# Kamino666/Video-Captioning-Transformer

Hardware: AMD Instinct MI355X
Metric: video-caption train samples/sec (whole node) (higher is better)
Workload: dtype bf16; 1 GPU; configs[1]: 2 enc + 2 dec layers d=512 ff=2048 H=8 V=30522, synthetic (256,12,512) features -> 20-token captions per GPU, fwd+bwd+Adam, dropout 0.3, SCE alpha 0.5; global_batch=256, per_gpu_batch=256, seq_len=20, frames=12, parallelism=dp1, executor=list

## Files before the change

### include/vct_hip.h

```cpp
#ifndef VCT_HIP_H
#define VCT_HIP_H
#include <stdint.h>

#ifdef __cplusplus
extern "C" {
#endif

#define VCT_ABI_VERSION 15

enum { VCT_F32 = 0, VCT_BF16 = 1 };
enum { VCT_ACT_NONE = 0, VCT_ACT_GELU = 1, VCT_ACT_RELU = 2 };
enum {
  VCT_OK = 0,
  VCT_E_ARG = -1,
  VCT_E_SHAPE = -2,
  VCT_E_ALIGN = -3,
  VCT_E_WORKSPACE = -4
};

int vct_abi_version(void);
int vct_build_info(char* buf, int buflen);

typedef struct vct_gemm_adam {
  float* param; float* exp_avg; float* exp_avg_sq;
  void* shadow; int64_t ld_shadow;
  void* pk_stream; int32_t pk_K, pk_mode; int32_t pk_chunk0[4]; int32_t pk_row0; int32_t store_grad;
  const float* hyper; const int32_t* step;
} vct_gemm_adam;

typedef struct vct_gemm_desc {
  int32_t dtype;
  int32_t out_dtype;
  int32_t ta, tb;
  int32_t M, N, K;
  int32_t act;
  const void* A; int64_t lda;
  const void* B; int64_t ldb;
  void* C; int64_t ldc;
  const float* bias;
  void* preact; int64_t ld_preact;
  const void* addend; int64_t ld_addend;
  const void* dact_src; int64_t ld_dact;
  const uint32_t* seed; uint32_t site; float p_drop;
  float* bias_grad;
  void* workspace; int64_t workspace_bytes;
  int32_t split_k;
  int32_t reserved;
  int32_t n_tile_counters;
  int32_t* tile_counters;
  const vct_gemm_adam* adam;
} vct_gemm_desc;
int vct_gemm(const vct_gemm_desc* d, void* stream);
int64_t vct_gemm_workspace_bytes(const vct_gemm_desc* d);

#define VCT_GEMM_GROUP_MAX 8
int vct_gemm_grouped(const vct_gemm_desc* descs, int32_t n, void* stream);
int64_t vct_gemm_grouped_workspace_bytes(const vct_gemm_desc* descs, int32_t n, int32_t i);

typedef struct vct_attn_desc {
  int32_t dtype;
  int32_t B, H, Lq, Lk, hd;
  int32_t causal;
  int32_t key_pad_shift;
  const void* q; int64_t ldq;
  const void* k; int64_t ldk;
  const void* v; int64_t ldv;
  void* o; int64_t ldo;
  const uint8_t* key_pad;
  const uint32_t* seed; uint32_t site; float p_drop;
  const void* d_o; int64_t ld_do;
  void* dq; int64_t ld_dq;
  void* dk; int64_t ld_dk;
  void* dv; int64_t ld_dv;
  int64_t q_bs, k_bs, v_bs, o_bs;
  const int64_t* key_ids; int64_t key_ids_bs; int64_t pad_id;
} vct_attn_desc;
int vct_attn_fwd(const vct_attn_desc* d, void* stream);
int vct_attn_bwd(const vct_attn_desc* d, void* stream);

typedef struct vct_attn_weights_desc {
  int32_t dtype;
  int32_t B, H, Lq, Lk, hd;
  int32_t causal;
  int32_t key_pad_shift;
  const void* q; int64_t ldq;
  const void* k; int64_t ldk;
  float* w; int64_t ldw;
  const uint8_t* key_pad;
  int64_t q_bs, k_bs, w_bs;
  const int64_t* key_ids; int64_t key_ids_bs; int64_t pad_id;
} vct_attn_weights_desc;
int vct_attn_weights(const vct_attn_weights_desc* d, void* stream);

typedef struct vct_ss_norm { const float* gamma; const float* beta; void* y; float* mean; float* rstd; } vct_ss_norm;
typedef struct vct_layer_ss_desc {
  int32_t dtype, B, L, Lm, d, H, ff, act;
  int32_t last, causal, key_pad_shift, reserved;
  const void* wpk; int64_t nchunks;
  const void* x; const void* mem;
  const float* b_qkv; const float* b_o;
  void* qkv; void* o; void* a;
  vct_ss_norm n1;
  const float* b_cq; const float* b_ckv; const float* b_co;
  void* cq; void* ckv; void* co; void* ca;
  vct_ss_norm n2;
  const float* b1; const float* b2;
  void* hpre; void* h; void* f;
  vct_ss_norm n3;
  vct_ss_norm nf;
  const uint8_t* key_pad; const int64_t* key_ids; int64_t key_ids_bs; int64_t pad_id;
  const uint32_t* seed; float p_drop;
  uint32_t site_sa, site_n1, site_ca, site_n2, site_ff, site_n3;
  uint32_t site_emb;
  int32_t pro, feats_dtype;
  const void* feats; void* x_in; const float* b_unify; const float* pe_rows;
  const int64_t* emb_ids; int64_t emb_ids_bs; const float* emb_table; const float* emb_pos;
} vct_layer_ss_desc;
typedef struct vct_ss_pack_seg { const void* w; int64_t ldw; int32_t nchunks; int32_t transposed; int64_t dst_chunk; } vct_ss_pack_seg;
int vct_layer_ss_supported(int dtype, int d, int H, int ff, int L, int Lm);
int64_t vct_layer_ss_stream_chunks(int ff, int cross);
int vct_ss_pack(const vct_ss_pack_seg* segs, int nseg, void* dst, void* stream);
int vct_layer_ss_fwd(const vct_layer_ss_desc* layers, int n_layers, void* stream);

typedef struct vct_ss_bwd_norm { const float* gamma; const float* mean; const float* rstd; float* ws; } vct_ss_bwd_norm;
typedef struct vct_layer_ss_bwd_desc {
  int32_t dtype, B, L, d, H, ff, act, last, causal, key_pad_shift;
  const void* wpk; int64_t nchunks;
  const void* dy; void* dx; const void* y_last;
  const void* x; const void* qkv; const void* a; const void* x1; const void* hpre; const void* f;
  vct_ss_bwd_norm n1, n3, nf;
  void* df; void* dhpre; void* da; void* dqkv;
  const uint8_t* key_pad; const int64_t* key_ids; int64_t key_ids_bs; int64_t pad_id;
  const uint32_t* seed; float p_drop;
  uint32_t site_sa, site_n1, site_ff, site_n3;
} vct_layer_ss_bwd_desc;
int64_t vct_layer_ss_bwd_stream_chunks(int ff);
int vct_layer_ss_bwd(const vct_layer_ss_bwd_desc* layers, int n_layers, void* stream);

int vct_add_ln_fwd(int dtype, int M, int d, const void* x, const void* res, const float* gamma,
                   const float* beta, void* y, float* mean, float* rstd, const uint32_t* seed,
                   uint32_t site, float p_drop, void* stream);
int vct_add_ln_ln_fwd(int dtype, int M, int d, const void* x, const void* res, const float* gamma, const float* beta,
                      void* y, float* mean, float* rstd, const float* gamma2, const float* beta2, void* y2, float* mean2,
                      float* rstd2, const uint32_t* seed, uint32_t site, float p_drop, void* stream);
int vct_add_ln_bwd(int dtype, int M, int d, const void* dy, const void* x, const void* res,
                   const float* gamma, const float* mean, const float* rstd, void* ds, void* dxo,
                   float* dgamma, float* dbeta, float* param_ws, const uint32_t* seed, uint32_t site,
                   float p_drop, void* stream);
int vct_add_ln_ln_bwd(int dtype, int M, int d, const void* dy2, const void* y, const float* gamma2, const float* mean2,
                      const float* rstd2, float* param_ws2, const void* x, const void* res, const float* gamma,
                      const float* mean, const float* rstd, void* ds, void* dxo, float* param_ws, const uint32_t* seed,
                      uint32_t site, float p_drop, void* stream);
int vct_ln_ws_rows(int M);
int vct_ln_param_finalize_batched(const int64_t* table_dev, int n_entries, int d, void* stream);

int vct_enc_frontend_fwd(int dtype, int B, int T, int d, const void* u, const float* pe_rows, void* z,
                         void* stream);
int vct_enc_frontend_bwd(int dtype, int B, int T, int d, const void* dz, void* du, void* stream);

#define VCT_MM_MAX_MODAL 8
typedef struct vct_mm_frontend_desc {
  int32_t dtype, n, B, d;
  int32_t n_labels, reserved;
  int32_t T[VCT_MM_MAX_MODAL];
  const void* u[VCT_MM_MAX_MODAL];
  const uint8_t* mask[VCT_MM_MAX_MODAL];
  const float* temp; const float* modal_w; const int32_t* labels;
  void* x0; uint8_t* key_pad;
  const void* dx;
  void* du[VCT_MM_MAX_MODAL];
  float* d_modal;
} vct_mm_frontend_desc;
int vct_mm_frontend_fwd(const vct_mm_frontend_desc* d, void* stream);
int vct_mm_frontend_bwd(const vct_mm_frontend_desc* d, void* stream);

#define VCT_AGG_MEAN 0
#define VCT_AGG_MAX 1
#define VCT_TEMPORAL_FIXED 0
#define VCT_TEMPORAL_LEARNED 1
typedef struct vct_enc_frontend_ex_desc {
  int32_t dtype, n, B, d;
  int32_t n_labels, agg, temporal, norm;
  int32_t emb_rows; uint32_t site; float p_drop; int32_t reserved;
  int32_t T[VCT_MM_MAX_MODAL];
  const void* u[VCT_MM_MAX_MODAL];
  const uint8_t* mask[VCT_MM_MAX_MODAL];
  const float* temp;
  const float* emb_w; const int32_t* tidx;
  const float* modal_w; const int32_t* labels;
  const float* gamma; const float* beta;
  const uint32_t* seed;
  void* x0; uint8_t* key_pad;
  float* mean; float* rstd;
  const void* dx;
  void* du[VCT_MM_MAX_MODAL];
  float* d_modal;
  float* d_emb;
  float* dpre; float* param_ws;
} vct_enc_frontend_ex_desc;
int vct_enc_frontend_ex_fwd(const vct_enc_frontend_ex_desc* d, void* stream);
int vct_enc_frontend_ex_bwd(const vct_enc_frontend_ex_desc* d, void* stream);

typedef struct vct_hmm_mix_desc {
  int32_t dtype, B, S, d;
  int32_t init, reserved;
  const uint8_t* take;
  const void* y; const void* x0; void* x;
  const void* dx;
  void* dy;
  float* acc;
  void* dx0;
} vct_hmm_mix_desc;
int vct_hmm_mix_fwd(const vct_hmm_mix_desc* d, void* stream);
int vct_hmm_mix_bwd(const vct_hmm_mix_desc* d, void* stream);

int vct_embed_fwd(int dtype, int B, int S, int d, const int64_t* ids, int64_t id_batch_stride,
                  const void* table, const float* pos, void* x, const uint32_t* seed, uint32_t site,
                  float p_drop, void* stream);
int vct_embed_bwd(int dtype, int B, int S, int d, int V, const int64_t* ids, int64_t id_batch_stride,
                  int64_t pad_id, const void* dx, float* dtable, int32_t* id_ws, int64_t id_ws_ints, int incremental,
                  const uint32_t* seed, uint32_t site, float p_drop, void* stream);

int vct_sce_loss(int dtype, int N, int S, int V, const void* logits, int64_t ldl, const int64_t* labels,
                 int64_t label_batch_stride, int64_t pad_id, float alpha, float* loss_out, void* dlogits,
                 int64_t ld_dl, float* row_ws, void* stream);

int vct_wce_loss(int dtype, int N, int S, int V, const void* logits, int64_t ldl, const int64_t* labels,
                 int64_t label_batch_stride, int64_t pad_id, const float* seq_w, float* loss_out, float* tok_logp,
                 void* dlogits, int64_t ld_dl, float* row_ws, void* stream);

int vct_group_sum(int dtype, int B, int G, int R, int d, const void* in, void* out, void* stream);

#define VCT_CIDER_MAX_LEN 64
#define VCT_CIDER_MAX_ORDER 4
typedef struct vct_cider_desc {
  int32_t B, N, L, n;
  const int64_t* ids;
  int64_t stride_b, stride_n, stride_l;
  int64_t end_id;
  double log_nvid, two_sigma_sq;
  const int32_t* vid_rows;
  int32_t n_videos, table_cap;
  const int32_t* table_keys;
  const double* table_idf;
  const int32_t* vid_ref_ptr;
  const int32_t* ref_len;
  const double* ref_norm;
  const int32_t* ref_ent_ptr;
  const int32_t* ent_keys;
  const double* ent_w;
  float* reward;
} vct_cider_desc;
int vct_cider_d(const vct_cider_desc* d, void* stream);
int vct_scst_advantages(int B, int N, const float* rewards, const float* baseline, float* adv, float* base_out, float* means,
                        void* stream);

enum { VCT_MATCH_CSL = 0, VCT_MATCH_CSL_WDS = 1 };
enum { VCT_MATCH_TEMP_NONE = 0, VCT_MATCH_TEMP_EXP = 1, VCT_MATCH_TEMP_DIV = 2 };
typedef struct vct_match_loss_desc {
  int32_t B, Dt, loss_kind, temp_kind;
  const float* text; int64_t ld_text;
  const float* vid; int64_t ld_vid;
  const float* temp;
  float* loss;
  float* dvid; int64_t ld_dvid;
  float* dtemp;
  float* sim; int64_t ld_sim;
  void* workspace; int64_t workspace_bytes;
} vct_match_loss_desc;
int vct_match_loss(const vct_match_loss_desc* d, void* stream);
int64_t vct_match_loss_workspace_bytes(int B, int Dt);

typedef struct vct_match_agg_desc {
  int32_t dtype, B, Te, d;
  int32_t empty; float beta;
  const void* mem; float* agg;
  const float* dagg; void* dmem;
} vct_match_agg_desc;
int vct_match_agg_fwd(const vct_match_agg_desc* d, void* stream);
int vct_match_agg_bwd(const vct_match_agg_desc* d, void* stream);

int vct_scale(float* x, int64_t n, float s, void* stream);
int vct_axpby(float* out, const float* x, float a, const float* y, float b, int64_t n, void* stream);

int vct_gather_pad_rows(int out_dtype, int B, int Tmax, int E, const float* store, const int64_t* offsets,
                        const int64_t* idx, void* out, uint8_t* mask, void* stream);

int vct_adam_step(float* param, const float* grad, float* exp_avg, float* exp_avg_sq, void* shadow_bf16,
                  int64_t n, float lr, float beta1, float beta2, float eps, float weight_decay,
                  int32_t* step_dev, int64_t shadow_skip_begin, int64_t shadow_skip_end, int32_t bump_step,
                  const float* hyper_dev, void* stream);
typedef struct vct_adam_pack_seg { int64_t begin, end; int32_t K, mode; int32_t chunk0[4]; void* stream; } vct_adam_pack_seg;
int vct_adam_step_pk(float* param, const float* grad, float* exp_avg, float* exp_avg_sq, void* shadow_bf16,
                     int64_t n, float lr, float beta1, float beta2, float eps, float weight_decay,
                     int32_t* step_dev, int64_t shadow_skip_begin, int64_t shadow_skip_end, int32_t bump_step,
                     const float* hyper_dev, const vct_adam_pack_seg* segs_dev, int32_t nseg, int64_t base, void* stream);
typedef struct vct_adam_range { int64_t begin, end; int32_t blk0, shadow; } vct_adam_range;
int vct_adam_step_ranges(float* param, const float* grad, float* exp_avg, float* exp_avg_sq, void* shadow_bf16,
                         const vct_adam_range* ranges_dev, int32_t nranges, int32_t total_blocks, float lr, float beta1, float beta2,
                         float eps, float weight_decay, int32_t* step_dev, const float* hyper_dev,
                         const vct_adam_pack_seg* segs_dev, int32_t nseg, void* stream);
int vct_adam_step_2d(float* param, const float* grad, float* exp_avg, float* exp_avg_sq, void* shadow_bf16,
                     void* shadow_t_bf16, int32_t rows, int32_t cols, int64_t ld_t, float lr, float beta1, float beta2,
                     float eps, float weight_decay, int32_t* step_dev, const float* hyper_dev, void* stream);

int vct_cast(int src_dtype, int dst_dtype, const void* src, void* dst, int64_t n, void* stream);
int vct_warm(const void* src, int64_t bytes, void* stream);
int vct_transpose(int dtype, int rows, int cols, const void* src, int64_t ld_src, void* dst, int64_t ld_dst, void* stream);
int vct_argmax_rows(int dtype, int rows, int cols, const void* x, int64_t ldx, int64_t* out, int64_t out_stride,
                    void* stream);
int vct_greedy_select(int dtype, int rows, int cols, const void* x, int64_t ldx, int64_t* out, int64_t out_stride,
                      int64_t end_id, uint8_t* ended, int32_t* ended_count, int64_t* all_ended_at, int32_t t,
                      void* stream);
int vct_beam_select(int dtype, int B, int K, int V, const void* x, int64_t ldx, float* scores, uint8_t* finished,
                    int32_t* parent, int64_t* out, int64_t out_stride, int64_t end_id, int64_t pad_id,
                    int32_t* finished_count, int64_t* all_finished_at, int32_t t, void* workspace, int64_t workspace_bytes,
                    void* stream);
int vct_beam_reorder(int dtype, int L, int M, int Lmax, int d, int t, const int32_t* parent, const void* src, void* dst,
                     int64_t layer_stride, void* stream);
typedef struct vct_sample_ctl {
  uint32_t seed;
  int32_t top_k;
  float inv_temp;
  float top_p;
} vct_sample_ctl;

typedef struct vct_sample_select_desc {
  int32_t dtype;
  int32_t rows, V, t;
  const void* x;
  int64_t ldx;
  int64_t* out;
  int64_t out_stride;
  int64_t end_id, pad_id;
  uint8_t* ended;
  int32_t* ended_count;
  int64_t* all_ended_at;
  float* step_logp;
  float* seq_logp;
  const vct_sample_ctl* ctl;
  void* workspace;
  int64_t workspace_bytes;
} vct_sample_select_desc;

int64_t vct_sample_select_workspace_bytes(int dtype, int rows, int V);
int vct_sample_select(const vct_sample_select_desc* d, void* stream);
enum { VCT_DEC_PRO_NONE = 0, VCT_DEC_PRO_EMBED = 1, VCT_DEC_PRO_LN = 2, VCT_DEC_PRO_LN_LN = 3, VCT_DEC_PRO_SELF_ATTN = 4,
       VCT_DEC_PRO_CROSS_ATTN = 5 };
typedef struct vct_decode_gemv_desc {
  int32_t wdtype, B, N, K;
  const void* W; int64_t ldw;
  const float* bias;
  int32_t pro, act;
  const float* x_in; int64_t ld_x;
  const float* g1; const float* b1; const float* g2; const float* b2;
  const int64_t* ids; int64_t id_stride; const float* table; const float* pos_row;
  const void* q; int64_t q_bs; const void* kc; const void* vc; int64_t kv_ld, kv_bs; int32_t H, Lk;
  const float* res; int64_t ld_res;
  void* out; int64_t ld_out; int32_t out_native; int32_t rows_per_wave;
  float* x_out;
} vct_decode_gemv_desc;
int vct_decode_gemv(const vct_decode_gemv_desc* d, void* stream);

typedef struct vct_decode_linear_desc {
  int32_t M, N, K;
  int32_t out_dtype, act, res_dtype;
  const void* x; int64_t ldx;
  const float* x_pre; int64_t ld_pre;
  const float* ln_g; const float* ln_b;
  float* x_norm; int64_t ld_norm;
  const void* W; int64_t ldw;
  const float* bias;
  const void* res; int64_t ld_res;
  void* out; int64_t ldo;
  const int64_t* ids; int64_t id_stride;
} vct_decode_linear_desc;
int vct_decode_linear(const vct_decode_linear_desc* d, void* stream);
int vct_decode_ln2(int M, int K, const float* x, int64_t ldx, const float* g1, const float* b1, const float* g2, const float* b2,
                   void* y, int64_t ldy, void* stream);

typedef struct vct_decode_block_desc {
  int32_t kind, d, ff, V, Lk, act;
  const int64_t* id; const float* table; const float* pos_row;
  const float* res; const float* res_bias; const float* part; int32_t n_part, pad0;
  const float* g1; const float* b1; const float* g2; const float* b2;
  float* x_out;
  const void* w_a; int64_t ld_a; const float* b_a;
  void* slot;
  const void* kc; const void* vc; int64_t kv_ld;
  const void* w_b; int64_t ld_b;
  float* part_out;
  float* sel_ws; int64_t* tok_out; int64_t end_id; uint8_t* ended; int32_t* ended_count; int64_t* all_ended_at; int32_t t, pad1;
} vct_decode_block_desc;
int vct_decode_block_supported(int dtype, int d, int H, int ff, int Lk);
int vct_decode_block(const vct_decode_block_desc* d, void* stream);

int vct_advance_seed(uint32_t* seed, void* stream);

int vct_cmdlist_create(void** out_list);
int vct_cmdlist_destroy(void* list);
int vct_cmdlist_begin(void* list, void* main_stream);
int vct_cmdlist_end(void* list);
int vct_cmdlist_replay(void* list, void* main_stream);
int vct_cmdlist_size(void* list);
int vct_cmdlist_streams(void* list);
int vct_cmdlist_inject_status(int status, void* stream);
int vct_cmdlist_host_call(int (*fn)(void*), void* arg, void* stream);
int vct_stream_wait(void* waiter_stream, void* signal_stream);
int vct_sync_record(int id, void* stream);
int vct_sync_wait(int id, void* stream);
int vct_comm_available(void);
int vct_comm_unique_id(uint8_t* out128);
int vct_comm_init(const uint8_t* id128, int rank, int world, void** out_comm);
int vct_comm_destroy(void* comm);
int vct_comm_rank(void* comm);
int vct_comm_world(void* comm);
int vct_comm_stream(void* comm, void** out_stream);
int vct_comm_allreduce_avg(void* comm, void* buf, int64_t count, int dtype, void* after_stream, int order_after);
int vct_comm_reduce_scatter_avg(void* comm, void* buf, int64_t count_per_rank, int dtype, void* after_stream, int order_after);
int vct_comm_all_gather(void* comm, void* buf, int64_t count_per_rank, int dtype, void* after_stream, int order_after);
int vct_comm_broadcast(void* comm, void* buf, int64_t count, int dtype, int root, void* after_stream, int order_after);
int vct_comm_wait(void* comm, void* stream);

int vct_stream_create_masked(const uint32_t* cu_mask, int words, void** out_stream);
int vct_stream_destroy(void* stream);
int vct_tap_enable(int on);
int vct_tap(int tag, int phase, void* stream);
int vct_tap_collect(int tag, float* ms_out, int cap);

#ifdef __cplusplus
}
#endif
#endif
```

### video-captioning-transformer_amd/_lib.py

```python
import ctypes as C
import os

import torch

_PKG = os.path.dirname(os.path.abspath(__file__))
LIB_PATH = os.path.join(_PKG, "libvct_hip.so")
_AB_LIB = os.environ.get("VCT_LIB_PATH")

F32, BF16 = 0, 1
ABI_VERSION = 15
GEMM_GROUP_MAX = 8
ACT = {"none": 0, None: 0, "gelu": 1, "relu": 2}
_ERR = {-1: "VCT_E_ARG (null pointer / bad enum)", -2: "VCT_E_SHAPE (unsupported shape)",
        -3: "VCT_E_ALIGN (leading dimension / alignment)", -4: "VCT_E_WORKSPACE (workspace too small)"}

vp, i32, i64, u32, f32, f64 = C.c_void_p, C.c_int32, C.c_int64, C.c_uint32, C.c_float, C.c_double


class GemmAdam(C.Structure):
    _fields_ = [("param", vp), ("exp_avg", vp), ("exp_avg_sq", vp), ("shadow", vp), ("ld_shadow", i64),
                ("pk_stream", vp), ("pk_K", i32), ("pk_mode", i32), ("pk_chunk0", i32 * 4), ("pk_row0", i32), ("store_grad", i32),
                ("hyper", vp), ("step", vp)]


class AdamRange(C.Structure):
    _fields_ = [("begin", i64), ("end", i64), ("blk0", i32), ("shadow", i32)]


class GemmDesc(C.Structure):
    _fields_ = [("dtype", i32), ("out_dtype", i32), ("ta", i32), ("tb", i32), ("M", i32), ("N", i32), ("K", i32),
                ("act", i32), ("A", vp), ("lda", i64), ("B", vp), ("ldb", i64), ("C", vp), ("ldc", i64),
                ("bias", vp), ("preact", vp), ("ld_preact", i64), ("addend", vp), ("ld_addend", i64),
                ("dact_src", vp), ("ld_dact", i64), ("seed", vp), ("site", u32), ("p_drop", f32),
                ("bias_grad", vp), ("workspace", vp), ("workspace_bytes", i64), ("split_k", i32), ("reserved", i32),
                ("n_tile_counters", i32), ("tile_counters", vp), ("adam", C.POINTER(GemmAdam))]


class AttnDesc(C.Structure):
    _fields_ = [("dtype", i32), ("B", i32), ("H", i32), ("Lq", i32), ("Lk", i32), ("hd", i32), ("causal", i32),
                ("key_pad_shift", i32), ("q", vp), ("ldq", i64), ("k", vp), ("ldk", i64), ("v", vp), ("ldv", i64),
                ("o", vp), ("ldo", i64), ("key_pad", vp), ("seed", vp), ("site", u32), ("p_drop", f32),
                ("d_o", vp), ("ld_do", i64), ("dq", vp), ("ld_dq", i64), ("dk", vp), ("ld_dk", i64),
                ("dv", vp), ("ld_dv", i64), ("q_bs", i64), ("k_bs", i64), ("v_bs", i64), ("o_bs", i64),
                ("key_ids", vp), ("key_ids_bs", i64), ("pad_id", i64)]


class AttnWeightsDesc(C.Structure):
    _fields_ = [("dtype", i32), ("B", i32), ("H", i32), ("Lq", i32), ("Lk", i32), ("hd", i32), ("causal", i32),
                ("key_pad_shift", i32), ("q", vp), ("ldq", i64), ("k", vp), ("ldk", i64), ("w", vp), ("ldw", i64),
                ("key_pad", vp), ("q_bs", i64), ("k_bs", i64), ("w_bs", i64), ("key_ids", vp), ("key_ids_bs", i64), ("pad_id", i64)]


class SsNorm(C.Structure):
    _fields_ = [("gamma", vp), ("beta", vp), ("y", vp), ("mean", vp), ("rstd", vp)]


class LayerSsDesc(C.Structure):
    _fields_ = [("dtype", i32), ("B", i32), ("L", i32), ("Lm", i32), ("d", i32), ("H", i32), ("ff", i32), ("act", i32),
                ("last", i32), ("causal", i32), ("key_pad_shift", i32), ("reserved", i32),
                ("wpk", vp), ("nchunks", i64), ("x", vp), ("mem", vp), ("b_qkv", vp), ("b_o", vp), ("qkv", vp), ("o", vp), ("a", vp),
                ("n1", SsNorm), ("b_cq", vp), ("b_ckv", vp), ("b_co", vp), ("cq", vp), ("ckv", vp), ("co", vp), ("ca", vp),
                ("n2", SsNorm), ("b1", vp), ("b2", vp), ("hpre", vp), ("h", vp), ("f", vp), ("n3", SsNorm), ("nf", SsNorm),
                ("key_pad", vp), ("key_ids", vp), ("key_ids_bs", i64), ("pad_id", i64), ("seed", vp), ("p_drop", f32),
                ("site_sa", u32), ("site_n1", u32), ("site_ca", u32), ("site_n2", u32), ("site_ff", u32), ("site_n3", u32), ("site_emb", u32),
                ("pro", i32), ("feats_dtype", i32), ("feats", vp), ("x_in", vp), ("b_unify", vp), ("pe_rows", vp),
                ("emb_ids", vp), ("emb_ids_bs", i64), ("emb_table", vp), ("emb_pos", vp)]


class SsPackSeg(C.Structure):
    _fields_ = [("w", vp), ("ldw", i64), ("nchunks", i32), ("transposed", i32), ("dst_chunk", i64)]


class AdamPackSeg(C.Structure):
    _fields_ = [("begin", i64), ("end", i64), ("K", i32), ("mode", i32), ("chunk0", i32 * 4), ("stream", vp)]


class SsBwdNorm(C.Structure):
    _fields_ = [("gamma", vp), ("mean", vp), ("rstd", vp), ("ws", vp)]


class LayerSsBwdDesc(C.Structure):
    _fields_ = [("dtype", i32), ("B", i32), ("L", i32), ("d", i32), ("H", i32), ("ff", i32), ("act", i32), ("last", i32), ("causal", i32),
                ("key_pad_shift", i32), ("wpk", vp), ("nchunks", i64), ("dy", vp), ("dx", vp), ("y_last", vp),
                ("x", vp), ("qkv", vp), ("a", vp), ("x1", vp), ("hpre", vp), ("f", vp),
                ("n1", SsBwdNorm), ("n3", SsBwdNorm), ("nf", SsBwdNorm),
                ("df", vp), ("dhpre", vp), ("da", vp), ("dqkv", vp),
                ("key_pad", vp), ("key_ids", vp), ("key_ids_bs", i64), ("pad_id", i64), ("seed", vp), ("p_drop", f32),
                ("site_sa", u32), ("site_n1", u32), ("site_ff", u32), ("site_n3", u32)]


class DecodeGemvDesc(C.Structure):
    _fields_ = [("wdtype", i32), ("B", i32), ("N", i32), ("K", i32), ("W", vp), ("ldw", i64), ("bias", vp), ("pro", i32), ("act", i32),
                ("x_in", vp), ("ld_x", i64), ("g1", vp), ("b1", vp), ("g2", vp), ("b2", vp),
                ("ids", vp), ("id_stride", i64), ("table", vp), ("pos_row", vp),
                ("q", vp), ("q_bs", i64), ("kc", vp), ("vc", vp), ("kv_ld", i64), ("kv_bs", i64), ("H", i32), ("Lk", i32),
                ("res", vp), ("ld_res", i64), ("out", vp), ("ld_out", i64), ("out_native", i32), ("rows_per_wave", i32),
                ("x_out", vp)]


class DecodeLinearDesc(C.Structure):
    _fields_ = [("M", i32), ("N", i32), ("K", i32), ("out_dtype", i32), ("act", i32), ("res_dtype", i32),
                ("x", vp), ("ldx", i64), ("x_pre", vp), ("ld_pre", i64), ("ln_g", vp), ("ln_b", vp), ("x_norm", vp), ("ld_norm", i64),
                ("W", vp), ("ldw", i64), ("bias", vp), ("res", vp), ("ld_res", i64), ("out", vp), ("ldo", i64),
                ("ids", vp), ("id_stride", i64)]


class DecodeBlockDesc(C.Structure):
    _fields_ = [("kind", i32), ("d", i32), ("ff", i32), ("V", i32), ("Lk", i32), ("act", i32),
                ("id", vp), ("table", vp), ("pos_row", vp), ("res", vp), ("res_bias", vp), ("part", vp), ("n_part", i32), ("pad0", i32),
                ("g1", vp), ("b1", vp), ("g2", vp), ("b2", vp), ("x_out", vp), ("w_a", vp), ("ld_a", i64), ("b_a", vp), ("slot", vp),
                ("kc", vp), ("vc", vp), ("kv_ld", i64), ("w_b", vp), ("ld_b", i64), ("part_out", vp),
                ("sel_ws", vp), ("tok_out", vp), ("end_id", i64), ("ended", vp), ("ended_count", vp), ("all_ended_at", vp), ("t", i32), ("pad1", i32)]


MM_MAX_MODAL = 8


class MmFrontendDesc(C.Structure):
    _fields_ = [("dtype", i32), ("n", i32), ("B", i32), ("d", i32), ("n_labels", i32), ("reserved", i32),
                ("T", i32 * MM_MAX_MODAL), ("u", vp * MM_MAX_MODAL), ("mask", vp * MM_MAX_MODAL),
                ("temp", vp), ("modal_w", vp), ("labels", vp), ("x0", vp), ("key_pad", vp), ("dx", vp),
                ("du", vp * MM_MAX_MODAL), ("d_modal", vp)]


AGG = {"avg": 0, "max": 1}
TEMPORAL = {"encoding": 0, "embedding": 1}


class EncFrontendExDesc(C.Structure):
    _fields_ = [("dtype", i32), ("n", i32), ("B", i32), ("d", i32), ("n_labels", i32), ("agg", i32), ("temporal", i32), ("norm", i32),
                ("emb_rows", i32), ("site", u32), ("p_drop", f32), ("reserved", i32),
                ("T", i32 * MM_MAX_MODAL), ("u", vp * MM_MAX_MODAL), ("mask", vp * MM_MAX_MODAL),
                ("temp", vp), ("emb_w", vp), ("tidx", vp), ("modal_w", vp), ("labels", vp), ("gamma", vp), ("beta", vp), ("seed", vp),
                ("x0", vp), ("key_pad", vp), ("mean", vp), ("rstd", vp), ("dx", vp), ("du", vp * MM_MAX_MODAL),
                ("d_modal", vp), ("d_emb", vp), ("dpre", vp), ("param_ws", vp)]


class HmmMixDesc(C.Structure):
    _fields_ = [("dtype", i32), ("B", i32), ("S", i32), ("d", i32), ("init", i32), ("reserved", i32),
                ("take", vp), ("y", vp), ("x0", vp), ("x", vp), ("dx", vp), ("dy", vp), ("acc", vp), ("dx0", vp)]


MATCH_LOSS = {"CSL": 0, "CSL_WDS": 1}
MATCH_TEMP = {"none": 0, "exp": 1, "div": 2}


class MatchLossDesc(C.Structure):
    _fields_ = [("B", i32), ("Dt", i32), ("loss_kind", i32), ("temp_kind", i32), ("text", vp), ("ld_text", i64), ("vid", vp), ("ld_vid", i64),
                ("temp", vp), ("loss", vp), ("dvid", vp), ("ld_dvid", i64), ("dtemp", vp), ("sim", vp), ("ld_sim", i64),
                ("workspace", vp), ("workspace_bytes", i64)]


class MatchAggDesc(C.Structure):
    _fields_ = [("dtype", i32), ("B", i32), ("Te", i32), ("d", i32), ("empty", i32), ("beta", f32), ("mem", vp), ("agg", vp),
                ("dagg", vp), ("dmem", vp)]


class SampleCtl(C.Structure):
    _fields_ = [("seed", u32), ("top_k", i32), ("inv_temp", f32), ("top_p", f32)]


class SampleSelectDesc(C.Structure):
    _fields_ = [("dtype", i32), ("rows", i32), ("V", i32), ("t", i32), ("x", vp), ("ldx", i64), ("out", vp), ("out_stride", i64),
                ("end_id", i64), ("pad_id", i64), ("ended", vp), ("ended_count", vp), ("all_ended_at", vp), ("step_logp", vp),
                ("seq_logp", vp), ("ctl", vp), ("workspace", vp), ("workspace_bytes", i64)]


CIDER_MAX_LEN, CIDER_MAX_ORDER = 64, 4


class CiderDesc(C.Structure):
    _fields_ = [("B", i32), ("N", i32), ("L", i32), ("n", i32), ("ids", vp), ("stride_b", i64), ("stride_n", i64), ("stride_l", i64),
                ("end_id", i64), ("log_nvid", f64), ("two_sigma_sq", f64), ("vid_rows", vp), ("n_videos", i32), ("table_cap", i32),
                ("table_keys", vp), ("table_idf", vp), ("vid_ref_ptr", vp), ("ref_len", vp), ("ref_norm", vp), ("ref_ent_ptr", vp),
                ("ent_keys", vp), ("ent_w", vp), ("reward", vp)]


DEC_PRO = {"none": 0, "embed": 1, "ln": 2, "ln_ln": 3, "self_attn": 4, "cross_attn": 5}

_SIGS = {
    "vct_abi_version": (C.c_int, []),
    "vct_build_info": (C.c_int, [C.c_char_p, C.c_int]),
    "vct_gemm": (C.c_int, [C.POINTER(GemmDesc), vp]),
    "vct_gemm_workspace_bytes": (i64, [C.POINTER(GemmDesc)]),
    "vct_gemm_grouped": (C.c_int, [C.POINTER(GemmDesc), i32, vp]),
    "vct_gemm_grouped_workspace_bytes": (i64, [C.POINTER(GemmDesc), i32, i32]),
    "vct_attn_fwd": (C.c_int, [C.POINTER(AttnDesc), vp]),
    "vct_attn_bwd": (C.c_int, [C.POINTER(AttnDesc), vp]),
    "vct_attn_weights": (C.c_int, [C.POINTER(AttnWeightsDesc), vp]),
    "vct_layer_ss_supported": (C.c_int, [C.c_int, C.c_int, C.c_int, C.c_int, C.c_int, C.c_int]),
    "vct_layer_ss_stream_chunks": (i64, [C.c_int, C.c_int]),
    "vct_ss_pack": (C.c_int, [C.POINTER(SsPackSeg), C.c_int, vp, vp]),
    "vct_layer_ss_fwd": (C.c_int, [C.POINTER(LayerSsDesc), C.c_int, vp]),
    "vct_layer_ss_bwd_stream_chunks": (i64, [C.c_int]),
    "vct_layer_ss_bwd": (C.c_int, [C.POINTER(LayerSsBwdDesc), C.c_int, vp]),
    "vct_add_ln_fwd": (C.c_int, [C.c_int, C.c_int, C.c_int, vp, vp, vp, vp, vp, vp, vp, vp, u32, f32, vp]),
    "vct_add_ln_ln_fwd": (C.c_int, [C.c_int, C.c_int, C.c_int, vp, vp, vp, vp, vp, vp, vp, vp, vp, vp, vp, vp, vp, u32, f32, vp]),
    "vct_add_ln_ln_bwd": (C.c_int, [C.c_int, C.c_int, C.c_int, vp, vp, vp, vp, vp, vp, vp, vp, vp, vp, vp, vp, vp, vp, vp, u32, f32, vp]),
    "vct_add_ln_bwd": (C.c_int, [C.c_int, C.c_int, C.c_int, vp, vp, vp, vp, vp, vp, vp, vp, vp, vp, vp, vp, u32, f32, vp]),
    "vct_ln_ws_rows": (C.c_int, [C.c_int]),
    "vct_ln_param_finalize_batched": (C.c_int, [vp, C.c_int, C.c_int, vp]),
    "vct_enc_frontend_fwd": (C.c_int, [C.c_int, C.c_int, C.c_int, C.c_int, vp, vp, vp, vp]),
    "vct_enc_frontend_bwd": (C.c_int, [C.c_int, C.c_int, C.c_int, C.c_int, vp, vp, vp]),
    "vct_mm_frontend_fwd": (C.c_int, [C.POINTER(MmFrontendDesc), vp]),
    "vct_mm_frontend_bwd": (C.c_int, [C.POINTER(MmFrontendDesc), vp]),
    "vct_enc_frontend_ex_fwd": (C.c_int, [C.POINTER(EncFrontendExDesc), vp]),
    "vct_enc_frontend_ex_bwd": (C.c_int, [C.POINTER(EncFrontendExDesc), vp]),
    "vct_hmm_mix_fwd": (C.c_int, [C.POINTER(HmmMixDesc), vp]),
    "vct_hmm_mix_bwd": (C.c_int, [C.POINTER(HmmMixDesc), vp]),
    "vct_match_loss": (C.c_int, [C.POINTER(MatchLossDesc), vp]),
    "vct_match_loss_workspace_bytes": (i64, [C.c_int, C.c_int]),
    "vct_match_agg_fwd": (C.c_int, [C.POINTER(MatchAggDesc), vp]),
    "vct_match_agg_bwd": (C.c_int, [C.POINTER(MatchAggDesc), vp]),
    "vct_scale": (C.c_int, [vp, i64, f32, vp]),
    "vct_axpby": (C.c_int, [vp, vp, f32, vp, f32, i64, vp]),
    "vct_embed_fwd": (C.c_int, [C.c_int, C.c_int, C.c_int, C.c_int, vp, i64, vp, vp, vp, vp, u32, f32, vp]),
    "vct_embed_bwd": (C.c_int, [C.c_int, C.c_int, C.c_int, C.c_int, C.c_int, vp, i64, i64, vp, vp, vp, i64, C.c_int, vp, u32, f32, vp]),
    "vct_sce_loss": (C.c_int, [C.c_int, C.c_int, C.c_int, C.c_int, vp, i64, vp, i64, i64, f32, vp, vp, i64, vp, vp]),
    "vct_wce_loss": (C.c_int, [C.c_int, C.c_int, C.c_int, C.c_int, vp, i64, vp, i64, i64, vp, vp, vp, vp, i64, vp, vp]),
    "vct_group_sum": (C.c_int, [C.c_int, C.c_int, C.c_int, C.c_int, C.c_int, vp, vp, vp]),
    "vct_cider_d": (C.c_int, [C.POINTER(CiderDesc), vp]),
    "vct_scst_advantages": (C.c_int, [C.c_int, C.c_int, vp, vp, vp, vp, vp, vp]),
    "vct_warm": (C.c_int, [vp, i64, vp]),
    "vct_cast": (C.c_int, [C.c_int, C.c_int, vp, vp, i64, vp]),
    "vct_argmax_rows": (C.c_int, [C.c_int, C.c_int, C.c_int, vp, i64, vp, i64, vp]),
    "vct_transpose": (C.c_int, [C.c_int, C.c_int, C.c_int, vp, i64, vp, i64, vp]),
    "vct_decode_gemv": (C.c_int, [C.POINTER(DecodeGemvDesc), vp]),
    "vct_decode_block_supported": (C.c_int, [C.c_int, C.c_int, C.c_int, C.c_int, C.c_int]),
    "vct_decode_block": (C.c_int, [C.POINTER(DecodeBlockDesc), vp]),
    "vct_decode_linear": (C.c_int, [C.POINTER(DecodeLinearDesc), vp]),
    "vct_decode_ln2": (C.c_int, [C.c_int, C.c_int, vp, i64, vp, vp, vp, vp, vp, i64, vp]),
    "vct_advance_seed": (C.c_int, [vp, vp]),
    "vct_greedy_select": (C.c_int, [C.c_int, C.c_int, C.c_int, vp, i64, vp, i64, i64, vp, vp, vp, i32, vp]),
    "vct_beam_select": (C.c_int, [C.c_int, C.c_int, C.c_int, C.c_int, vp, i64, vp, vp, vp, vp, i64, i64, i64, vp, vp, i32, vp, i64, vp]),
    "vct_beam_reorder": (C.c_int, [C.c_int, C.c_int, C.c_int, C.c_int, C.c_int, C.c_int, vp, vp, vp, i64, vp]),
    "vct_sample_select_workspace_bytes": (i64, [C.c_int, C.c_int, C.c_int]),
    "vct_sample_select": (C.c_int, [C.POINTER(SampleSelectDesc), vp]),
    "vct_gather_pad_rows": (C.c_int, [C.c_int, C.c_int, C.c_int, C.c_int, vp, vp, vp, vp, vp, vp]),
    "vct_adam_step": (C.c_int, [vp, vp, vp, vp, vp, i64, f32, f32, f32, f32, f32, vp, i64, i64, i32, vp, vp]),
    "vct_adam_step_pk": (C.c_int, [vp, vp, vp, vp, vp, i64, f32, f32, f32, f32, f32, vp, i64, i64, i32, vp, vp, C.c_int, i64, vp]),
    "vct_adam_step_ranges": (C.c_int, [vp, vp, vp, vp, vp, vp, i32, i32, f32, f32, f32, f32, f32, vp, vp, vp, i32, vp]),
    "vct_adam_step_2d": (C.c_int, [vp, vp, vp, vp, vp, vp, i32, i32, i64, f32, f32, f32, f32, f32, vp, vp, vp]),
    "vct_cmdlist_create": (C.c_int, [C.POINTER(vp)]),
    "vct_cmdlist_destroy": (C.c_int, [vp]),
    "vct_cmdlist_begin": (C.c_int, [vp, vp]),
    "vct_cmdlist_end": (C.c_int, [vp]),
    "vct_cmdlist_replay": (C.c_int, [vp, vp]),
    "vct_cmdlist_size": (C.c_int, [vp]),
    "vct_cmdlist_streams": (C.c_int, [vp]),
    "vct_cmdlist_inject_status": (C.c_int, [C.c_int, vp]),
    "vct_cmdlist_host_call": (C.c_int, [vp, vp, vp]),
    "vct_stream_wait": (C.c_int, [vp, vp]),
    "vct_sync_record": (C.c_int, [C.c_int, vp]),
    "vct_sync_wait": (C.c_int, [C.c_int, vp]),
    "vct_comm_available": (C.c_int, []),
    "vct_comm_unique_id": (C.c_int, [vp]),
    "vct_comm_init": (C.c_int, [vp, C.c_int, C.c_int, C.POINTER(vp)]),
    "vct_comm_destroy": (C.c_int, [vp]),
    "vct_comm_rank": (C.c_int, [vp]),
    "vct_comm_world": (C.c_int, [vp]),
    "vct_comm_stream": (C.c_int, [vp, C.POINTER(vp)]),
    "vct_comm_allreduce_avg": (C.c_int, [vp, vp, i64, C.c_int, vp, C.c_int]),
    "vct_comm_reduce_scatter_avg": (C.c_int, [vp, vp, i64, C.c_int, vp, C.c_int]),
    "vct_comm_all_gather": (C.c_int, [vp, vp, i64, C.c_int, vp, C.c_int]),
    "vct_comm_broadcast": (C.c_int, [vp, vp, i64, C.c_int, C.c_int, vp, C.c_int]),
    "vct_comm_wait": (C.c_int, [vp, vp]),
    "vct_stream_create_masked": (C.c_int, [C.POINTER(u32), C.c_int, C.POINTER(vp)]),
    "vct_stream_destroy": (C.c_int, [vp]),
    "vct_tap_enable": (C.c_int, [C.c_int]),
    "vct_tap": (C.c_int, [C.c_int, C.c_int, vp]),
    "vct_tap_collect": (C.c_int, [C.c_int, C.POINTER(f32), C.c_int]),
}
_OPTIONAL = {}
HOST_FN = C.CFUNCTYPE(C.c_int, vp)

_lib = None


def exported_symbols():
    return sorted(list(_SIGS) + list(_OPTIONAL))


def load():
    global _lib
    if _lib is not None:
        return _lib
    if _AB_LIB:
        lib = C.CDLL(_AB_LIB)
        for name, (res, args) in _SIGS.items():
            if not hasattr(lib, name):
                raise RuntimeError(f"VCT_LIB_PATH={_AB_LIB}: symbol {name} is missing (built from another include/vct_hip.h)")
            fn = getattr(lib, name)
            fn.restype, fn.argtypes = res, args
        if lib.vct_abi_version() != ABI_VERSION:
            raise RuntimeError(f"VCT_LIB_PATH={_AB_LIB}: ABI version {lib.vct_abi_version()} != {ABI_VERSION}")
        _lib = lib
        return lib
    _ensure_current()
    if not os.path.exists(LIB_PATH):
        raise RuntimeError(
            f"{LIB_PATH} is missing: the HIP extension is the product path and has no CPU/eager fallback. "
            "Build it with `python -c 'import __graft_entry__ as g; g.build()'`.")
    lib = C.CDLL(LIB_PATH)
    for name, (res, args) in _SIGS.items():
        fn = getattr(lib, name)
        fn.restype, fn.argtypes = res, args
    for name, (res, args) in _OPTIONAL.items():
        if hasattr(lib, name):
            fn = getattr(lib, name)
            fn.restype, fn.argtypes = res, args
    if lib.vct_abi_version() != ABI_VERSION:
        raise RuntimeError("libvct_hip.so ABI version mismatch")
    try:
        n = sum(1 for ln in open("/proc/self/maps") if "libamdhip64" in ln and " r-xp " in ln)
        if n > 1:
            raise RuntimeError("two copies of libamdhip64 are mapped; import torch before loading libvct_hip.so")
    except OSError:
        pass
    _lib = lib
    return lib


def _ensure_current():
    try:
        import importlib.util
        spec = importlib.util.spec_from_file_location("_vct_build", os.path.join(_PKG, "build.py"))
        mod = importlib.util.module_from_spec(spec)
        spec.loader.exec_module(mod)
        stamp = os.path.join(_PKG, "build", "stamp")
        fresh = os.path.exists(LIB_PATH) and mod._read(stamp) == mod._digest()
        if not fresh and os.path.exists(mod._hipcc()):
            import fcntl
            import sys
            os.makedirs(os.path.join(_PKG, "build"), exist_ok=True)
            with open(os.path.join(_PKG, "build", "lock"), "w") as lk:
                fcntl.flock(lk, fcntl.LOCK_EX)
                try:
                    if not (os.path.exists(LIB_PATH) and mod._read(stamp) == mod._digest()):
                        print("[vct_amd] libvct_hip.so is missing or older than csrc/: rebuilding with hipcc ...", file=sys.stderr)
                        mod.build_library()
                finally:
                    fcntl.flock(lk, fcntl.LOCK_UN)
        elif not fresh and os.path.exists(LIB_PATH):
            raise RuntimeError("csrc/ changed after libvct_hip.so was built and hipcc is not available to rebuild it")
    except Exception as e:
        raise RuntimeError(f"libvct_hip.so is missing or stale and rebuilding it failed: {e}") from e


def check(rc, what):
    if rc == 0:
        return
    if rc < 0:
        raise ValueError(f"{what}: {_ERR.get(rc, rc)}")
    if rc >= 10000:
        raise RuntimeError(f"{what}: ncclResult_t {rc - 10000}")
    raise RuntimeError(f"{what}: hipError_t {rc}")


def dtype_code(t: torch.dtype) -> int:
    if t == torch.float32:
        return F32
    if t == torch.bfloat16:
        return BF16
    raise TypeError(f"unsupported dtype {t}")


def stream_ptr() -> int:
    return torch.cuda.current_stream().cuda_stream


def ptr(t):
    return 0 if t is None else t.data_ptr()
```

### video-captioning-transformer_amd/csrc/vct_elem.hip

```cpp
#include "vct_common.h"

namespace vct {

template <typename T> struct EV { static constexpr int VEC = 16 / sizeof(T); };
template <typename T, int VEC> struct alignas(sizeof(T) * VEC) PackT { T v[VEC]; };

template <typename T>
__global__ void enc_frontend_fwd_kernel(int B, int Tn, int d, const T* __restrict__ u, const float* __restrict__ pe,
                                        T* __restrict__ z) {
  constexpr int VEC = EV<T>::VEC;
  using P = PackT<T, VEC>;
  const int b = blockIdx.x;
  const int nvec = d / VEC;
  for (int vi = threadIdx.x; vi < nvec; vi += blockDim.x) {
    float acc[VEC];
#pragma unroll
    for (int j = 0; j < VEC; j++) acc[j] = 0.0f;
    for (int t = 0; t < Tn; t++) {
      const P uv = *reinterpret_cast<const P*>(u + ((size_t)b * Tn + t) * d + vi * VEC);
      P o;
#pragma unroll
      for (int j = 0; j < VEC; j++) {
        const float f = to_f<T>(uv.v[j]);
        acc[j] += f;
        o.v[j] = from_f<T>(f + pe[(size_t)(t + 1) * d + vi * VEC + j]);
      }
      *reinterpret_cast<P*>(z + ((size_t)b * (Tn + 1) + t + 1) * d + vi * VEC) = o;
    }
    P m;
#pragma unroll
    for (int j = 0; j < VEC; j++) m.v[j] = from_f<T>(acc[j] / (float)Tn + pe[vi * VEC + j]);
    *reinterpret_cast<P*>(z + ((size_t)b * (Tn + 1)) * d + vi * VEC) = m;
  }
}

template <typename T>
__global__ void enc_frontend_bwd_kernel(int B, int Tn, int d, const T* __restrict__ dz, T* __restrict__ du) {
  constexpr int VEC = EV<T>::VEC;
  using P = PackT<T, VEC>;
  const int b = blockIdx.x;
  const int nvec = d / VEC;
  const float inv = 1.0f / (float)Tn;
  for (int vi = threadIdx.x; vi < nvec; vi += blockDim.x) {
    const P g0 = *reinterpret_cast<const P*>(dz + ((size_t)b * (Tn + 1)) * d + vi * VEC);
    for (int t = 0; t < Tn; t++) {
      const P g = *reinterpret_cast<const P*>(dz + ((size_t)b * (Tn + 1) + t + 1) * d + vi * VEC);
      P o;
#pragma unroll
      for (int j = 0; j < VEC; j++) o.v[j] = from_f<T>(to_f<T>(g.v[j]) + to_f<T>(g0.v[j]) * inv);
      *reinterpret_cast<P*>(du + ((size_t)b * Tn + t) * d + vi * VEC) = o;
    }
  }
}

template <typename T>
__global__ __launch_bounds__(256) void embed_fwd_kernel(int N, int S, int d, const int64_t* __restrict__ ids,
                                                        int64_t id_bstride, const float* __restrict__ table,
                                                        const float* __restrict__ pos, T* __restrict__ x,
                                                        const uint32_t* seed, uint32_t site, float p_drop) {
  const int lane = threadIdx.x & 63;
  const int n = blockIdx.x * 4 + (threadIdx.x >> 6);
  if (n >= N) return;
  const Dropout dr = make_dropout(seed, site, p_drop);
  const int b = n / S, s = n % S;
  const int64_t id = ids[(size_t)b * id_bstride + s];
  const float4* trow = reinterpret_cast<const float4*>(table + (size_t)id * d);
  const float4* prow = reinterpret_cast<const float4*>(pos + (size_t)s * d);
  for (int vi = lane; vi < d / 4; vi += 64) {
    const float4 tv = trow[vi], pv = prow[vi];
    const float e[4] = {tv.x + pv.x, tv.y + pv.y, tv.z + pv.z, tv.w + pv.w};
    PackT<T, 4> o;
    float dmv[4];
    drop_mults<4>(dr, (uint32_t)n * (uint32_t)d + (uint32_t)(vi * 4), dmv);
#pragma unroll
    for (int j = 0; j < 4; j++) o.v[j] = from_f<T>(e[j] * dmv[j]);
    *reinterpret_cast<PackT<T, 4>*>(x + (size_t)n * d + vi * 4) = o;
  }
}

__global__ void embed_index_kernel(int N, int S, const int64_t* __restrict__ ids, int64_t id_bstride, int64_t pad_id,
                                   int32_t* __restrict__ first_pos, int32_t* __restrict__ cnt, int32_t* __restrict__ hdr,
                                   int32_t* __restrict__ flat_cur) {
  const int n = blockIdx.x * blockDim.x + threadIdx.x;
  if (n == 0) hdr[1] = N;
  if (n >= N) return;
  const int64_t id = ids[(size_t)(n / S) * id_bstride + (n % S)];
  flat_cur[n] = (int32_t)id;
  if (id == pad_id) return;
  atomicMin(&first_pos[id], n);
  atomicAdd(&cnt[id], 1);
}

constexpr int EMB_LIGHT_MAX = 8;

template <typename T>
__device__ __forceinline__ void embed_bwd_light(int n, int N, int d, const int32_t* __restrict__ flat, int32_t pad_id,
                                                const T* __restrict__ dx, float* __restrict__ dtable,
                                                const int32_t* __restrict__ first_pos, const int32_t* __restrict__ cnt,
                                                const uint32_t* seed, uint32_t site, float p_drop) {
  constexpr int VEC = EV<T>::VEC, MAXCH = 1024 / (64 * VEC) > 0 ? 1024 / (64 * VEC) : 1;
  using P = PackT<T, VEC>;
  const int lane = threadIdx.x & 63;
  if (n >= N) return;
  const int32_t id = flat[n];
  if (id == pad_id || first_pos[id] != n) return;
  const int occurrences = cnt[id];
  if (occurrences > EMB_LIGHT_MAX) return;
  const Dropout dr = make_dropout(seed, site, p_drop);
  const int nch = d / (64 * VEC);
  const int tailv = (d - nch * 64 * VEC) / VEC;
  float acc[MAXCH + 1][VEC];
#pragma unroll
  for (int c = 0; c <= MAXCH; c++)
#pragma unroll
    for (int j = 0; j < VEC; j++) acc[c][j] = 0.0f;
  auto add_row = [&](int pos) {
#pragma unroll
    for (int c = 0; c <= MAXCH; c++) {
      const bool on = c < nch || (c == nch && lane < tailv);
      if (on) {
        const int col = (c * 64 + lane) * VEC;
        const P v = *reinterpret_cast<const P*>(dx + (size_t)pos * d + col);
        float dmv[VEC];
        drop_mults<VEC>(dr, (uint32_t)pos * (uint32_t)d + (uint32_t)col, dmv);
#pragma unroll
        for (int j = 0; j < VEC; j++) acc[c][j] += to_f<T>(v.v[j]) * dmv[j];
      }
    }
  };
  add_row(n);
  int found = 1;
  constexpr int TRIP = 16;
  for (int base = n + 1; base < N && found < occurrences; base += TRIP * 64) {
    unsigned long long bal[TRIP];
#pragma unroll
    for (int u = 0; u < TRIP; u++) {
      const int j = base + u * 64 + lane;
      const bool mt = flat[min(j, N - 1)] == id && j < N;
      bal[u] = __ballot(mt);
    }
#pragma unroll
    for (int u = 0; u < TRIP; u++) {
      unsigned long long mk = bal[u];
      while (mk != 0ull) {
        const int bit = __ffsll((long long)mk) - 1;
        mk &= mk - 1ull;
        add_row(base + u * 64 + bit);
        found++;
      }
    }
  }
#pragma unroll
  for (int c = 0; c <= MAXCH; c++) {
    const bool on = c < nch || (c == nch && lane < tailv);
    if (on) {
      const int col = (c * 64 + lane) * VEC;
#pragma unroll
      for (int j = 0; j < VEC; j += 4)
        *reinterpret_cast<float4*>(dtable + (size_t)id * d + col + j) = float4{acc[c][j], acc[c][j + 1], acc[c][j + 2], acc[c][j + 3]};
    }
  }
}

constexpr int EMB_HEAVY_WGS = 32;

template <typename T>
__global__ __launch_bounds__(1024) void embed_bwd_kernel(int N, int d, int V, const int32_t* __restrict__ flat, int32_t pad_id,
                                                         const T* __restrict__ dx, float* __restrict__ dtable,
                                                         const int32_t* __restrict__ first_pos, const int32_t* __restrict__ cnt,
                                                         const uint32_t* seed, uint32_t site, float p_drop) {
  constexpr int VEC = EV<T>::VEC, NT = 1024, NWV = NT / 64, SUBS = 8;
  using P = PackT<T, VEC>;
  if (blockIdx.x >= EMB_HEAVY_WGS) {
    embed_bwd_light<T>((blockIdx.x - EMB_HEAVY_WGS) * NWV + (threadIdx.x >> 6), N, d, flat, pad_id, dx, dtable, first_pos, cnt, seed,
                       site, p_drop);
    return;
  }
  extern __shared__ __attribute__((aligned(16))) unsigned char smem[];
  int* s_list = reinterpret_cast<int*>(smem);
  int* s_wcnt = s_list + SUBS * NT;
  int* s_off = s_wcnt + SUBS * NWV;
  int* s_own = s_off + 256;
  int* s_oid = s_own + NT;
  int* s_onum = s_oid + NT;
  int* s_ocnt = s_onum + NT;
  float* s_part = reinterpret_cast<float*>(s_ocnt + 32);
  const Dropout dr = make_dropout(seed, site, p_drop);
  const int chunks = d / VEC, slots = NT / chunks;
  const int chunk = threadIdx.x % chunks, slot = threadIdx.x / chunks;
  const bool active = slot < slots;
  const int w = threadIdx.x >> 6, l = threadIdx.x & 63;
  for (int ibase = blockIdx.x * NT; ibase < V; ibase += EMB_HEAVY_WGS * NT) {
   {
    const int pid = ibase + (int)threadIdx.x;
    const int fp = first_pos[min(pid, V - 1)];
    const int pc = cnt[min(pid, V - 1)];
    const bool own = pid < V && pc > EMB_LIGHT_MAX;
    const unsigned long long ob = __ballot(own);
    __syncthreads();
    if (l == 0) s_ocnt[w] = __popcll(ob);
    __syncthreads();
    int off = 0;
    for (int i = 0; i < w; i++) off += s_ocnt[i];
    if (own) {
      const int slot_o = off + __popcll(ob & ((1ull << l) - 1ull));
      s_own[slot_o] = fp; s_oid[slot_o] = pid; s_onum[slot_o] = pc;
    }
    if (threadIdx.x == NT - 1) s_ocnt[NWV] = off + __popcll(ob);
    __syncthreads();
   }
   const int nown = s_ocnt[NWV];
   for (int e = 0; e < nown; e++) {
    const int n = s_own[e];
    const int32_t id = s_oid[e];
    const int occurrences = s_onum[e];
    float acc[VEC];
#pragma unroll
    for (int j = 0; j < VEC; j++) acc[j] = 0.0f;
    int seen = 0;
    for (int base = n; base < N && seen < occurrences; base += SUBS * NT) {
      bool match[SUBS];
      unsigned long long bal[SUBS];
#pragma unroll
      for (int sub = 0; sub < SUBS; sub++) {
        match[sub] = flat[min(base + sub * NT + (int)threadIdx.x, N - 1)] == id;
      }
      __syncthreads();
#pragma unroll
      for (int sub = 0; sub < SUBS; sub++) {
        match[sub] = match[sub] && (base + sub * NT + (int)threadIdx.x < N);
        bal[sub] = __ballot(match[sub]);
        if (l == 0) s_wcnt[sub * NWV + w] = __popcll(bal[sub]);
      }
      __syncthreads();
      if (w == 0) {
        const int c0 = s_wcnt[2 * l], c1 = s_wcnt[2 * l + 1];
        int incl = c0 + c1;
#pragma unroll
        for (int off = 1; off < 64; off <<= 1) { const int t = __shfl_up(incl, off); if (l >= off) incl += t; }
        const int excl = incl - (c0 + c1);
        s_off[2 * l] = excl; s_off[2 * l + 1] = excl + c0;
        if (l == 63) s_off[SUBS * NWV] = incl;
      }
      __syncthreads();
#pragma unroll
      for (int sub = 0; sub < SUBS; sub++)
        if (match[sub]) s_list[s_off[sub * NWV + w] + __popcll(bal[sub] & ((1ull << l) - 1ull))] = base + sub * NT + threadIdx.x;
      const int found = s_off[SUBS * NWV];
      __syncthreads();
      if (active) {
        constexpr int DEPTH = 8;
        for (int q = ((slot - seen) % slots + slots) % slots; q < found; q += DEPTH * slots) {
          P v[DEPTH];
          int pos[DEPTH];
#pragma unroll
          for (int u = 0; u < DEPTH; u++) {
            const int qi = q + u * slots;
            pos[u] = qi < found ? s_list[qi] : -1;
            v[u] = *reinterpret_cast<const P*>(dx + (size_t)(pos[u] >= 0 ? pos[u] : n) * d + chunk * VEC);
          }
#pragma unroll
          for (int u = 0; u < DEPTH; u++) {
            if (pos[u] >= 0) {
              float dmv[VEC];
              drop_mults<VEC>(dr, (uint32_t)pos[u] * (uint32_t)d + (uint32_t)(chunk * VEC), dmv);
#pragma unroll
              for (int j = 0; j < VEC; j++) acc[j] += to_f<T>(v[u].v[j]) * dmv[j];
            }
          }
        }
      }
      seen += found;
    }
    __syncthreads();
    if (active) {
#pragma unroll
      for (int j = 0; j < VEC; j++) s_part[slot * d + chunk * VEC + j] = acc[j];
    }
    __syncthreads();
    for (int c = threadIdx.x; c < d; c += NT) {
      float sm = 0.0f;
      for (int sl = 0; sl < slots; sl++) sm += s_part[sl * d + c];
      dtable[(size_t)id * d + c] = sm;
    }
   }
  }
}

__global__ void count_valid_kernel(int N, int S, const int64_t* __restrict__ labels, int64_t lbstride, int64_t pad_id,
                                   float* __restrict__ out) {
  __shared__ float red[16];
  float c = 0.0f;
  for (int n = threadIdx.x; n < N; n += blockDim.x) c += (labels[(size_t)(n / S) * lbstride + (n % S)] != pad_id) ? 1.0f : 0.0f;
  c = block_sum<16>(c, red);
  if (threadIdx.x == 0) out[0] = c;
}

constexpr float SCE_C = 9.210340371976184f;

template <typename T, int IT, int NT>
__global__ __launch_bounds__(NT, NT / 128) void sce_loss_kernel(int N, int S, int V, const T* __restrict__ logits, int64_t ldl,
                                                        const int64_t* __restrict__ labels, int64_t lbstride,
                                                        int64_t pad_id, float alpha, T* __restrict__ dlogits, int64_t ld_dl,
                                                        float* __restrict__ row_ws) {
  __shared__ float red_m[16], red_s[16], red_q[16], red_c[16];
  constexpr int VEC = EV<T>::VEC, NW = NT / 64;
  using P = PackT<T, VEC>;
  const int n = blockIdx.x, tid = threadIdx.x, wv = tid >> 6, ln = tid & 63;
  const T* x = logits + (size_t)n * ldl;
  const int64_t y_in = labels[(size_t)(n / S) * lbstride + (n % S)];
  const bool valid = (y_in != pad_id);
  const bool oob = (y_in < 0 || y_in >= V);
  const int64_t y = oob ? 0 : y_in;
  const float nvalid = row_ws[2 * N];
  const float xy = to_f<T>(x[y]);
  const int nv = (V + VEC - 1) / VEC;
  P pk[IT];
#pragma unroll
  for (int it = 0; it < IT; it++) pk[it] = *reinterpret_cast<const P*>(x + (size_t)min(it * NT + tid, nv - 1) * VEC);
  float e[IT][VEC];
  float mx = -INFINITY;
#pragma unroll
  for (int it = 0; it < IT; it++) {
    const int vi = it * NT + tid;
#pragma unroll
    for (int j = 0; j < VEC; j++) e[it][j] = to_f<T>(pk[it].v[j]);
    if (vi >= nv - 1) {
#pragma unroll
      for (int j = 0; j < VEC; j++)
        if (vi >= nv || vi * VEC + j >= V) e[it][j] = -INFINITY;
    }
#pragma unroll
    for (int j = 0; j < VEC; j++) mx = fmaxf(mx, e[it][j]);
  }
  mx = wave_max(mx);
  if (ln == 0) red_m[wv] = mx;
  __syncthreads();
  mx = red_m[0];
#pragma unroll
  for (int i = 1; i < NW; i++) mx = fmaxf(mx, red_m[i]);
  float se = 0.0f;
#pragma unroll
  for (int it = 0; it < IT; it++)
#pragma unroll
    for (int j = 0; j < VEC; j++) { e[it][j] = __expf(e[it][j] - mx); se += e[it][j]; }
  se = wave_sum(se);
  if (ln == 0) red_s[wv] = se;
  __syncthreads();
  se = 0.0f;
#pragma unroll
  for (int i = 0; i < NW; i++) se += red_s[i];
  const float inv = 1.0f / se;
  const float beta = 1.0f - alpha;
  const float py = __expf(xy - mx) * inv;
  float q = 0.0f, cnt = 0.0f;
  if (alpha != 1.0f) {
#pragma unroll
    for (int it = 0; it < IT; it++)
#pragma unroll
      for (int j = 0; j < VEC; j++) {
        const float pj = e[it][j] * inv;
        const bool big = pj >= 1e-7f;
        q += big ? pj : 0.0f;
        cnt += big ? 0.0f : 1.0f;
      }
    q = wave_sum(q);
    cnt = wave_sum(cnt);
    if (ln == 0) { red_q[wv] = q; red_c[wv] = cnt; }
    __syncthreads();
    q = 0.0f; cnt = 0.0f;
#pragma unroll
    for (int i = 0; i < NW; i++) { q += red_q[i]; cnt += red_c[i]; }
    cnt -= (float)(IT * NT * VEC - V);
    if (py >= 1e-7f) q -= py; else cnt -= 1.0f;
  }
  if (tid == 0) {
    row_ws[n] = valid ? (oob ? __builtin_nanf("") : (mx + __logf(se)) - xy) : 0.0f;
    row_ws[N + n] = SCE_C * (q + 1e-7f * cnt);
  }
  if (dlogits == nullptr) return;
  const float a = valid ? alpha / nvalid : 0.0f;
  const float bn = (alpha != 1.0f) ? beta / (float)N : 0.0f;
  const float k_small = a - bn * SCE_C * q;
  const float k_big = k_small + bn * SCE_C;
  T* dx = dlogits + (size_t)n * ld_dl;
  const int nvo = (int)(ld_dl / VEC);
#pragma unroll
  for (int it = 0; it < IT; it++) {
    const int vi = it * NT + tid;
    if (vi < nvo) {
      P o;
#pragma unroll
      for (int j = 0; j < VEC; j++) {
        const float pj = e[it][j] * inv;
        o.v[j] = from_f<T>(pj * (pj >= 1e-7f ? k_big : k_small));
      }
      *reinterpret_cast<P*>(dx + vi * VEC) = o;
    }
  }
  __syncthreads();
  if (tid == 0) dx[y] = from_f<T>(a * (py - 1.0f) - bn * py * SCE_C * q);
}

__global__ void sce_finalize_kernel(int N, float alpha, const float* __restrict__ row_ws, float* __restrict__ loss) {
  __shared__ float red[16];
  float ce = 0.0f, rce = 0.0f;
  for (int n = threadIdx.x; n < N; n += blockDim.x) { ce += row_ws[n]; rce += row_ws[N + n]; }
  ce = block_sum<16>(ce, red);
  rce = block_sum<16>(rce, red);
  if (threadIdx.x == 0) {
    const float nvalid = row_ws[2 * N];
    const float l_ce = ce / nvalid;
    loss[0] = (alpha == 1.0f) ? l_ce : alpha * l_ce + (1.0f - alpha) * (rce / (float)N);
  }
}

template <typename TS, typename TD>
__global__ void cast_kernel(const TS* __restrict__ src, TD* __restrict__ dst, int64_t n) {
  const int64_t n4 = n / 4;
  for (int64_t i = (int64_t)blockIdx.x * blockDim.x + threadIdx.x; i < n4; i += (int64_t)gridDim.x * blockDim.x) {
    const PackT<TS, 4> s = reinterpret_cast<const PackT<TS, 4>*>(src)[i];
    PackT<TD, 4> o;
#pragma unroll
    for (int j = 0; j < 4; j++) o.v[j] = from_f<TD>(to_f<TS>(s.v[j]));
    reinterpret_cast<PackT<TD, 4>*>(dst)[i] = o;
  }
  if (blockIdx.x == 0 && threadIdx.x < (n & 3)) {
    const int64_t i = n4 * 4 + threadIdx.x;
    dst[i] = from_f<TD>(to_f<TS>(src[i]));
  }
}

template <typename TD>
__global__ __launch_bounds__(256) void gather_pad_rows_kernel(const float* __restrict__ store, const int64_t* __restrict__ offsets,
                                                              const int64_t* __restrict__ idx, int B, int Tmax, int E,
                                                              TD* __restrict__ out, uint8_t* __restrict__ mask) {
  const int row = blockIdx.x * 4 + (threadIdx.x >> 6), lane = threadIdx.x & 63;
  if (row >= B * Tmax) return;
  const int b = row / Tmax, t = row % Tmax;
  const int64_t clip = idx[b], r0 = offsets[clip], len = offsets[clip + 1] - r0;
  const bool valid = t < len;
  if (lane == 0) mask[row] = valid ? 0 : 1;
  const float* src = store + (size_t)(r0 + (valid ? t : 0)) * E;
  TD* dst = out + (size_t)row * E;
  const int e4 = (E % 4 == 0) ? E / 4 : 0;
  for (int i = lane; i < e4; i += 64) {
    PackT<float, 4> v = reinterpret_cast<const PackT<float, 4>*>(src)[i];
    PackT<TD, 4> o;
#pragma unroll
    for (int j = 0; j < 4; j++) o.v[j] = from_f<TD>(valid ? v.v[j] : 0.0f);
    reinterpret_cast<PackT<TD, 4>*>(dst)[i] = o;
  }
  for (int i = e4 * 4 + lane; i < E; i += 64) dst[i] = from_f<TD>(valid ? src[i] : 0.0f);
}

constexpr int AMX_THREADS = 1024;
template <typename T>
__global__ __launch_bounds__(AMX_THREADS) void argmax_rows_kernel(int cols, const T* __restrict__ x, int64_t ldx,
                                                          int64_t* __restrict__ out, int64_t out_stride,
                                                          int64_t end_id, uint8_t* __restrict__ ended,
                                                          int32_t* __restrict__ ended_count,
                                                          unsigned long long* __restrict__ all_ended_at, int t) {
  __shared__ float s_v[AMX_THREADS / 64];
  __shared__ int s_i[AMX_THREADS / 64];
  const T* r = x + (size_t)blockIdx.x * ldx;
  float best = -INFINITY;
  int bi = 0x7fffffff;
  constexpr int VEC = 16 / (int)sizeof(T);
  const bool vec_ok = (((uintptr_t)r) & 15) == 0;
  const int nv = vec_ok ? cols / VEC : 0;
  struct alignas(16) V { T e[VEC]; };
  for (int j = threadIdx.x; j < nv; j += AMX_THREADS) {
    const V v = reinterpret_cast<const V*>(r)[j];
#pragma unroll
    for (int u = 0; u < VEC; u++) {
      const float f = to_f<T>(v.e[u]);
      const int c = j * VEC + u;
      if (f > best || (f == best && c < bi)) { best = f; bi = c; }
    }
  }
  for (int j = nv * VEC + threadIdx.x; j < cols; j += AMX_THREADS) {
    const float v = to_f<T>(r[j]);
    if (v > best || (v == best && j < bi)) { best = v; bi = j; }
  }
#pragma unroll
  for (int o = 32; o > 0; o >>= 1) {
    const float ov = __shfl_xor(best, o);
    const int oi = __shfl_xor(bi, o);
    if (ov > best || (ov == best && oi < bi)) { best = ov; bi = oi; }
  }
  if ((threadIdx.x & 63) == 0) { s_v[threadIdx.x >> 6] = best; s_i[threadIdx.x >> 6] = bi; }
  __syncthreads();
  if (threadIdx.x == 0) {
    for (int w = 1; w < AMX_THREADS / 64; w++)
      if (s_v[w] > best || (s_v[w] == best && s_i[w] < bi)) { best = s_v[w]; bi = s_i[w]; }
    const int tok = (bi == 0x7fffffff) ? 0 : bi;
    out[(size_t)blockIdx.x * out_stride] = tok;
    if (ended != nullptr && tok == end_id && !ended[blockIdx.x]) {
      ended[blockIdx.x] = 1;
      if (atomicAdd(ended_count, 1) + 1 == (int)gridDim.x) atomicMin(all_ended_at, (unsigned long long)t);
    }
  }
}

__global__ void advance_seed_kernel(uint32_t* seed) { seed[0] += 1u; }

}
using namespace vct;

static bool dt_ok(int dt) { return dt == VCT_F32 || dt == VCT_BF16; }
static int vec_of(int dt) { return dt == VCT_BF16 ? 8 : 4; }

extern "C" int vct_enc_frontend_fwd(int dtype, int B, int T, int d, const void* u, const float* pe_rows, void* z,
                                    void* stream) {
  if (!dt_ok(dtype) || !u || !pe_rows || !z) return VCT_E_ARG;
  if (B <= 0 || T <= 0 || d <= 0) return VCT_E_SHAPE;
  if (d % vec_of(dtype)) return VCT_E_ALIGN;
  hipStream_t st = (hipStream_t)stream;
  const int threads = 128;
  if (dtype == VCT_BF16)
    vct::launch((enc_frontend_fwd_kernel<bf16_t>), dim3(B), dim3(threads), 0, st, B, T, d, (const bf16_t*)u, pe_rows, (bf16_t*)z);
  else
    vct::launch((enc_frontend_fwd_kernel<float>), dim3(B), dim3(threads), 0, st, B, T, d, (const float*)u, pe_rows, (float*)z);
  VCT_CHECK_LAUNCH();
  return VCT_OK;
}

extern "C" int vct_enc_frontend_bwd(int dtype, int B, int T, int d, const void* dz, void* du, void* stream) {
  if (!dt_ok(dtype) || !dz || !du) return VCT_E_ARG;
  if (B <= 0 || T <= 0 || d <= 0) return VCT_E_SHAPE;
  if (d % vec_of(dtype)) return VCT_E_ALIGN;
  hipStream_t st = (hipStream_t)stream;
  if (dtype == VCT_BF16)
    vct::launch((enc_frontend_bwd_kernel<bf16_t>), dim3(B), dim3(128), 0, st, B, T, d, (const bf16_t*)dz, (bf16_t*)du);
  else
    vct::launch((enc_frontend_bwd_kernel<float>), dim3(B), dim3(128), 0, st, B, T, d, (const float*)dz, (float*)du);
  VCT_CHECK_LAUNCH();
  return VCT_OK;
}

extern "C" int vct_embed_fwd(int dtype, int B, int S, int d, const int64_t* ids, int64_t id_batch_stride,
                             const void* table, const float* pos, void* x, const uint32_t* seed, uint32_t site,
                             float p_drop, void* stream) {
  if (!dt_ok(dtype) || !ids || !table || !pos || !x) return VCT_E_ARG;
  if (B <= 0 || S <= 0 || d <= 0) return VCT_E_SHAPE;
  if (d % 4) return VCT_E_ALIGN;
  hipStream_t st = (hipStream_t)stream;
  const int N = B * S;
  if (dtype == VCT_BF16)
    vct::launch((embed_fwd_kernel<bf16_t>), dim3((N + 3) / 4), dim3(256), 0, st, N, S, d, ids, id_batch_stride,
                       (const float*)table, pos, (bf16_t*)x, seed, site, p_drop);
  else
    vct::launch((embed_fwd_kernel<float>), dim3((N + 3) / 4), dim3(256), 0, st, N, S, d, ids, id_batch_stride,
                       (const float*)table, pos, (float*)x, seed, site, p_drop);
  VCT_CHECK_LAUNCH();
  return VCT_OK;
}

namespace vct {
__global__ __launch_bounds__(256) void embed_prep_kernel(int V, int d, float* __restrict__ dtable, int32_t* __restrict__ first_pos,
                                                         int32_t* __restrict__ cnt, const int32_t* __restrict__ flat_prev,
                                                         const int32_t* __restrict__ hdr, int incremental) {
  const int gt = blockIdx.x * 256 + threadIdx.x, nth = gridDim.x * 256;
  for (int i = gt; i < V; i += nth) { first_pos[i] = 0x7f7f7f7f; cnt[i] = 0; }
  const float4 z = {0.0f, 0.0f, 0.0f, 0.0f};
  if (!incremental) {
    float4* dst = reinterpret_cast<float4*>(dtable);
    const size_t n4 = (size_t)V * d / 4;
    for (size_t i = gt; i < n4; i += nth) dst[i] = z;
  } else {
    const int nprev = hdr[1], d4 = d / 4;
    const int w = gt >> 6, nw = nth >> 6, lane = threadIdx.x & 63;
    for (int r = w; r < nprev; r += nw) {
      const int id = flat_prev[r];
      if (id < 0 || id >= V) continue;
      float4* dst = reinterpret_cast<float4*>(dtable + (size_t)id * d);
      for (int c = lane; c < d4; c += 64) dst[c] = z;
    }
  }
}
}

extern "C" int vct_embed_bwd(int dtype, int B, int S, int d, int V, const int64_t* ids, int64_t id_batch_stride,
                             int64_t pad_id, const void* dx, float* dtable, int32_t* id_ws, int64_t id_ws_ints, int incremental,
                             const uint32_t* seed, uint32_t site, float p_drop, void* stream) {
  if (!dt_ok(dtype) || !ids || !dx || !dtable || !id_ws) return VCT_E_ARG;
  if (B <= 0 || S <= 0 || d <= 0 || V <= 0) return VCT_E_SHAPE;
  if (d % vec_of(dtype) || d / vec_of(dtype) > 256 || (d % 4) || d > 1024) return VCT_E_SHAPE;
  if (((uintptr_t)dtable & 15)) return VCT_E_ALIGN;
  hipStream_t st = (hipStream_t)stream;
  const int N = B * S;
  int32_t* first_pos = id_ws;
  int32_t* cnt = id_ws + V;
  int32_t* hdr = id_ws + 2 * (size_t)V;
  int32_t* flat = hdr + 4;
  if (id_ws_ints < 2 * (int64_t)V + 4 + N) return VCT_E_WORKSPACE;
  vct::launch(embed_prep_kernel, dim3(incremental ? 512 : 2048), dim3(256), 0, st, V, d, dtable, first_pos, cnt, flat, hdr,
              incremental ? 1 : 0);
  VCT_CHECK_LAUNCH();
  vct::launch(embed_index_kernel, dim3((N + 255) / 256), dim3(256), 0, st, N, S, ids, id_batch_stride, pad_id, first_pos, cnt, hdr, flat);
  VCT_CHECK_LAUNCH();
  const int vecb = vec_of(dtype);
  const int slots = 1024 / (d / vecb);
  const size_t heavy_lds = (size_t)(8 * 1024 + 8 * 16 + 256 + 3 * 1024 + 32) * sizeof(int) + (size_t)slots * d * sizeof(float);
  const dim3 grid(EMB_HEAVY_WGS + (N + 15) / 16);
  if (dtype == VCT_BF16) {
    static vct::DynLdsOptIn optin;
    if (optin.ensure((const void*)embed_bwd_kernel<bf16_t>, 160 * 1024) != hipSuccess) return VCT_E_SHAPE;
    vct::launch((embed_bwd_kernel<bf16_t>), grid, dim3(1024), heavy_lds, st, N, d, V, flat, (int32_t)pad_id, (const bf16_t*)dx, dtable,
                first_pos, cnt, seed, site, p_drop);
  } else {
    static vct::DynLdsOptIn optin;
    if (optin.ensure((const void*)embed_bwd_kernel<float>, 160 * 1024) != hipSuccess) return VCT_E_SHAPE;
    vct::launch((embed_bwd_kernel<float>), grid, dim3(1024), heavy_lds, st, N, d, V, flat, (int32_t)pad_id, (const float*)dx, dtable,
                first_pos, cnt, seed, site, p_drop);
  }
  VCT_CHECK_LAUNCH();
  return VCT_OK;
}

extern "C" int vct_sce_loss(int dtype, int N, int S, int V, const void* logits, int64_t ldl, const int64_t* labels,
                            int64_t label_batch_stride, int64_t pad_id, float alpha, float* loss_out, void* dlogits,
                            int64_t ld_dl, float* row_ws, void* stream) {
  if (!dt_ok(dtype) || !logits || !labels || !loss_out || !row_ws) return VCT_E_ARG;
  if (N <= 0 || S <= 0 || V <= 0 || N % S) return VCT_E_SHAPE;
  const int vec = vec_of(dtype);
  const int64_t vround = ((int64_t)V + vec - 1) / vec * vec;
  if (ldl < vround || ldl % vec || ((uintptr_t)logits & 15)) return VCT_E_ALIGN;
  if (dlogits && (ld_dl < vround || ld_dl % vec || ((uintptr_t)dlogits & 15))) return VCT_E_ALIGN;
  if (ld_dl > (int64_t)8 * 1024 * vec || vround > (int64_t)8 * 1024 * vec) return VCT_E_SHAPE;
  hipStream_t st = (hipStream_t)stream;
  vct::launch(count_valid_kernel, dim3(1), dim3(1024), 0, st, N, S, labels, label_batch_stride, pad_id, row_ws + 2 * (size_t)N);
  VCT_CHECK_LAUNCH();
  const int64_t width = dlogits ? (ld_dl > vround ? ld_dl : vround) : vround;
  const bool small = width <= (int64_t)4 * 1024 * vec;
#define VCT_SCE(T_, IT_, NT_) vct::launch((sce_loss_kernel<T_, IT_, NT_>), dim3(N), dim3(NT_), 0, st, N, S, V, (const T_*)logits, ldl, \
                                                 labels, label_batch_stride, pad_id, alpha, (T_*)dlogits, ld_dl, row_ws)
  if (dtype == VCT_BF16) { if (small) VCT_SCE(bf16_t, 8, 512); else VCT_SCE(bf16_t, 8, 1024); }
  else { if (small) VCT_SCE(float, 4, 1024); else VCT_SCE(float, 8, 1024); }
#undef VCT_SCE
  VCT_CHECK_LAUNCH();
  vct::launch(sce_finalize_kernel, dim3(1), dim3(1024), 0, st, N, alpha, row_ws, loss_out);
  VCT_CHECK_LAUNCH();
  return VCT_OK;
}

namespace vct {
__global__ __launch_bounds__(256) void warm_kernel(const uint4* __restrict__ src, const int64_t n16, unsigned int* sink) {
  uint4 a = {0u, 0u, 0u, 0u};
  for (int64_t i = (int64_t)blockIdx.x * 256 + threadIdx.x; i < n16; i += (int64_t)gridDim.x * 256) {
    const uint4 v = src[i];
    a.x ^= v.x; a.y ^= v.y; a.z ^= v.z; a.w ^= v.w;
  }
  if ((a.x ^ a.y) == 0x9e3779b9u && (a.z ^ a.w) == 0x7f4a7c15u && a.x == 0x85ebca6bu && sink != nullptr) *sink = a.w;
}
}
extern "C" int vct_warm(const void* src, int64_t bytes, void* stream) {
  if (!src || ((uintptr_t)src & 15)) return VCT_E_ARG;
  if (bytes < 16) return VCT_E_SHAPE;
  const int64_t n16 = bytes / 16;
  const int64_t want = (n16 + 256 * 8 - 1) / (256 * 8);
  const int blocks = (int)(want < 1 ? 1 : (want > 2048 ? 2048 : want));
  vct::launch(vct::warm_kernel, dim3(blocks), dim3(256), 0, (hipStream_t)stream, (const uint4*)src, n16, (unsigned int*)nullptr);
  VCT_CHECK_LAUNCH();
  return VCT_OK;
}

extern "C" int vct_cast(int src_dtype, int dst_dtype, const void* src, void* dst, int64_t n, void* stream) {
  if (!dt_ok(src_dtype) || !dt_ok(dst_dtype) || !src || !dst) return VCT_E_ARG;
  if (n <= 0) return VCT_E_SHAPE;
  hipStream_t st = (hipStream_t)stream;
  const int64_t want = (n / 4 + 255) / 256;
  const int blocks = (int)(want < 1 ? 1 : (want > 4096 ? 4096 : want));
  if (src_dtype == VCT_F32 && dst_dtype == VCT_BF16)
    vct::launch((cast_kernel<float, bf16_t>), dim3(blocks), dim3(256), 0, st, (const float*)src, (bf16_t*)dst, n);
  else if (src_dtype == VCT_BF16 && dst_dtype == VCT_F32)
    vct::launch((cast_kernel<bf16_t, float>), dim3(blocks), dim3(256), 0, st, (const bf16_t*)src, (float*)dst, n);
  else if (src_dtype == VCT_F32)
    vct::launch((cast_kernel<float, float>), dim3(blocks), dim3(256), 0, st, (const float*)src, (float*)dst, n);
  else
    vct::launch((cast_kernel<bf16_t, bf16_t>), dim3(blocks), dim3(256), 0, st, (const bf16_t*)src, (bf16_t*)dst, n);
  VCT_CHECK_LAUNCH();
  return VCT_OK;
}

extern "C" int vct_argmax_rows(int dtype, int rows, int cols, const void* x, int64_t ldx, int64_t* out, int64_t out_stride,
                               void* stream) {
  if (!dt_ok(dtype) || !x || !out) return VCT_E_ARG;
  if (rows <= 0 || cols <= 0 || out_stride <= 0) return VCT_E_SHAPE;
  hipStream_t st = (hipStream_t)stream;
  if (dtype == VCT_BF16)
    vct::launch((argmax_rows_kernel<bf16_t>), dim3(rows), dim3(AMX_THREADS), 0, st, cols, (const bf16_t*)x, ldx, out, out_stride,
                       (int64_t)0, (uint8_t*)nullptr, (int32_t*)nullptr, (unsigned long long*)nullptr, 0);
  else
    vct::launch((argmax_rows_kernel<float>), dim3(rows), dim3(AMX_THREADS), 0, st, cols, (const float*)x, ldx, out, out_stride,
                       (int64_t)0, (uint8_t*)nullptr, (int32_t*)nullptr, (unsigned long long*)nullptr, 0);
  VCT_CHECK_LAUNCH();
  return VCT_OK;
}

extern "C" int vct_greedy_select(int dtype, int rows, int cols, const void* x, int64_t ldx, int64_t* out, int64_t out_stride,
                                 int64_t end_id, uint8_t* ended, int32_t* ended_count, int64_t* all_ended_at, int32_t t,
                                 void* stream) {
  if (!dt_ok(dtype) || !x || !out || !ended || !ended_count || !all_ended_at) return VCT_E_ARG;
  if (rows <= 0 || cols <= 0 || out_stride <= 0 || t < 0) return VCT_E_SHAPE;
  hipStream_t st = (hipStream_t)stream;
  unsigned long long* at = reinterpret_cast<unsigned long long*>(all_ended_at);
  if (dtype == VCT_BF16)
    vct::launch((argmax_rows_kernel<bf16_t>), dim3(rows), dim3(AMX_THREADS), 0, st, cols, (const bf16_t*)x, ldx, out, out_stride,
                       end_id, ended, ended_count, at, (int)t);
  else
    vct::launch((argmax_rows_kernel<float>), dim3(rows), dim3(AMX_THREADS), 0, st, cols, (const float*)x, ldx, out, out_stride,
                       end_id, ended, ended_count, at, (int)t);
  VCT_CHECK_LAUNCH();
  return VCT_OK;
}

extern "C" int vct_gather_pad_rows(int out_dtype, int B, int Tmax, int E, const float* store, const int64_t* offsets,
                                   const int64_t* idx, void* out, uint8_t* mask, void* stream) {
  if (!dt_ok(out_dtype) || !store || !offsets || !idx || !out || !mask) return VCT_E_ARG;
  if (B <= 0 || Tmax <= 0 || E <= 0) return VCT_E_SHAPE;
  if ((E % 4 == 0) && ((((uintptr_t)store) & 15) || (((uintptr_t)out) & 15))) return VCT_E_ALIGN;
  hipStream_t st = (hipStream_t)stream;
  const int blocks = (B * Tmax + 3) / 4;
  if (out_dtype == VCT_BF16)
    vct::launch((gather_pad_rows_kernel<bf16_t>), dim3(blocks), dim3(256), 0, st, store, offsets, idx, B, Tmax, E, (bf16_t*)out, mask);
  else
    vct::launch((gather_pad_rows_kernel<float>), dim3(blocks), dim3(256), 0, st, store, offsets, idx, B, Tmax, E, (float*)out, mask);
  VCT_CHECK_LAUNCH();
  return VCT_OK;
}

extern "C" int vct_advance_seed(uint32_t* seed, void* stream) {
  if (!seed) return VCT_E_ARG;
  vct::launch(advance_seed_kernel, dim3(1), dim3(1), 0, (hipStream_t)stream, seed);
  VCT_CHECK_LAUNCH();
  return VCT_OK;
}

template <bool VEC>
__global__ __launch_bounds__(256) void transpose16_kernel(int rows, int cols, const uint16_t* __restrict__ src, int64_t lds_,
                                                          uint16_t* __restrict__ dst, int64_t ldd) {
  constexpr int STR = 72;
  __shared__ __attribute__((aligned(16))) uint16_t tile[64 * STR];
  const int r0 = blockIdx.y * 64, c0 = blockIdx.x * 64, t = threadIdx.x;
  struct alignas(16) V8 { uint16_t e[8]; };
  if constexpr (VEC) {
#pragma unroll
    for (int i = 0; i < 2; i++) {
      const int row = (t >> 3) + 32 * i, ch = t & 7;
      const int r = r0 + row, c = c0 + ch * 8;
      V8 v;
#pragma unroll
      for (int j = 0; j < 8; j++) v.e[j] = 0;
      if (r < rows) {
        if (c + 8 <= cols) v = *reinterpret_cast<const V8*>(src + (size_t)r * lds_ + c);
        else for (int j = 0; j < 8; j++) if (c + j < cols) v.e[j] = src[(size_t)r * lds_ + c + j];
      }
      *reinterpret_cast<V8*>(tile + row * STR + ch * 8) = v;
    }
    __syncthreads();
#pragma unroll
    for (int i = 0; i < 2; i++) {
      const int cc = t & 63, ch = (t >> 6) + 4 * i;
      V8 v;
#pragma unroll
      for (int j = 0; j < 8; j++) v.e[j] = tile[(ch * 8 + j) * STR + cc];
      const int c = c0 + cc, r = r0 + ch * 8;
      if (c < cols && r < rows) {
        if (r + 8 <= rows) *reinterpret_cast<V8*>(dst + (size_t)c * ldd + r) = v;
        else for (int j = 0; j < 8; j++) if (r + j < rows) dst[(size_t)c * ldd + r + j] = v.e[j];
      }
    }
  } else {
    const int tx = t & 63, ty = t >> 6;
    for (int i = ty; i < 64; i += 4) {
      const int r = r0 + i, c = c0 + tx;
      tile[i * STR + tx] = (r < rows && c < cols) ? src[(size_t)r * lds_ + c] : (uint16_t)0;
    }
    __syncthreads();
    for (int i = ty; i < 64; i += 4) {
      const int c = c0 + i, r = r0 + tx;
      if (c < cols && r < rows) dst[(size_t)c * ldd + r] = tile[tx * STR + i];
    }
  }
}

extern "C" int vct_transpose(int dtype, int rows, int cols, const void* src, int64_t ld_src, void* dst, int64_t ld_dst, void* stream) {
  if (dtype != VCT_BF16 || src == nullptr || dst == nullptr) return VCT_E_ARG;
  if (rows <= 0 || cols <= 0 || ld_src < cols || ld_dst < rows) return VCT_E_SHAPE;
  const bool vec = (ld_src % 8 == 0) && (ld_dst % 8 == 0) && (((uintptr_t)src & 15) == 0) && (((uintptr_t)dst & 15) == 0);
  const dim3 grid((cols + 63) / 64, (rows + 63) / 64);
  if (vec) vct::launch(transpose16_kernel<true>, grid, dim3(256), 0, (hipStream_t)stream, rows, cols,
                       reinterpret_cast<const uint16_t*>(src), ld_src, reinterpret_cast<uint16_t*>(dst), ld_dst);
  else vct::launch(transpose16_kernel<false>, grid, dim3(256), 0, (hipStream_t)stream, rows, cols,
                   reinterpret_cast<const uint16_t*>(src), ld_src, reinterpret_cast<uint16_t*>(dst), ld_dst);
  VCT_CHECK_LAUNCH();
  return VCT_OK;
}

extern "C" int vct_abi_version(void) { return VCT_ABI_VERSION; }
extern "C" int vct_build_info(char* buf, int buflen) {
  static const char info[] = "libvct_hip gfx950 (CDNA4) abi 2; bf16 mfma 16x16x32 + f32 mfma 16x16x4";
  int n = (int)sizeof(info) - 1;
  if (buf && buflen > 0) {
    int c = n < buflen - 1 ? n : buflen - 1;
    for (int i = 0; i < c; i++) buf[i] = info[i];
    buf[c] = 0;
  }
  return n;
}
```

### video-captioning-transformer_amd/csrc/vct_optim.hip

```cpp
#include "vct_adam_core.h"

namespace vct {

struct AdamPackSeg { int64_t begin, end; int32_t K, mode; int32_t chunk0[4]; bf16_t* stream; };

__global__ __launch_bounds__(256) void adam_kernel(float* __restrict__ p, const float* __restrict__ g, float* __restrict__ m,
                                                   float* __restrict__ v, bf16_t* __restrict__ shadow, int64_t n, float lr,
                                                   float b1, float b2, float eps, float wd, const int32_t* __restrict__ step,
                                                   int64_t skip_a, int64_t skip_b, const float* __restrict__ hyper,
                                                   const AdamPackSeg* __restrict__ segs, int nseg, int64_t base) {
  const AdamConsts hc = adam_consts(lr, b1, b2, eps, wd, hyper, step);
  const int64_t n4 = n >> 2;
  for (int64_t i = (int64_t)blockIdx.x * blockDim.x + threadIdx.x; i < n4; i += (int64_t)gridDim.x * blockDim.x) {
    float4 pv = reinterpret_cast<float4*>(p)[i];
    const float4 gv = reinterpret_cast<const float4*>(g)[i];
    float4 mv = reinterpret_cast<float4*>(m)[i];
    float4 vv = reinterpret_cast<float4*>(v)[i];
    float* pp = &pv.x; const float* gp = &gv.x; float* mp = &mv.x; float* vp = &vv.x;
#pragma unroll
    for (int j = 0; j < 4; j++) adam_update(pp[j], gp[j], mp[j], vp[j], hc);
    reinterpret_cast<float4*>(p)[i] = pv;
    reinterpret_cast<float4*>(m)[i] = mv;
    reinterpret_cast<float4*>(v)[i] = vv;
    const int64_t e = i << 2;
    if (shadow != nullptr && !(e >= skip_a && e < skip_b)) {
      ushort4 o;
      o.x = f2bf(pv.x); o.y = f2bf(pv.y); o.z = f2bf(pv.z); o.w = f2bf(pv.w);
      reinterpret_cast<ushort4*>(shadow)[i] = o;
      if (nseg > 0) {
        const int64_t ef = base + e;
        int lo = 0, hi = nseg;
        while (hi - lo > 1) { const int mid = (lo + hi) >> 1; if (segs[mid].begin <= ef) lo = mid; else hi = mid; }
        const AdamPackSeg sg = segs[lo];
        if (ef >= sg.begin && ef < sg.end) {
          const int64_t rel = ef - sg.begin;
          const int r = (int)(rel / sg.K), c = (int)(rel - (int64_t)r * sg.K);
          const int64_t at = adam_pack_index(r, c, sg.mode, adam_pack_chunks(sg.chunk0[0], sg.chunk0[1], sg.chunk0[2], sg.chunk0[3]));
          if (at >= 0) *reinterpret_cast<ushort4*>(sg.stream + at) = o;
        }
      }
    }
  }
}

__global__ __launch_bounds__(256) void adam2d_kernel(float* __restrict__ p, const float* __restrict__ g, float* __restrict__ m,
                                                     float* __restrict__ v, bf16_t* __restrict__ shadow, bf16_t* __restrict__ shadow_t,
                                                     int rows, int cols, int64_t ld_t, float lr, float b1, float b2, float eps, float wd,
                                                     const int32_t* __restrict__ step, const float* __restrict__ hyper) {
  constexpr int STR = 72;
  __shared__ __attribute__((aligned(16))) bf16_t tile[64 * STR];
  const AdamConsts hc = adam_consts(lr, b1, b2, eps, wd, hyper, step);
  const int tiles_c = cols / 64;
  const int r0 = (blockIdx.x / tiles_c) * 64, c0 = (blockIdx.x % tiles_c) * 64, tid = threadIdx.x;
  float4 pv[4], gv[4], mv[4], vv[4];
#pragma unroll
  for (int i = 0; i < 4; i++) {
    const int r = min(r0 + (tid >> 4) + 16 * i, rows - 1);
    const int64_t e = (int64_t)r * cols + c0 + (tid & 15) * 4;
    pv[i] = *reinterpret_cast<const float4*>(p + e); gv[i] = *reinterpret_cast<const float4*>(g + e);
    mv[i] = *reinterpret_cast<const float4*>(m + e); vv[i] = *reinterpret_cast<const float4*>(v + e);
  }
#pragma unroll
  for (int i = 0; i < 4; i++) {
    const int rl = (tid >> 4) + 16 * i, r = r0 + rl;
    float* pp = &pv[i].x; const float* gp = &gv[i].x; float* mp = &mv[i].x; float* vp = &vv[i].x;
#pragma unroll
    for (int j = 0; j < 4; j++) adam_update(pp[j], gp[j], mp[j], vp[j], hc);
    ushort4 o;
    o.x = f2bf(pv[i].x); o.y = f2bf(pv[i].y); o.z = f2bf(pv[i].z); o.w = f2bf(pv[i].w);
    *reinterpret_cast<ushort4*>(tile + rl * STR + (tid & 15) * 4) = o;
    if (r < rows) {
      const int64_t e = (int64_t)r * cols + c0 + (tid & 15) * 4;
      *reinterpret_cast<float4*>(p + e) = pv[i];
      *reinterpret_cast<float4*>(m + e) = mv[i];
      *reinterpret_cast<float4*>(v + e) = vv[i];
      if (shadow != nullptr) *reinterpret_cast<ushort4*>(shadow + e) = o;
    }
  }
  __syncthreads();
  struct alignas(16) V8 { bf16_t e[8]; };
#pragma unroll
  for (int i = 0; i < 2; i++) {
    const int cc = tid & 63, ch = (tid >> 6) + 4 * i;
    V8 o;
#pragma unroll
    for (int j = 0; j < 8; j++) o.e[j] = tile[(ch * 8 + j) * STR + cc];
    const int r = r0 + ch * 8;
    bf16_t* dst = shadow_t + (int64_t)(c0 + cc) * ld_t + r;
    if (r + 8 <= rows) *reinterpret_cast<V8*>(dst) = o;
    else for (int j = 0; j < 8; j++) if (r + j < rows) dst[j] = o.e[j];
  }
}

struct AdamRange { int64_t begin, end; int32_t blk0, shadow; };
constexpr int ADAM_RANGE_EPB = 4096;
__global__ __launch_bounds__(256) void adam_ranges_kernel(float* __restrict__ p, const float* __restrict__ g, float* __restrict__ m,
                                                          float* __restrict__ v, bf16_t* __restrict__ shadow,
                                                          const AdamRange* __restrict__ ranges, int nranges, float lr, float b1, float b2,
                                                          float eps, float wd, const int32_t* __restrict__ step,
                                                          const float* __restrict__ hyper, const AdamPackSeg* __restrict__ segs, int nseg) {
  const AdamConsts hc = adam_consts(lr, b1, b2, eps, wd, hyper, step);
  int lo = 0, hi = nranges;
  while (hi - lo > 1) { const int mid = (lo + hi) >> 1; if (ranges[mid].blk0 <= (int)blockIdx.x) lo = mid; else hi = mid; }
  const AdamRange rg = ranges[lo];
  const int64_t e0 = rg.begin + (int64_t)((int)blockIdx.x - rg.blk0) * ADAM_RANGE_EPB;
  const int64_t e1 = e0 + ADAM_RANGE_EPB < rg.end ? e0 + ADAM_RANGE_EPB : rg.end;
  for (int64_t e = e0 + (int64_t)threadIdx.x * 4; e < e1; e += 256 * 4) {
    float4 pv = *reinterpret_cast<float4*>(p + e);
    const float4 gv = *reinterpret_cast<const float4*>(g + e);
    float4 mv = *reinterpret_cast<float4*>(m + e);
    float4 vv = *reinterpret_cast<float4*>(v + e);
    float* pp = &pv.x; const float* gp = &gv.x; float* mp = &mv.x; float* vp = &vv.x;
#pragma unroll
    for (int j = 0; j < 4; j++) adam_update(pp[j], gp[j], mp[j], vp[j], hc);
    *reinterpret_cast<float4*>(p + e) = pv;
    *reinterpret_cast<float4*>(m + e) = mv;
    *reinterpret_cast<float4*>(v + e) = vv;
    if (shadow != nullptr && rg.shadow) {
      ushort4 o;
      o.x = f2bf(pv.x); o.y = f2bf(pv.y); o.z = f2bf(pv.z); o.w = f2bf(pv.w);
      *reinterpret_cast<ushort4*>(shadow + e) = o;
      if (nseg > 0) {
        int slo = 0, shi = nseg;
        while (shi - slo > 1) { const int mid = (slo + shi) >> 1; if (segs[mid].begin <= e) slo = mid; else shi = mid; }
        const AdamPackSeg sg = segs[slo];
        if (e >= sg.begin && e < sg.end) {
          const int64_t rel = e - sg.begin;
          const int r = (int)(rel / sg.K), c = (int)(rel - (int64_t)r * sg.K);
          const int64_t at = adam_pack_index(r, c, sg.mode, adam_pack_chunks(sg.chunk0[0], sg.chunk0[1], sg.chunk0[2], sg.chunk0[3]));
          if (at >= 0) *reinterpret_cast<ushort4*>(sg.stream + at) = o;
        }
      }
    }
  }
}

__global__ void bump_step_kernel(int32_t* step) { step[0] += 1; }

}
using namespace vct;

extern "C" int vct_adam_step(float* param, const float* grad, float* exp_avg, float* exp_avg_sq, void* shadow_bf16,
                             int64_t n, float lr, float beta1, float beta2, float eps, float weight_decay,
                             int32_t* step_dev, int64_t shadow_skip_begin, int64_t shadow_skip_end, int32_t bump_step,
                             const float* hyper_dev, void* stream) {
  return vct_adam_step_pk(param, grad, exp_avg, exp_avg_sq, shadow_bf16, n, lr, beta1, beta2, eps, weight_decay, step_dev, shadow_skip_begin,
                          shadow_skip_end, bump_step, hyper_dev, nullptr, 0, 0, stream);
}

extern "C" int vct_adam_step_pk(float* param, const float* grad, float* exp_avg, float* exp_avg_sq, void* shadow_bf16,
                                int64_t n, float lr, float beta1, float beta2, float eps, float weight_decay,
                                int32_t* step_dev, int64_t shadow_skip_begin, int64_t shadow_skip_end, int32_t bump_step,
                                const float* hyper_dev, const vct_adam_pack_seg* segs_dev, int32_t nseg, int64_t base, void* stream) {
  static_assert(sizeof(vct_adam_pack_seg) == sizeof(AdamPackSeg), "descriptor layout");
  if (nseg < 0 || (nseg > 0 && (segs_dev == nullptr || shadow_bf16 == nullptr || (base & 3)))) return VCT_E_ARG;
  if (!param || !grad || !exp_avg || !exp_avg_sq || !step_dev) return VCT_E_ARG;
  if (n < 0 || (n & 3)) return VCT_E_SHAPE;
  if (((uintptr_t)param | (uintptr_t)grad | (uintptr_t)exp_avg | (uintptr_t)exp_avg_sq) & 15) return VCT_E_ALIGN;
  hipStream_t st = (hipStream_t)stream;
  if (n == 0) {
    if (bump_step) { vct::launch(bump_step_kernel, dim3(1), dim3(1), 0, st, step_dev); VCT_CHECK_LAUNCH(); }
    return VCT_OK;
  }
  const int64_t want = ((n >> 2) + 255) / 256;
  const int blocks = (int)(want > 8192 ? 8192 : want);
  vct::launch(adam_kernel, dim3(blocks), dim3(256), 0, st, param, grad, exp_avg, exp_avg_sq, (bf16_t*)shadow_bf16, n, lr,
                     beta1, beta2, eps, weight_decay, step_dev, shadow_skip_begin, shadow_skip_end, hyper_dev,
                     reinterpret_cast<const AdamPackSeg*>(segs_dev), (int)nseg, base);
  VCT_CHECK_LAUNCH();
  if (bump_step) {
    vct::launch(bump_step_kernel, dim3(1), dim3(1), 0, st, step_dev);
    VCT_CHECK_LAUNCH();
  }
  return VCT_OK;
}

extern "C" int vct_adam_step_ranges(float* param, const float* grad, float* exp_avg, float* exp_avg_sq, void* shadow_bf16,
                                    const vct_adam_range* ranges_dev, int32_t nranges, int32_t total_blocks, float lr, float beta1,
                                    float beta2, float eps, float weight_decay, int32_t* step_dev, const float* hyper_dev,
                                    const vct_adam_pack_seg* segs_dev, int32_t nseg, void* stream) {
  static_assert(sizeof(vct_adam_range) == sizeof(AdamRange), "descriptor layout");
  if (!param || !grad || !exp_avg || !exp_avg_sq || !step_dev || !ranges_dev || nranges < 1 || total_blocks < 1) return VCT_E_ARG;
  if (nseg < 0 || (nseg > 0 && (segs_dev == nullptr || shadow_bf16 == nullptr))) return VCT_E_ARG;
  if (((uintptr_t)param | (uintptr_t)grad | (uintptr_t)exp_avg | (uintptr_t)exp_avg_sq) & 15) return VCT_E_ALIGN;
  vct::launch(adam_ranges_kernel, dim3(total_blocks), dim3(256), 0, (hipStream_t)stream, param, grad, exp_avg, exp_avg_sq,
              (bf16_t*)shadow_bf16, reinterpret_cast<const AdamRange*>(ranges_dev), (int)nranges, lr, beta1, beta2, eps, weight_decay,
              step_dev, hyper_dev, reinterpret_cast<const AdamPackSeg*>(segs_dev), (int)nseg);
  VCT_CHECK_LAUNCH();
  return VCT_OK;
}

extern "C" int vct_adam_step_2d(float* param, const float* grad, float* exp_avg, float* exp_avg_sq, void* shadow_bf16,
                                void* shadow_t_bf16, int32_t rows, int32_t cols, int64_t ld_t, float lr, float beta1, float beta2,
                                float eps, float weight_decay, int32_t* step_dev, const float* hyper_dev, void* stream) {
  if (!param || !grad || !exp_avg || !exp_avg_sq || !step_dev || !shadow_t_bf16) return VCT_E_ARG;
  if (rows < 1 || cols < 64 || (cols % 64) || ld_t < rows || (ld_t % 8)) return VCT_E_SHAPE;
  if (((uintptr_t)param | (uintptr_t)grad | (uintptr_t)exp_avg | (uintptr_t)exp_avg_sq | (uintptr_t)shadow_t_bf16) & 15) return VCT_E_ALIGN;
  if (shadow_bf16 != nullptr && ((uintptr_t)shadow_bf16 & 7)) return VCT_E_ALIGN;
  const int blocks = ((rows + 63) / 64) * (cols / 64);
  vct::launch(adam2d_kernel, dim3(blocks), dim3(256), 0, (hipStream_t)stream, param, grad, exp_avg, exp_avg_sq, (bf16_t*)shadow_bf16,
              (bf16_t*)shadow_t_bf16, rows, cols, ld_t, lr, beta1, beta2, eps, weight_decay, step_dev, hyper_dev);
  VCT_CHECK_LAUNCH();
  return VCT_OK;
}
```

### video-captioning-transformer_amd/ops.py

```python
from typing import Optional, Tuple

import torch

from . import _lib as L

Drop = Optional[Tuple[torch.Tensor, int, float]]



def _drop(d: Drop):
    if d is None or d[2] <= 0.0:
        return 0, 0, 0.0
    return d[0].data_ptr(), int(d[1]), float(d[2])


def _ld(t: torch.Tensor) -> int:
    assert t.dim() == 2 and t.stride(1) == 1, "row-major 2-D view required"
    return t.stride(0)


class GemmScratch:
    COUNTERS_PER_SLOT = 16384

    def __init__(self, device, nbytes: int = 64 << 20):
        self.ws = torch.empty(nbytes // 4, dtype=torch.float32, device=device)
        self.counters = torch.zeros(L.GEMM_GROUP_MAX * self.COUNTERS_PER_SLOT, dtype=torch.int32, device=device)


def _gemm_desc(a, b, out, ta, tb, bias, act, preact, addend, dact_src, dropout, bias_grad, workspace, split_k,
               n_valid, k_valid, m_valid, adam=None):
    d = L.GemmDesc()
    if adam is not None:
        d.adam = L.C.pointer(adam)
    d.dtype, d.out_dtype = L.dtype_code(a.dtype), L.dtype_code(out.dtype)
    assert b.dtype == a.dtype
    d.ta, d.tb = int(ta), int(tb)
    M = a.shape[1] if ta else a.shape[0]
    K = a.shape[0] if ta else a.shape[1]
    N = b.shape[0] if tb else b.shape[1]
    Kb = b.shape[1] if tb else b.shape[0]
    if k_valid is not None:
        K = k_valid
    else:
        assert K == Kb, (a.shape, b.shape, ta, tb)
    if n_valid is not None:
        N = n_valid
    if m_valid is not None:
        M = m_valid
    d.M, d.N, d.K = M, N, K
    d.act = L.ACT[act]
    d.A, d.lda, d.B, d.ldb, d.C, d.ldc = a.data_ptr(), _ld(a), b.data_ptr(), _ld(b), out.data_ptr(), _ld(out)
    d.bias = L.ptr(bias)
    if preact is not None:
        d.preact, d.ld_preact = preact.data_ptr(), _ld(preact)
    if addend is not None:
        d.addend, d.ld_addend = addend.data_ptr(), _ld(addend)
    if dact_src is not None:
        d.dact_src, d.ld_dact = dact_src.data_ptr(), _ld(dact_src)
    d.seed, d.site, d.p_drop = _drop(dropout)
    d.bias_grad = L.ptr(bias_grad)
    if isinstance(workspace, GemmScratch):
        d.workspace, d.workspace_bytes = workspace.ws.data_ptr(), workspace.ws.numel() * 4
        d.tile_counters, d.n_tile_counters = workspace.counters.data_ptr(), GemmScratch.COUNTERS_PER_SLOT
    elif workspace is not None:
        d.workspace, d.workspace_bytes = workspace.data_ptr(), workspace.numel() * workspace.element_size()
    d.split_k = split_k
    return d


def gemm(a: torch.Tensor, b: torch.Tensor, out: torch.Tensor, *, ta: bool = False, tb: bool = True,
         bias: Optional[torch.Tensor] = None, act: Optional[str] = None, preact: Optional[torch.Tensor] = None,
         addend: Optional[torch.Tensor] = None, dact_src: Optional[torch.Tensor] = None, dropout: Drop = None,
         bias_grad: Optional[torch.Tensor] = None, workspace=None, split_k: int = 0,
         n_valid: Optional[int] = None, k_valid: Optional[int] = None, m_valid: Optional[int] = None,
         tag: Optional[str] = None, tile: int = 0, adam=None) -> torch.Tensor:
    lib = L.load()
    d = _gemm_desc(a, b, out, ta, tb, bias, act, preact, addend, dact_src, dropout, bias_grad, workspace, split_k,
                   n_valid, k_valid, m_valid, adam)
    d.reserved = tile
    timed = _taps_on and tag in TAPS and (_taps_only is None or tag in _taps_only)
    if timed:
        tap(tag, 0)
    L.check(lib.vct_gemm(d, L.stream_ptr()), "vct_gemm")
    if timed:
        tap(tag, 1)
    return out


def gemm_grouped(items, scratch: GemmScratch, split_k: int = 0, tile: int = 0):
    lib = L.load()
    n = len(items)
    if not 1 <= n <= L.GEMM_GROUP_MAX:
        raise ValueError(f"gemm_grouped: 1..{L.GEMM_GROUP_MAX} problems per launch, got {n}")
    arr = (L.GemmDesc * n)()
    for i, it in enumerate(items):
        dy, x, dw, db = it[:4]
        d = _gemm_desc(dy, x, dw, True, False, None, None, None, None, None, None, db, None, split_k, None, None, None,
                       it[4] if len(it) > 4 else None)
        C_ = L.C
        C_.memmove(C_.byref(arr[i]), C_.byref(d), C_.sizeof(L.GemmDesc))
    arr[0].reserved = tile
    off = 0
    for i in range(n):
        need = int(lib.vct_gemm_grouped_workspace_bytes(arr, n, i))
        need = (need + 255) // 256 * 256
        arr[i].workspace, arr[i].workspace_bytes = scratch.ws.data_ptr() + off, need
        arr[i].tile_counters = scratch.counters.data_ptr() + 4 * i * GemmScratch.COUNTERS_PER_SLOT
        arr[i].n_tile_counters = GemmScratch.COUNTERS_PER_SLOT
        off += need
    if off > scratch.ws.numel() * 4:
        raise ValueError(f"gemm_grouped: scratch too small ({off} > {scratch.ws.numel() * 4} bytes)")
    L.check(lib.vct_gemm_grouped(arr, n, L.stream_ptr()), "vct_gemm_grouped")


def gemm_workspace_bytes(M: int, N: int, K: int, dtype: torch.dtype) -> int:
    lib = L.load()
    d = L.GemmDesc()
    d.dtype, d.out_dtype, d.ta, d.tb, d.M, d.N, d.K = L.dtype_code(dtype), L.F32, 1, 0, M, N, K
    return int(lib.vct_gemm_workspace_bytes(d))


def _attn_desc(dtype, B, H, Lq, Lk, hd, causal, q, k, v, key_pad, dropout):
    d = L.AttnDesc()
    d.dtype, d.B, d.H, d.Lq, d.Lk, d.hd, d.causal = L.dtype_code(dtype), B, H, Lq, Lk, hd, int(causal)
    d.q, d.ldq, d.k, d.ldk, d.v, d.ldv = q.data_ptr(), _ld(q), k.data_ptr(), _ld(k), v.data_ptr(), _ld(v)
    if isinstance(key_pad, tuple) and key_pad[0] == "ids":
        _tag, ids, pad_id = key_pad
        assert ids.dtype == torch.int64 and ids.stride(1) == 1 and ids.shape[1] >= Lk
        d.key_ids, d.key_ids_bs, d.pad_id = ids.data_ptr(), ids.stride(0), int(pad_id)
    elif isinstance(key_pad, tuple):
        m, shift = key_pad
        assert m.is_contiguous() and m.element_size() == 1 and tuple(m.shape) == (B, Lk - shift)
        d.key_pad, d.key_pad_shift = m.data_ptr(), int(shift)
    else:
        d.key_pad = L.ptr(key_pad)
    d.seed, d.site, d.p_drop = _drop(dropout)
    return d


def attn_fwd(q, k, v, o, B, H, Lq, Lk, causal=False, key_pad=None, dropout: Drop = None, kv_batch_stride: int = 0):
    hd = o.shape[1] // H
    d = _attn_desc(q.dtype, B, H, Lq, Lk, hd, causal, q, k, v, key_pad, dropout)
    d.o, d.ldo = o.data_ptr(), _ld(o)
    d.k_bs = d.v_bs = kv_batch_stride
    L.check(L.load().vct_attn_fwd(d, L.stream_ptr()), "vct_attn_fwd")
    return o


def attn_weights(q, k, w, B, H, Lq, Lk, causal=False, key_pad=None, kv_batch_stride: int = 0):
    assert w.dtype == torch.float32 and tuple(w.shape) == (B, Lq, Lk) and w.stride(2) == 1
    hd = q.shape[1] // H
    src = _attn_desc(q.dtype, B, H, Lq, Lk, hd, causal, q, k, k, key_pad, None)
    d = L.AttnWeightsDesc()
    for f in ("dtype", "B", "H", "Lq", "Lk", "hd", "causal", "key_pad_shift", "q", "ldq", "k", "ldk", "key_pad",
              "key_ids", "key_ids_bs", "pad_id"):
        setattr(d, f, getattr(src, f))
    d.w, d.ldw, d.w_bs = w.data_ptr(), (w.stride(1) if Lq > 1 else Lk), w.stride(0)
    d.k_bs = kv_batch_stride
    L.check(L.load().vct_attn_weights(d, L.stream_ptr()), "vct_attn_weights")
    return w


_ss_ok = {}
SS_CHUNK = 32768


def layer_ss_supported(dtype, d: int, H: int, ff: int, L_: int, Lm: int) -> bool:
    if dtype != torch.bfloat16:
        return False
    key = (d, H, ff, L_, Lm)
    r = _ss_ok.get(key)
    if r is None:
        r = _ss_ok[key] = bool(L.load().vct_layer_ss_supported(L.BF16, d, H, ff, L_, Lm))
    return r


def layer_ss_stream_chunks(ff: int, cross: bool) -> int:
    return int(L.load().vct_layer_ss_stream_chunks(int(ff), int(cross)))


def ss_pack(blocks, dst: torch.Tensor):
    n = len(blocks)
    segs = (L.SsPackSeg * n)()
    for i, blk in enumerate(blocks):
        w, nch, dc = blk[:3]
        tr = bool(blk[3]) if len(blk) > 3 else False
        if tr:
            assert w.dtype == torch.bfloat16 and w.stride(1) == 1 and w.shape[1] >= 512 and w.shape[0] >= 64 * nch
        else:
            assert w.dtype == torch.bfloat16 and w.stride(1) == 1 and w.shape[0] >= 512 and w.shape[1] >= 64 * nch
        segs[i].w, segs[i].ldw, segs[i].nchunks, segs[i].dst_chunk = w.data_ptr(), w.stride(0), int(nch), int(dc)
        segs[i].transposed = int(tr)
    L.check(L.load().vct_ss_pack(segs, n, dst.data_ptr(), L.stream_ptr()), "vct_ss_pack")
    return dst


def layer_ss_bwd_stream_chunks(ff: int) -> int:
    return int(L.load().vct_layer_ss_bwd_stream_chunks(int(ff)))


def layer_ss_bwd_desc(*, B, Lr, wpk, nchunks, ff, act, H, x, qkv, a, x1, hpre, f, n1, n3, outs, sites, nf=None, y_last=None, dy=None, dx=None,
                      causal=False, key_pad=None, seed=None, p_drop=0.0):
    q = L.LayerSsBwdDesc()
    q.dtype, q.B, q.L, q.d, q.H, q.ff, q.act = L.BF16, int(B), int(Lr), x.shape[1], int(H), int(ff), L.ACT[act]
    q.last, q.causal = int(nf is not None), int(causal)
    q.wpk, q.nchunks = wpk.data_ptr(), int(nchunks)
    q.dy, q.dx, q.y_last = L.ptr(dy), L.ptr(dx), L.ptr(y_last)
    q.x, q.qkv, q.a, q.x1, q.hpre, q.f = (t.data_ptr() for t in (x, qkv, a, x1, hpre, f))

    def norm(dst, t):
        dst.gamma, dst.mean, dst.rstd, dst.ws = (z.data_ptr() for z in t)
    norm(q.n1, n1)
    norm(q.n3, n3)
    if nf is not None:
        norm(q.nf, nf)
    q.df, q.dhpre, q.da, q.dqkv = (t.data_ptr() for t in outs)
    q.key_pad_shift = 0
    if isinstance(key_pad, tuple) and key_pad[0] == "ids":
        _tag, ids, pad_id = key_pad
        q.key_ids, q.key_ids_bs, q.pad_id = ids.data_ptr(), ids.stride(0), int(pad_id)
    elif isinstance(key_pad, tuple):
        m, shift = key_pad
        q.key_pad, q.key_pad_shift = m.data_ptr(), int(shift)
    elif key_pad is not None:
        q.key_pad = key_pad.data_ptr()
    q.seed, q.p_drop = L.ptr(seed), float(p_drop)
    q.site_sa, q.site_n1, q.site_ff, q.site_n3 = (int(z) for z in sites)
    return q


def layer_ss_bwd(descs):
    n = len(descs)
    arr = (L.LayerSsBwdDesc * n)(*descs)
    L.check(L.load().vct_layer_ss_bwd(arr, n, L.stream_ptr()), "vct_layer_ss_bwd")


def layer_ss_desc(*, B, Lr, x, wpk, nchunks, ff, act, H, bias, sa, n1, ffn, n3, cross=None, n2=None, nf=None, mem=None, Lm=0,
                  causal=False, key_pad=None, seed=None, p_drop=0.0, sites=(0, 0, 0, 0, 0, 0), frontend=None, embed=None):
    q = L.LayerSsDesc()
    q.dtype, q.B, q.L, q.Lm, q.d, q.H, q.ff, q.act = L.BF16, int(B), int(Lr), int(Lm), x.shape[1], int(H), int(ff), L.ACT[act]
    q.last, q.causal = int(nf is not None), int(causal)
    q.wpk, q.nchunks, q.x, q.mem = wpk.data_ptr(), int(nchunks), x.data_ptr(), L.ptr(mem)

    def norm(dst, t):
        dst.gamma, dst.beta, dst.y, dst.mean, dst.rstd = (z.data_ptr() for z in t)
    q.b_qkv, q.b_o = bias["qkv"].data_ptr(), bias["o"].data_ptr()
    q.qkv, q.o, q.a = (t.data_ptr() for t in sa)
    norm(q.n1, n1)
    if cross is not None:
        q.b_cq, q.b_ckv, q.b_co = bias["cq"].data_ptr(), bias["ckv"].data_ptr(), bias["co"].data_ptr()
        q.cq, q.ckv, q.co, q.ca = (t.data_ptr() for t in cross)
        norm(q.n2, n2)
    q.b1, q.b2 = bias["l1"].data_ptr(), bias["l2"].data_ptr()
    q.hpre, q.h, q.f = (t.data_ptr() for t in ffn)
    norm(q.n3, n3)
    if nf is not None:
        norm(q.nf, nf)
    if isinstance(key_pad, tuple) and key_pad[0] == "ids":
        _tag, ids, pad_id = key_pad
        assert ids.dtype == torch.int64 and ids.stride(1) == 1 and ids.shape[1] >= Lr
        q.key_ids, q.key_ids_bs, q.pad_id = ids.data_ptr(), ids.stride(0), int(pad_id)
    elif isinstance(key_pad, tuple):
        m, shift = key_pad
        assert m.is_contiguous() and m.element_size() == 1 and tuple(m.shape) == (B, Lr - shift)
        q.key_pad, q.key_pad_shift = m.data_ptr(), int(shift)
    elif key_pad is not None:
        q.key_pad = key_pad.data_ptr()
    if seed is not None and p_drop > 0.0:
        q.seed, q.p_drop = seed.data_ptr(), float(p_drop)
    q.site_sa, q.site_n1, q.site_ca, q.site_n2, q.site_ff, q.site_n3 = (int(s) for s in sites)
    if frontend is not None:
        feats, x_in, b_u, pe_rows = frontend
        q.pro, q.feats_dtype, q.feats, q.x_in = 1, L.dtype_code(feats.dtype), feats.data_ptr(), L.ptr(x_in)
        q.b_unify, q.pe_rows = b_u.data_ptr(), pe_rows.data_ptr()
    if embed is not None:
        ids, table, pos, site = embed
        assert ids.dtype == torch.int64 and ids.stride(1) == 1 and ids.shape[1] >= Lr
        q.pro, q.emb_ids, q.emb_ids_bs, q.emb_table, q.emb_pos, q.site_emb = 2, ids.data_ptr(), ids.stride(0), table.data_ptr(), pos.data_ptr(), int(site)
    return q


def layer_ss_fwd(descs):
    arr = (L.LayerSsDesc * len(descs))(*descs)
    L.check(L.load().vct_layer_ss_fwd(arr, len(descs), L.stream_ptr()), "vct_layer_ss_fwd")


def attn_bwd(q, k, v, d_o, dq, dk, dv, B, H, Lq, Lk, causal=False, key_pad=None, dropout: Drop = None):
    hd = d_o.shape[1] // H
    d = _attn_desc(q.dtype, B, H, Lq, Lk, hd, causal, q, k, v, key_pad, dropout)
    d.d_o, d.ld_do = d_o.data_ptr(), _ld(d_o)
    d.dq, d.ld_dq, d.dk, d.ld_dk, d.dv, d.ld_dv = dq.data_ptr(), _ld(dq), dk.data_ptr(), _ld(dk), dv.data_ptr(), _ld(dv)
    L.check(L.load().vct_attn_bwd(d, L.stream_ptr()), "vct_attn_bwd")


def add_ln_fwd(x, res, gamma, beta, y, mean, rstd, dropout: Drop = None):
    M, dm = x.shape
    s, site, p = _drop(dropout)
    L.check(L.load().vct_add_ln_fwd(L.dtype_code(x.dtype), M, dm, x.data_ptr(), L.ptr(res), gamma.data_ptr(),
                                    beta.data_ptr(), y.data_ptr(), mean.data_ptr(), rstd.data_ptr(), s, site, p,
                                    L.stream_ptr()), "vct_add_ln_fwd")
    return y


def add_ln_ln_fwd(x, res, gamma, beta, y, mean, rstd, gamma2, beta2, y2, mean2, rstd2, dropout: Drop = None):
    M, dm = x.shape
    s, site, p = _drop(dropout)
    L.check(L.load().vct_add_ln_ln_fwd(L.dtype_code(x.dtype), M, dm, x.data_ptr(), L.ptr(res), gamma.data_ptr(), beta.data_ptr(),
                                       y.data_ptr(), mean.data_ptr(), rstd.data_ptr(), gamma2.data_ptr(), beta2.data_ptr(),
                                       y2.data_ptr(), mean2.data_ptr(), rstd2.data_ptr(), s, site, p, L.stream_ptr()),
            "vct_add_ln_ln_fwd")
    return y2


def ln_ws_rows(M: int) -> int:
    return int(L.load().vct_ln_ws_rows(M))


def add_ln_bwd(dy, x, res, gamma, mean, rstd, ds, dxo, dgamma, dbeta, param_ws, dropout: Drop = None):
    M, dm = x.shape
    s, site, p = _drop(dropout)
    L.check(L.load().vct_add_ln_bwd(L.dtype_code(x.dtype), M, dm, dy.data_ptr(), x.data_ptr(), L.ptr(res),
                                    gamma.data_ptr(), mean.data_ptr(), rstd.data_ptr(), ds.data_ptr(), L.ptr(dxo),
                                    L.ptr(dgamma), L.ptr(dbeta), param_ws.data_ptr(), s, site, p,
                                    L.stream_ptr()), "vct_add_ln_bwd")


def add_ln_ln_bwd(dy2, y, gamma2, mean2, rstd2, param_ws2, x, res, gamma, mean, rstd, ds, dxo, param_ws, dropout: Drop = None):
    M, dm = x.shape
    s, site, p = _drop(dropout)
    L.check(L.load().vct_add_ln_ln_bwd(L.dtype_code(x.dtype), M, dm, dy2.data_ptr(), y.data_ptr(), gamma2.data_ptr(), mean2.data_ptr(),
                                       rstd2.data_ptr(), param_ws2.data_ptr(), x.data_ptr(), L.ptr(res), gamma.data_ptr(), mean.data_ptr(),
                                       rstd.data_ptr(), ds.data_ptr(), L.ptr(dxo), param_ws.data_ptr(), s, site, p, L.stream_ptr()),
            "vct_add_ln_ln_bwd")


def ln_param_finalize_batched(table, n_entries, d):
    L.check(L.load().vct_ln_param_finalize_batched(table.data_ptr(), n_entries, d, L.stream_ptr()), "vct_ln_param_finalize_batched")


def enc_frontend_fwd(u, pe_rows, z, B, T):
    L.check(L.load().vct_enc_frontend_fwd(L.dtype_code(u.dtype), B, T, u.shape[1], u.data_ptr(), pe_rows.data_ptr(),
                                          z.data_ptr(), L.stream_ptr()), "vct_enc_frontend_fwd")
    return z


def enc_frontend_bwd(dz, du, B, T):
    L.check(L.load().vct_enc_frontend_bwd(L.dtype_code(dz.dtype), B, T, dz.shape[1], dz.data_ptr(), du.data_ptr(),
                                          L.stream_ptr()), "vct_enc_frontend_bwd")
    return du


def _mm_desc(dtype, B, d, Ts, labels, n_labels):
    if not 2 <= len(Ts) <= L.MM_MAX_MODAL:
        raise ValueError(f"multi-modal front end: 2..{L.MM_MAX_MODAL} modalities, got {len(Ts)}")
    if labels.dtype != torch.int32 or labels.numel() != sum(t + 1 for t in Ts):
        raise ValueError("multi-modal front end: labels must be int32 [sum(T_i + 1)]")
    desc = L.MmFrontendDesc()
    desc.dtype, desc.n, desc.B, desc.d, desc.n_labels = L.dtype_code(dtype), len(Ts), B, d, n_labels
    for i, t in enumerate(Ts):
        desc.T[i] = int(t)
    desc.labels = labels.data_ptr()
    return desc


def mm_frontend_fwd(us, masks, temp, modal_w, labels, x0, key_pad, B, Ts):
    d = x0.shape[-1]
    desc = _mm_desc(x0.dtype, B, d, Ts, labels, modal_w.shape[0])
    for i, u in enumerate(us):
        desc.u[i] = u.data_ptr()
        desc.mask[i] = L.ptr(masks[i]) if masks is not None else 0
    desc.temp, desc.modal_w, desc.x0, desc.key_pad = temp.data_ptr(), modal_w.data_ptr(), x0.data_ptr(), L.ptr(key_pad)
    L.check(L.load().vct_mm_frontend_fwd(L.C.byref(desc), L.stream_ptr()), "vct_mm_frontend_fwd")
    return x0


def mm_frontend_bwd(dx, dus, d_modal, labels, B, Ts):
    desc = _mm_desc(dx.dtype, B, dx.shape[-1], Ts, labels, d_modal.shape[0])
    for i, du in enumerate(dus):
        desc.du[i] = du.data_ptr()
    desc.dx, desc.d_modal = dx.data_ptr(), d_modal.data_ptr()
    L.check(L.load().vct_mm_frontend_bwd(L.C.byref(desc), L.stream_ptr()), "vct_mm_frontend_bwd")
    return dus


def _fx_desc(dtype, B, d, Ts, agg, temp, emb_w, tidx, modal_w, labels, norm):
    n, S = len(Ts), sum(t + 1 for t in Ts)
    if not 1 <= n <= L.MM_MAX_MODAL:
        raise ValueError(f"encoder front end: 1..{L.MM_MAX_MODAL} feature streams, got {n}")
    if (temp is None) == (tidx is None):
        raise ValueError("encoder front end: exactly one temporal source (the fixed table, or the embedding weight with its row indices)")
    if tidx is not None and (tidx.dtype != torch.int32 or tidx.numel() != S):
        raise ValueError("encoder front end: tidx must be int32 [sum(T_i + 1)]")
    if n >= 2 and (labels is None or labels.dtype != torch.int32 or labels.numel() != S):
        raise ValueError("encoder front end: labels must be int32 [sum(T_i + 1)]")
    desc = L.EncFrontendExDesc()
    desc.dtype, desc.n, desc.B, desc.d, desc.agg = L.dtype_code(dtype), n, B, d, L.AGG[agg]
    for i, t in enumerate(Ts):
        desc.T[i] = int(t)
    if tidx is not None:
        desc.temporal, desc.tidx, desc.emb_w, desc.emb_rows = L.TEMPORAL["embedding"], tidx.data_ptr(), L.ptr(emb_w), emb_w.shape[0]
    else:
        desc.temporal, desc.temp = L.TEMPORAL["encoding"], temp.data_ptr()
    if n >= 2:
        desc.labels, desc.modal_w, desc.n_labels = labels.data_ptr(), L.ptr(modal_w), modal_w.shape[0]
    if norm is not None:
        s, site, p = _drop(norm.get("dropout"))
        desc.norm, desc.gamma, desc.beta, desc.mean, desc.rstd = 1, norm["gamma"].data_ptr(), L.ptr(norm.get("beta")), \
            norm["mean"].data_ptr(), norm["rstd"].data_ptr()
        desc.seed, desc.site, desc.p_drop = s, site, p
    return desc


def enc_frontend_ex_fwd(us, masks, x0, key_pad, B, Ts, *, agg="avg", temp=None, emb_w=None, tidx=None, modal_w=None, labels=None,
                        norm=None):
    desc = _fx_desc(x0.dtype, B, x0.shape[-1], Ts, agg, temp, emb_w, tidx, modal_w, labels, norm)
    for i, u in enumerate(us):
        desc.u[i] = u.data_ptr()
        desc.mask[i] = L.ptr(masks[i]) if masks is not None else 0
    desc.x0, desc.key_pad = x0.data_ptr(), L.ptr(key_pad)
    L.check(L.load().vct_enc_frontend_ex_fwd(L.C.byref(desc), L.stream_ptr()), "vct_enc_frontend_ex_fwd")
    return x0


def enc_frontend_ex_bwd(dx, dus, B, Ts, *, agg="avg", us=None, temp=None, emb_w=None, tidx=None, modal_w=None, labels=None,
                        d_modal=None, d_emb=None, norm=None, dpre=None, param_ws=None):
    desc = _fx_desc(dx.dtype, B, dx.shape[-1], Ts, agg, temp, emb_w, tidx, modal_w, labels, norm)
    for i, du in enumerate(dus):
        desc.du[i] = du.data_ptr()
        desc.u[i] = us[i].data_ptr() if us is not None else 0
    desc.dx, desc.d_modal, desc.d_emb, desc.dpre, desc.param_ws = dx.data_ptr(), L.ptr(d_modal), L.ptr(d_emb), L.ptr(dpre), L.ptr(param_ws)
    L.check(L.load().vct_enc_frontend_ex_bwd(L.C.byref(desc), L.stream_ptr()), "vct_enc_frontend_ex_bwd")
    return dus


def _hmm_desc(t, B, S, take):
    if t.dim() != 2 or t.shape[0] != B * S:
        raise ValueError(f"hierarchical encoder mix: rows [B*S, d] = [{B * S}, d] expected, got {tuple(t.shape)}")
    if take is not None and (take.dtype != torch.uint8 or take.numel() != S or not take.is_contiguous()):
        raise ValueError("hierarchical encoder mix: take must be contiguous uint8 [S]")
    desc = L.HmmMixDesc()
    desc.dtype, desc.B, desc.S, desc.d, desc.take = L.dtype_code(t.dtype), B, S, t.shape[1], L.ptr(take)
    return desc


def hmm_mix_fwd(y, x0, take, x, B, S):
    desc = _hmm_desc(x, B, S, take)
    desc.y, desc.x0, desc.x = y.data_ptr(), x0.data_ptr(), x.data_ptr()
    L.check(L.load().vct_hmm_mix_fwd(L.C.byref(desc), L.stream_ptr()), "vct_hmm_mix_fwd")
    return x


def hmm_mix_bwd(dx, take, acc, B, S, *, dy=None, dx0=None, init: bool = False):
    if acc.dtype != torch.float32 or tuple(acc.shape) != tuple(dx.shape):
        raise ValueError("hierarchical encoder mix: acc must be fp32 with the shape of dx")
    if (dy is None) == (dx0 is None):
        raise ValueError("hierarchical encoder mix: exactly one of dy (layers above 0) and dx0 (layer 0)")
    desc = _hmm_desc(dx, B, S, take if dx0 is None else None)
    desc.dx, desc.dy, desc.acc, desc.dx0, desc.init = dx.data_ptr(), L.ptr(dy), acc.data_ptr(), L.ptr(dx0), int(bool(init))
    L.check(L.load().vct_hmm_mix_bwd(L.C.byref(desc), L.stream_ptr()), "vct_hmm_mix_bwd")
    return dy if dx0 is None else dx0


def embed_fwd(ids, S, table, pos, x, dropout: Drop = None):
    B = ids.shape[0]
    s, site, p = _drop(dropout)
    L.check(L.load().vct_embed_fwd(L.dtype_code(x.dtype), B, S, x.shape[1], ids.data_ptr(), ids.stride(0),
                                   table.data_ptr(), pos.data_ptr(), x.data_ptr(), s, site, p, L.stream_ptr()),
            "vct_embed_fwd")
    return x


_embed_ws = {}
_embed_ws_retired = []


def embed_bwd(ids, S, pad_id, dx, dtable, dropout: Drop = None, id_ws=None, exclusive: bool = False, on_grow=None):
    B = ids.shape[0]
    s, site, p = _drop(dropout)
    V = dtable.shape[0]
    incremental = False
    if id_ws is None:
        key = (V, dx.device, dtable.data_ptr())
        ent = _embed_ws.get(key)
        need = 2 * V + 4 + max(B * S, 65536)
        if ent is None or ent[0].numel() < need:
            if ent is not None:
                _embed_ws_retired.append(ent[0])
                if on_grow is not None:
                    on_grow()
            ent = _embed_ws[key] = [torch.zeros(need, dtype=torch.int32, device=dx.device), None]
        id_ws = ent[0]
        incremental = exclusive and ent[1] == dtable.data_ptr()
        ent[1] = dtable.data_ptr() if exclusive else None
    else:
        assert id_ws.numel() >= 2 * V + 4 + B * S
    L.check(L.load().vct_embed_bwd(L.dtype_code(dx.dtype), B, S, dx.shape[1], V, ids.data_ptr(),
                                   ids.stride(0), int(pad_id), dx.data_ptr(), dtable.data_ptr(), id_ws.data_ptr(), id_ws.numel(), int(incremental),
                                   s, site, p, L.stream_ptr()), "vct_embed_bwd")


def sce_loss(logits, V, labels, S, pad_id, alpha, loss_out, dlogits, row_ws):
    N = logits.shape[0]
    L.check(L.load().vct_sce_loss(L.dtype_code(logits.dtype), N, S, V, logits.data_ptr(), _ld(logits), labels.data_ptr(),
                                  labels.stride(0), int(pad_id), float(alpha), loss_out.data_ptr(), L.ptr(dlogits),
                                  _ld(dlogits) if dlogits is not None else 0, row_ws.data_ptr(), L.stream_ptr()),
            "vct_sce_loss")
    return loss_out


def wce_loss(logits, V, labels, S, pad_id, seq_w, loss_out, dlogits, row_ws, tok_logp=None):
    N = logits.shape[0]
    if seq_w is not None:
        assert seq_w.dtype == torch.float32 and seq_w.is_contiguous() and seq_w.numel() * S == N, (seq_w.shape, N, S)
    if tok_logp is not None:
        assert tok_logp.dtype == torch.float32 and tok_logp.is_contiguous() and tok_logp.numel() == N
    L.check(L.load().vct_wce_loss(L.dtype_code(logits.dtype), N, S, V, logits.data_ptr(), _ld(logits), labels.data_ptr(),
                                  labels.stride(0), int(pad_id), L.ptr(seq_w), loss_out.data_ptr(), L.ptr(tok_logp), L.ptr(dlogits),
                                  _ld(dlogits) if dlogits is not None else 0, row_ws.data_ptr(), L.stream_ptr()),
            "vct_wce_loss")
    return loss_out


def group_sum(src, out, B: int, G: int, R: int):
    d = src.shape[1]
    assert src.is_contiguous() and out.is_contiguous() and src.dtype == out.dtype
    assert tuple(src.shape) == (B * G * R, d) and tuple(out.shape) == (B * R, d), (src.shape, out.shape, B, G, R)
    L.check(L.load().vct_group_sum(L.dtype_code(src.dtype), B, G, R, d, src.data_ptr(), out.data_ptr(), L.stream_ptr()), "vct_group_sum")
    return out


def check_cider_ids(ids, device=None):
    if not torch.is_tensor(ids) or ids.dtype != torch.int64 or ids.dim() != 3:
        raise ValueError(f"cider_d: ids must be an int64 tensor [B, N, L], got {getattr(ids, 'dtype', type(ids))} {tuple(getattr(ids, 'shape', ()))}")
    if not ids.is_cuda or (device is not None and ids.device != device):
        raise ValueError(f"cider_d: ids must live on the reward tables' device, got {ids.device}")
    B, N, Lc = ids.shape
    if B < 1 or N < 1 or Lc < 1 or Lc > 1 + L.CIDER_MAX_LEN:
        raise ValueError(f"cider_d: ids [B >= 1, N >= 1, 1 <= L <= {1 + L.CIDER_MAX_LEN}] (start column + at most {L.CIDER_MAX_LEN} "
                         f"tokens), got {tuple(ids.shape)}")


def cider_d(ids, vid_rows, tab, out=None):
    check_cider_ids(ids)
    B, N, Lc = ids.shape
    if vid_rows.dtype != torch.int32 or tuple(vid_rows.shape) != (B,) or not vid_rows.is_contiguous() or vid_rows.device != ids.device:
        raise ValueError(f"cider_d: vid_rows must be int32 [B = {B}] on {ids.device}, got {vid_rows.dtype} {tuple(vid_rows.shape)} on {vid_rows.device}")
    if not 1 <= int(tab.n) <= L.CIDER_MAX_ORDER:
        raise ValueError(f"cider_d: n-gram orders 1 .. {L.CIDER_MAX_ORDER}, got n = {tab.n}")
    if out is None:
        out = torch.empty(B, N, dtype=torch.float32, device=ids.device)
    elif out.dtype != torch.float32 or tuple(out.shape) != (B, N) or not out.is_contiguous() or out.device != ids.device:
        raise ValueError(f"cider_d: out must be contiguous fp32 [{B}, {N}] on {ids.device}, got {out.dtype} {tuple(out.shape)}")
    t = tab.t
    if t["table_keys"].device != ids.device:
        raise ValueError(f"cider_d: the reward tables live on {t['table_keys'].device}, ids on {ids.device}")
    d = L.CiderDesc()
    d.B, d.N, d.L, d.n = B, N, Lc - 1, int(tab.n)
    d.ids = ids.data_ptr()
    d.stride_b, d.stride_n, d.stride_l = ids.stride(0), ids.stride(1), ids.stride(2)
    d.end_id, d.log_nvid, d.two_sigma_sq = int(tab.end_id), float(tab.log_nvid), float(tab.two_sigma_sq)
    d.vid_rows, d.n_videos, d.table_cap = vid_rows.data_ptr(), int(tab.n_videos), int(tab.table_cap)
    for k in ("table_keys", "table_idf", "vid_ref_ptr", "ref_len", "ref_norm", "ref_ent_ptr", "ent_keys", "ent_w"):
        setattr(d, k, t[k].data_ptr())
    d.reward = out.data_ptr()
    L.check(L.load().vct_cider_d(d, L.stream_ptr()), "vct_cider_d")
    return out


def scst_advantages(rewards, baseline=None, adv=None, base_out=None, means=None):
    if not torch.is_tensor(rewards) or rewards.dtype != torch.float32 or rewards.dim() != 2 or not rewards.is_cuda or not rewards.is_contiguous():
        raise ValueError(f"scst_advantages: rewards must be contiguous fp32 [B, N] on the GPU, got {getattr(rewards, 'dtype', type(rewards))} "
                         f"{tuple(getattr(rewards, 'shape', ()))}")
    B, N = rewards.shape
    if B < 1 or N < 1:
        raise ValueError(f"scst_advantages: rewards [B >= 1, N >= 1], got {tuple(rewards.shape)}")
    if baseline is None and N < 2:
        raise ValueError("scst_advantages: the leave-one-out baseline needs num_samples >= 2")

    def buf(x, shape, what):
        if x is None:
            return torch.empty(shape, dtype=torch.float32, device=rewards.device)
        if x.dtype != torch.float32 or x.numel() != shape[0] or not x.is_contiguous() or x.device != rewards.device:
            raise ValueError(f"scst_advantages: {what} must be contiguous fp32 with {shape[0]} elements on {rewards.device}, "
                             f"got {x.dtype} {tuple(x.shape)} on {x.device}")
        return x
    if baseline is not None:
        baseline = buf(baseline, (B,), "baseline")
    adv, base_out, means = buf(adv, (B * N,), "adv"), buf(base_out, (B,), "base_out"), buf(means, (2,), "means")
    L.check(L.load().vct_scst_advantages(B, N, rewards.data_ptr(), L.ptr(baseline), adv.data_ptr(), base_out.data_ptr(), means.data_ptr(),
                                         L.stream_ptr()), "vct_scst_advantages")
    return adv, base_out, means


def match_loss_workspace_bytes(B: int, Dt: int) -> int:
    n = int(L.load().vct_match_loss_workspace_bytes(int(B), int(Dt)))
    if n <= 0:
        raise ValueError(f"matching loss: batch {B} x text dimension {Dt} is outside the kernels' range "
                         f"(1 <= batch <= 256, dimension a multiple of 4 up to 1024)")
    return n


def match_loss(text, vid, loss_out, workspace, *, kind: str = "CSL", temp=None, temp_kind: str = "none", dvid=None, dtemp=None, sim=None):
    B, Dt = text.shape
    if tuple(vid.shape) != (B, Dt):
        raise ValueError(f"matching loss: text {tuple(text.shape)} and video {tuple(vid.shape)} features must have one shape (square batches)")
    for t in (text, vid, dvid, sim, loss_out, temp, dtemp):
        if t is not None and t.dtype != torch.float32:
            raise ValueError("matching loss: every operand is fp32")
    need = match_loss_workspace_bytes(B, Dt)
    d = L.MatchLossDesc()
    d.B, d.Dt, d.loss_kind, d.temp_kind = B, Dt, L.MATCH_LOSS[kind], L.MATCH_TEMP[temp_kind]
    d.text, d.ld_text, d.vid, d.ld_vid = text.data_ptr(), _ld(text), vid.data_ptr(), _ld(vid)
    d.temp, d.loss, d.dtemp = L.ptr(temp), loss_out.data_ptr(), L.ptr(dtemp)
    if dvid is not None:
        d.dvid, d.ld_dvid = dvid.data_ptr(), _ld(dvid)
    if sim is not None:
        if tuple(sim.shape) != (B, B):
            raise ValueError(f"matching loss: sim must be [{B}, {B}]")
        d.sim, d.ld_sim = sim.data_ptr(), _ld(sim)
    d.workspace, d.workspace_bytes = workspace.data_ptr(), workspace.numel() * workspace.element_size()
    if d.workspace_bytes < need:
        raise ValueError(f"matching loss: workspace of {d.workspace_bytes} bytes, {need} needed")
    L.check(L.load().vct_match_loss(L.C.byref(d), L.stream_ptr()), "vct_match_loss")
    return loss_out


def _agg_desc(t, B, Te):
    if t.dim() != 2 or t.shape[0] != B * Te or not t.is_contiguous():
        raise ValueError(f"matching aggregation rows: contiguous [B*Te, d] = [{B * Te}, d] expected, got {tuple(t.shape)}")
    d = L.MatchAggDesc()
    d.dtype, d.B, d.Te, d.d = L.dtype_code(t.dtype), B, Te, t.shape[1]
    return d


def match_agg_fwd(mem, agg, B, Te):
    d = _agg_desc(mem, B, Te)
    if agg.dtype != torch.float32 or tuple(agg.shape) != (B, mem.shape[1]) or not agg.is_contiguous():
        raise ValueError("matching aggregation rows: agg must be contiguous fp32 [B, d]")
    d.mem, d.agg = mem.data_ptr(), agg.data_ptr()
    L.check(L.load().vct_match_agg_fwd(L.C.byref(d), L.stream_ptr()), "vct_match_agg_fwd")
    return agg


def match_agg_bwd(dmem, dagg, B, Te, beta: float, empty: bool = False):
    d = _agg_desc(dmem, B, Te)
    if dagg.dtype != torch.float32 or tuple(dagg.shape) != (B, dmem.shape[1]) or not dagg.is_contiguous():
        raise ValueError("matching aggregation rows: dagg must be contiguous fp32 [B, d]")
    d.dmem, d.dagg, d.beta, d.empty = dmem.data_ptr(), dagg.data_ptr(), float(beta), int(bool(empty))
    L.check(L.load().vct_match_agg_bwd(L.C.byref(d), L.stream_ptr()), "vct_match_agg_bwd")
    return dmem


def scale(x: torch.Tensor, s: float):
    if x.dtype != torch.float32 or not x.is_contiguous():
        raise ValueError("scale: a contiguous fp32 tensor")
    L.check(L.load().vct_scale(x.data_ptr(), x.numel(), float(s), L.stream_ptr()), "vct_scale")
    return x


def axpby(out: torch.Tensor, x: torch.Tensor, a: float, y: Optional[torch.Tensor] = None, b: float = 0.0):
    for t in (out, x, y):
        if t is not None and (t.dtype != torch.float32 or not t.is_contiguous() or t.numel() != out.numel()):
            raise ValueError("axpby: contiguous fp32 tensors of one size")
    L.check(L.load().vct_axpby(out.data_ptr(), x.data_ptr(), float(a), L.ptr(y), float(b), out.numel(), L.stream_ptr()), "vct_axpby")
    return out


def warm(t: torch.Tensor):
    L.check(L.load().vct_warm(t.data_ptr(), t.numel() * t.element_size(), L.stream_ptr()), "vct_warm")


def cast(src, dst):
    L.check(L.load().vct_cast(L.dtype_code(src.dtype), L.dtype_code(dst.dtype), src.data_ptr(), dst.data_ptr(),
                              src.numel(), L.stream_ptr()), "vct_cast")
    return dst


def argmax_rows(x, out, cols=None):
    L.check(L.load().vct_argmax_rows(L.dtype_code(x.dtype), x.shape[0], cols or x.shape[1], x.data_ptr(), _ld(x),
                                     out.data_ptr(), out.stride(0), L.stream_ptr()), "vct_argmax_rows")
    return out


def advance_seed(seed):
    L.check(L.load().vct_advance_seed(seed.data_ptr(), L.stream_ptr()), "vct_advance_seed")


def adam_step(param, grad, exp_avg, exp_avg_sq, shadow, lr, beta1, beta2, eps, weight_decay, step_dev, skip=(0, 0), bump=True,
              hyper=None, pack=None):
    if pack is not None:
        table, nseg, base = pack
        L.check(L.load().vct_adam_step_pk(param.data_ptr(), grad.data_ptr(), exp_avg.data_ptr(), exp_avg_sq.data_ptr(), L.ptr(shadow),
                                          param.numel(), float(lr), float(beta1), float(beta2), float(eps), float(weight_decay),
                                          step_dev.data_ptr(), int(skip[0]), int(skip[1]), int(bool(bump)), L.ptr(hyper),
                                          table.data_ptr(), int(nseg), int(base), L.stream_ptr()), "vct_adam_step_pk")
        return
    L.check(L.load().vct_adam_step(param.data_ptr(), grad.data_ptr(), exp_avg.data_ptr(), exp_avg_sq.data_ptr(), L.ptr(shadow),
                                   param.numel(), float(lr), float(beta1), float(beta2), float(eps), float(weight_decay),
                                   step_dev.data_ptr(), int(skip[0]), int(skip[1]), int(bool(bump)), L.ptr(hyper), L.stream_ptr()),
            "vct_adam_step")


def adam_ranges_table(ranges, device):
    EPB = 4096
    arr = (L.AdamRange * len(ranges))()
    blk = 0
    for i, (a, b, sh) in enumerate(ranges):
        assert a % 4 == 0 and b % 4 == 0 and b > a
        arr[i].begin, arr[i].end, arr[i].blk0, arr[i].shadow = int(a), int(b), blk, int(bool(sh))
        blk += (b - a + EPB - 1) // EPB
    table = torch.frombuffer(bytearray(bytes(arr)), dtype=torch.uint8).to(device)
    return table, len(ranges), blk


def adam_step_ranges(param, grad, exp_avg, exp_avg_sq, shadow, table, lr, beta1, beta2, eps, weight_decay, step_dev, hyper=None, pack=None):
    tab, n, blocks = table
    pk, nseg = (pack[0].data_ptr(), int(pack[1])) if pack is not None and pack[1] else (0, 0)
    L.check(L.load().vct_adam_step_ranges(param.data_ptr(), grad.data_ptr(), exp_avg.data_ptr(), exp_avg_sq.data_ptr(), L.ptr(shadow),
                                          tab.data_ptr(), int(n), int(blocks), float(lr), float(beta1), float(beta2), float(eps),
                                          float(weight_decay), step_dev.data_ptr(), L.ptr(hyper), pk, nseg, L.stream_ptr()),
            "vct_adam_step_ranges")


def adam_step_2d(param, grad, exp_avg, exp_avg_sq, shadow, shadow_t, lr, beta1, beta2, eps, weight_decay, step_dev, hyper=None):
    rows, cols = param.shape
    L.check(L.load().vct_adam_step_2d(param.data_ptr(), grad.data_ptr(), exp_avg.data_ptr(), exp_avg_sq.data_ptr(), L.ptr(shadow),
                                      shadow_t.data_ptr(), rows, cols, shadow_t.stride(0), float(lr), float(beta1), float(beta2),
                                      float(eps), float(weight_decay), step_dev.data_ptr(), L.ptr(hyper), L.stream_ptr()),
            "vct_adam_step_2d")


def adam_bump(step_dev):
    L.check(L.load().vct_adam_step(step_dev.data_ptr(), step_dev.data_ptr(), step_dev.data_ptr(), step_dev.data_ptr(), 0, 0,
                                   0.0, 0.0, 0.0, 0.0, 0.0, step_dev.data_ptr(), 0, 0, 1, 0, L.stream_ptr()), "vct_adam_step(bump)")


def greedy_select(x, out, end_id: int, ended, ended_count, all_ended_at, t: int, cols=None):
    L.check(L.load().vct_greedy_select(L.dtype_code(x.dtype), x.shape[0], cols or x.shape[1], x.data_ptr(), _ld(x),
                                       out.data_ptr(), out.stride(0), int(end_id), ended.data_ptr(), ended_count.data_ptr(),
                                       all_ended_at.data_ptr(), int(t), L.stream_ptr()), "vct_greedy_select")
    return out


def beam_select_workspace_bytes(dtype, B: int, K: int, V: int) -> int:
    chunk = 256 * (8 if dtype == torch.bfloat16 else 4)
    return B * K * ((V + chunk - 1) // chunk) * (2 + 2 * K) * 4


def beam_select(x, B: int, K: int, scores, finished, parent, out, end_id: int, pad_id: int, finished_count, all_finished_at,
                t: int, ws, cols=None):
    L.check(L.load().vct_beam_select(L.dtype_code(x.dtype), int(B), int(K), int(cols or x.shape[1]), x.data_ptr(), _ld(x),
                                     scores.data_ptr(), finished.data_ptr(), parent.data_ptr(), out.data_ptr(), out.stride(0),
                                     int(end_id), int(pad_id), finished_count.data_ptr(), all_finished_at.data_ptr(), int(t),
                                     ws.data_ptr(), ws.numel() * ws.element_size(), L.stream_ptr()), "vct_beam_select")


def beam_reorder(src, dst, parent, M: int, Lmax: int, d: int, t: int):
    L.check(L.load().vct_beam_reorder(L.dtype_code(src.dtype), src.shape[0], int(M), int(Lmax), int(d), int(t), parent.data_ptr(),
                                      src.data_ptr(), dst.data_ptr(), src.stride(0), L.stream_ptr()), "vct_beam_reorder")


def sample_select_workspace_bytes(dtype, rows: int, V: int) -> int:
    chunk = 256 * (8 if dtype == torch.bfloat16 else 4)
    return rows * ((V + chunk - 1) // chunk) * (2 + 2 * 64) * 4


def sample_select(x, out, end_id: int, pad_id: int, ended, ended_count, all_ended_at, t: int, step_logp, seq_logp, ctl, ws, cols=None):
    d = L.SampleSelectDesc()
    d.dtype, d.rows, d.V, d.t = L.dtype_code(x.dtype), x.shape[0], int(cols or x.shape[1]), int(t)
    d.x, d.ldx, d.out, d.out_stride = x.data_ptr(), _ld(x), out.data_ptr(), out.stride(0)
    d.end_id, d.pad_id = int(end_id), int(pad_id)
    d.ended, d.ended_count, d.all_ended_at = ended.data_ptr(), ended_count.data_ptr(), all_ended_at.data_ptr()
    d.step_logp, d.seq_logp, d.ctl = step_logp.data_ptr(), seq_logp.data_ptr(), ctl.data_ptr()
    d.workspace, d.workspace_bytes = ws.data_ptr(), ws.numel() * ws.element_size()
    L.check(L.load().vct_sample_select(L.C.byref(d), L.stream_ptr()), "vct_sample_select")


def decode_gemv(W, out, B, *, bias=None, pro="none", x_in=None, ln1=None, ln2=None, embed=None, attn=None, act=None, res=None,
                out_native=False, ld_out=None, x_out=None, n_valid=None):
    d = L.DecodeGemvDesc()
    d.wdtype, d.B, d.N, d.K = L.dtype_code(W.dtype), B, (n_valid or W.shape[0]), W.shape[1]
    d.W, d.ldw, d.bias = W.data_ptr(), _ld(W), L.ptr(bias)
    d.pro, d.act = L.DEC_PRO[pro], L.ACT[act]
    if x_in is not None:
        d.x_in, d.ld_x = x_in.data_ptr(), x_in.stride(0)
    if ln1 is not None:
        d.g1, d.b1 = ln1[0].data_ptr(), ln1[1].data_ptr()
    if ln2 is not None:
        d.g2, d.b2 = ln2[0].data_ptr(), ln2[1].data_ptr()
    if embed is not None:
        ids, table, pos_row = embed
        d.ids, d.id_stride, d.table, d.pos_row = ids.data_ptr(), ids.stride(0), table.data_ptr(), pos_row.data_ptr()
    if attn is not None:
        q, k, v, kv_ld, kv_bs, H, Lk = attn
        d.q, d.q_bs, d.kc, d.vc, d.kv_ld, d.kv_bs, d.H, d.Lk = q.data_ptr(), q.stride(0), k.data_ptr(), v.data_ptr(), kv_ld, kv_bs, H, Lk
    if res is not None:
        d.res, d.ld_res = res.data_ptr(), res.stride(0)
    d.out, d.ld_out, d.out_native = out.data_ptr(), (ld_out if ld_out is not None else out.stride(0)), int(out_native)
    d.x_out = L.ptr(x_out)
    L.check(L.load().vct_decode_gemv(d, L.stream_ptr()), "vct_decode_gemv")


def decode_block(kind: str, d: int, *, w_a, b_a, part_out, embed=None, res=None, res_bias=None, part=None, ln1=None, ln2=None, x_out=None,
                 slot=None, kc=None, vc=None, kv_ld=0, Lk=1, w_b=None, ff=0, act=None, V=0, select=None):
    q = L.DecodeBlockDesc()
    q.kind, q.d, q.ff, q.V, q.Lk, q.act = {"self": 0, "cross": 1, "ffn": 2, "gen": 3}[kind], d, ff, V, Lk, L.ACT[act]
    if embed is not None:
        ids, table, pos_row = embed
        q.id, q.table, q.pos_row = ids.data_ptr(), table.data_ptr(), pos_row.data_ptr()
    q.res, q.res_bias = L.ptr(res), L.ptr(res_bias)
    if part is not None:
        q.part, q.n_part = part.data_ptr(), part.shape[0]
    if ln1 is not None:
        q.g1, q.b1 = ln1[0].data_ptr(), ln1[1].data_ptr()
    if ln2 is not None:
        q.g2, q.b2 = ln2[0].data_ptr(), ln2[1].data_ptr()
    q.x_out = L.ptr(x_out)
    q.w_a, q.ld_a, q.b_a = w_a.data_ptr(), _ld(w_a), b_a.data_ptr()
    q.slot, q.kc, q.vc, q.kv_ld = L.ptr(slot), L.ptr(kc), L.ptr(vc), kv_ld
    if w_b is not None:
        q.w_b, q.ld_b = w_b.data_ptr(), _ld(w_b)
    q.part_out = part_out.data_ptr()
    if select is not None:
        ws, out, end_id, ended, ended_count, all_ended_at, t = select
        assert ws.numel() >= 2 * ((V + 127) // 128) + 1
        q.sel_ws, q.tok_out, q.end_id, q.ended = ws.data_ptr(), out.data_ptr(), int(end_id), ended.data_ptr()
        q.ended_count, q.all_ended_at, q.t = ended_count.data_ptr(), all_ended_at.data_ptr(), int(t)
    L.check(L.load().vct_decode_block(q, L.stream_ptr()), "vct_decode_block")


_db_ok = {}


def decode_block_supported(dtype, d: int, H: int, ff: int, Lk: int) -> bool:
    if dtype != torch.bfloat16:
        return False
    key = (d, H, ff, Lk)
    r = _db_ok.get(key)
    if r is None:
        r = _db_ok[key] = bool(L.load().vct_decode_block_supported(L.BF16, d, H, ff, Lk))
    return r


def transpose(src: torch.Tensor, dst: torch.Tensor):
    L.check(L.load().vct_transpose(L.dtype_code(src.dtype), src.shape[0], src.shape[1], src.data_ptr(), src.stride(0),
                                   dst.data_ptr(), dst.stride(0), L.stream_ptr()), "vct_transpose")
    return dst


def decode_linear(W, out, *, x=None, x_pre=None, ln=None, x_norm=None, bias=None, act=None, res=None, n_valid=None, embed=None):
    d = L.DecodeLinearDesc()
    d.M, d.N, d.K = out.shape[0], (n_valid or W.shape[0]), W.shape[1]
    d.out_dtype, d.act = L.dtype_code(out.dtype), L.ACT[act]
    if x is not None:
        d.x, d.ldx = x.data_ptr(), x.stride(0)
    if x_pre is not None:
        d.x_pre, d.ld_pre = x_pre.data_ptr(), x_pre.stride(0)
        d.ln_g, d.ln_b = ln[0].data_ptr(), ln[1].data_ptr()
    if embed is not None:
        ids, table, pos_row = embed
        d.x_pre, d.ld_pre, d.ln_b = table.data_ptr(), table.stride(0), pos_row.data_ptr()
        d.ids, d.id_stride = ids.data_ptr(), ids.stride(0)
    if x_norm is not None:
        d.x_norm, d.ld_norm = x_norm.data_ptr(), x_norm.stride(0)
    d.W, d.ldw, d.bias = W.data_ptr(), _ld(W), L.ptr(bias)
    if res is not None:
        d.res, d.ld_res, d.res_dtype = res.data_ptr(), res.stride(0), L.dtype_code(res.dtype)
    d.out, d.ldo = out.data_ptr(), out.stride(0)
    L.check(L.load().vct_decode_linear(d, L.stream_ptr()), "vct_decode_linear")
    return out


def decode_ln2(x, ln1, ln2, y):
    g2, b2 = (ln2[0].data_ptr(), ln2[1].data_ptr()) if ln2 is not None else (None, None)
    L.check(L.load().vct_decode_ln2(x.shape[0], x.shape[1], x.data_ptr(), x.stride(0), ln1[0].data_ptr(), ln1[1].data_ptr(), g2, b2,
                                    y.data_ptr(), y.stride(0), L.stream_ptr()), "vct_decode_ln2")
    return y


def gather_pad_rows(store: torch.Tensor, offsets: torch.Tensor, idx: torch.Tensor, tmax: int, out_dtype=torch.float32):
    B, E = idx.numel(), store.shape[1]
    out = torch.empty(B, tmax, E, dtype=out_dtype, device=store.device)
    mask = torch.empty(B, tmax, dtype=torch.bool, device=store.device)
    L.check(L.load().vct_gather_pad_rows(L.dtype_code(out_dtype), B, tmax, E, store.data_ptr(), offsets.data_ptr(), idx.data_ptr(),
                                         out.data_ptr(), mask.data_ptr(), L.stream_ptr()), "vct_gather_pad_rows")
    return out, mask


def _sptr(stream) -> int:
    return stream.cuda_stream if stream is not None else L.stream_ptr()


def stream_wait(waiter, signal):
    L.check(L.load().vct_stream_wait(_sptr(waiter), _sptr(signal)), "vct_stream_wait")


def sync_record(ident: int, stream=None):
    L.check(L.load().vct_sync_record(int(ident), _sptr(stream)), "vct_sync_record")


def sync_wait(ident: int, stream=None):
    L.check(L.load().vct_sync_wait(int(ident), _sptr(stream)), "vct_sync_wait")


import threading

_rec = threading.local()


def is_recording() -> bool:
    return getattr(_rec, "ll", None) is not None


_host_fns = []


def host_call(fn, stream=None):
    def thunk(_arg):
        try:
            fn()
            return 0
        except Exception:
            import traceback
            traceback.print_exc()
            return 1
    cfn = L.HOST_FN(thunk)
    ll = getattr(_rec, "ll", None)
    if ll is not None:
        ll._thunks.append(cfn)
    L.check(L.load().vct_cmdlist_host_call(L.C.cast(cfn, L.vp), None, _sptr(stream)), "vct_cmdlist_host_call")


def masked_stream(cu_bits, device=None):
    words = (L.u32 * 8)()
    n = 0
    for c in (cu_bits or ()):
        words[c // 32] |= (1 << (c % 32))
        n += 1
    h = L.vp()
    L.check(L.load().vct_stream_create_masked(words, 8 if n else 0, L.C.byref(h)), "vct_stream_create_masked")
    return torch.cuda.ExternalStream(h.value, device=device)


TAPS = {"gen_fwd": 0, "gen_dx": 1, "gen_dw": 2, "layers_fwd": 3, "loss": 4, "adam": 5, "step": 6,
        "comm_wait": 7, **{f"comm_b{i}": 8 + i for i in range(8)},
        "ss_enc": 16, "ss_dec": 17}
_taps_on = False
_taps_only = None


def taps_enable(on: bool, only=None):
    global _taps_on, _taps_only
    _taps_on = bool(on)
    _taps_only = None if only is None else frozenset(only)
    L.check(L.load().vct_tap_enable(int(_taps_on)), "vct_tap_enable")


def tap(tag: str, phase: int, stream=None):
    if _taps_on and (_taps_only is None or tag in _taps_only):
        L.check(L.load().vct_tap(TAPS[tag], phase, _sptr(stream)), "vct_tap")


def tap_collect(tag: str, cap: int = 4096):
    buf = (L.f32 * cap)()
    n = L.load().vct_tap_collect(TAPS[tag], buf, cap)
    if n < 0:
        L.check(n, "vct_tap_collect")
    return [float(buf[i]) for i in range(n)]


class LaunchList:

    def __init__(self):
        h = L.vp()
        L.check(L.load().vct_cmdlist_create(L.C.byref(h)), "vct_cmdlist_create")
        self._h = h
        self._thunks = []

    class _Rec:
        def __init__(self, ll):
            self.ll = ll

        def __enter__(self):
            L.check(L.load().vct_cmdlist_begin(self.ll._h, L.stream_ptr()), "vct_cmdlist_begin")
            self.ll._thunks = []
            _rec.ll = self.ll
            return self.ll

        def __exit__(self, *exc):
            _rec.ll = None
            L.check(L.load().vct_cmdlist_end(self.ll._h), "vct_cmdlist_end")
            return False

    def record(self):
        return LaunchList._Rec(self)

    def replay(self):
        L.check(L.load().vct_cmdlist_replay(self._h, L.stream_ptr()), "vct_cmdlist_replay")

    def __len__(self):
        return int(L.load().vct_cmdlist_size(self._h))

    @property
    def n_streams(self):
        return int(L.load().vct_cmdlist_streams(self._h))

    def close(self):
        if self._h is not None and self._h.value:
            L.load().vct_cmdlist_destroy(self._h)
            self._h = None
            self._thunks = []

    def __del__(self):
        try:
            self.close()
        except Exception:
            pass
```

### video-captioning-transformer_amd/trainer/optim.py

```python
import os

import torch

from .. import ops


def owned_range(model, task):
    if task in (None, "caption"):
        return 0, model.caption_param_end
    if task == "match":
        return model.encoder_param_begin, model._ps.total
    if task == "cross":
        return 0, model._ps.total
    raise ValueError(f"unknown task {task!r}")


class FusedAdam(torch.optim.Optimizer):

    def __init__(self, model, lr=1e-3, betas=(0.9, 0.999), eps=1e-8, weight_decay=0.0):
        self.model = model
        flat = torch.nn.Parameter(model.flat_params, requires_grad=True)
        flat.grad = model.flat_grads
        super().__init__([flat], dict(lr=lr, betas=betas, eps=eps, weight_decay=weight_decay))
        ps = model._ps
        self.exp_avg = torch.zeros_like(ps.flat)
        self.exp_avg_sq = torch.zeros_like(ps.flat)
        self.step_dev = torch.zeros(1, dtype=torch.int32, device=ps.flat.device)
        emb = "cap_decoder.tgt_to_emb.weight"
        a = ps.offsets[emb]
        self.skip = (a, a + (ps.params[emb].numel() + ps.ALIGN - 1) // ps.ALIGN * ps.ALIGN)
        self.task = model.f_type
        self.begin, self.end = owned_range(model, self.task)
        self.hyper = torch.zeros(8, dtype=torch.float32, device=ps.flat.device)
        self._hyper_host = None
        self.sync_hyper()
        self.pre_state_dict = None
        self._gathered_at = None
        self.dw_fusion = False
        self._dw_ranges = []
        self.range_elems = {}
        self._dw_desc = {}
        self._range_tables = {}

    def _hyper_now(self):
        g = self.param_groups[0]
        return (float(g["lr"]), float(g["betas"][0]), float(g["betas"][1]), float(g["eps"]), float(g["weight_decay"]))

    def sync_hyper(self):
        h = self._hyper_now()
        if h != self._hyper_host:
            self.hyper[:5].copy_(torch.tensor(h, dtype=torch.float32))
            self._hyper_host = h

    fuse_dw_default = os.environ.get("VCT_FUSE_ADAM", "1") != "0"
    keep_grads = os.environ.get("VCT_FUSE_ADAM_KEEP_GRAD", "0") == "1"

    def enable_dw_fusion(self, on: bool = True):
        ps = self.model._ps
        ok = bool(on) and ps.compute_dtype == torch.bfloat16 and ps.flat.is_cuda
        self.dw_fusion = ok
        ps.dw_adam = self if ok else None
        self._dw_ranges = []
        return ok

    def set_keep_grads(self, on: bool):
        if bool(on) != bool(self.keep_grads):
            self.keep_grads = bool(on)
            self._dw_desc.clear()

    def begin_step(self):
        self._dw_ranges = []

    def desc_for(self, dw: torch.Tensor):
        ps = self.model._ps
        off = (dw.data_ptr() - ps.gflat.data_ptr()) // 4
        if not self.dw_fusion or dw.dim() != 2 or dw.dtype != torch.float32 or not (self.begin <= off < self.end):
            return None
        name, base = ps.name_at(off)
        shape = ps.params[name].shape
        rows, K = dw.shape
        if len(shape) != 2 or K != shape[1] or dw.stride(0) != K or dw.stride(1) != 1 or (off - base) % K or name in ps.no_shadow:
            return None
        if K % 4 or off % 4 or (ps.flat.data_ptr() | self.exp_avg.data_ptr() | self.exp_avg_sq.data_ptr() | ps.gflat.data_ptr()) & 15 \
                or ps.cflat.data_ptr() & 7:
            return None
        key = (off, rows, tuple(sorted(ps.packed)))
        ad = self._dw_desc.get(key)
        if ad is None:
            ad = ops.L.GemmAdam()
            ad.param, ad.exp_avg, ad.exp_avg_sq = (t.data_ptr() + 4 * off for t in (ps.flat, self.exp_avg, self.exp_avg_sq))
            ad.shadow, ad.ld_shadow = ps.cflat.data_ptr() + 2 * off, K
            seg = ps.pack_seg(name)
            if seg is not None:
                ad.pk_K, ad.pk_mode, ad.pk_stream, ad.pk_row0 = seg.K, seg.mode, seg.stream, (off - base) // K
                for i in range(4):
                    ad.pk_chunk0[i] = seg.chunk0[i]
            ad.hyper, ad.step = self.hyper.data_ptr(), self.step_dev.data_ptr()
            ad.store_grad = int(self.keep_grads)
            self._dw_desc[key] = ad
        self._dw_ranges.append((off, off + rows * K))
        return ad

    def _left_ranges(self, a: int, b: int):
        cuts = sorted(set((max(x, a), min(y, b)) for x, y in self._dw_ranges if y > a and x < b))
        out, cur = [], a
        for x, y in cuts:
            if x > cur:
                out.append((cur, x))
            cur = max(cur, y)
        if cur < b:
            out.append((cur, b))
        res = []
        s0, s1 = self.skip
        for x, y in out:
            for lo, hi, sh in ((x, min(y, s0), True), (max(x, s0), min(y, s1), False), (max(x, s1), y, True)):
                if hi > lo:
                    res.append((lo, hi, sh))
        return res

    @torch.no_grad()
    def step(self, closure=None):
        if not torch.cuda.is_current_stream_capturing():
            self.sync_hyper()
        self.step_range(self.begin, self.end)
        self.finish_ranges()

    pack_in_adam = os.environ.get("VCT_ADAM_PACK", "1") != "0"
    adam_2d = os.environ.get("VCT_ADAM2D", "1") != "0"

    @torch.no_grad()
    def step_range(self, a: int, b: int):
        a, b = max(a, self.begin), min(b, self.end)
        if b <= a:
            return
        lr, b1, b2, eps, wd = self._hyper_now()
        ps = self.model._ps
        bf = ps.compute_dtype != torch.float32
        if self.dw_fusion and self._dw_ranges:
            left = self._left_ranges(a, b)
            self.range_elems[(a, b)] = sum(r[1] - r[0] for r in left)
            table, nseg, pk_parts = ps.adam_pack_table(a, b) if (self.pack_in_adam and ps.packed) else (None, 0, [])
            if left:
                key = (tuple(left), )
                tab = self._range_tables.get(key)
                if tab is None:
                    tab = self._range_tables[key] = ops.adam_ranges_table(left, ps.flat.device)
                ops.adam_step_ranges(ps.flat, ps.gflat, self.exp_avg, self.exp_avg_sq, ps.cflat, tab, lr, b1, b2, eps, wd, self.step_dev,
                                     hyper=self.hyper, pack=(table, nseg) if nseg else None)
            ps.refresh_transposed(a, b, packed_done=pk_parts)
            return
        fused = []
        if bf and self.adam_2d:
            fused = sorted((x, y, name, t) for name, t, x, y in ps.eager_transposed_in(a, b)
                           if ps.params[name].shape[1] % 64 == 0 and not (x < self.skip[1] and y > self.skip[0]))

        table, nseg, pk_parts = ps.adam_pack_table(a, b) if (bf and self.pack_in_adam and ps.packed) else (None, 0, [])

        def flat_range(lo, hi):
            if hi <= lo:
                return
            shadow = ps.cflat[lo:hi] if bf else None
            s0, s1 = max(self.skip[0], lo) - lo, min(self.skip[1], hi) - lo
            ops.adam_step(ps.flat[lo:hi], ps.gflat[lo:hi], self.exp_avg[lo:hi], self.exp_avg_sq[lo:hi], shadow, lr, b1, b2, eps, wd,
                          self.step_dev, (s0, s1) if s1 > s0 else (0, 0), bump=False, hyper=self.hyper,
                          pack=(table, nseg, lo) if nseg else None)
        cur = a
        for x, y, name, t in fused:
            flat_range(cur, x)
            shape = ps.params[name].shape
            ops.adam_step_2d(ps.flat[x:y].view(shape), ps.gflat[x:y].view(shape), self.exp_avg[x:y].view(shape),
                             self.exp_avg_sq[x:y].view(shape), ps.cflat[x:y].view(shape), t, lr, b1, b2, eps, wd, self.step_dev,
                             hyper=self.hyper)
            cur = y
        flat_range(cur, b)
        if bf:
            ps.refresh_transposed(a, b, skip=[name for _x, _y, name, _t in fused], packed_done=pk_parts)

    @torch.no_grad()
    def finish_ranges(self):
        ops.adam_bump(self.step_dev)
        self.model._ps.optimizer_stepped()

    def zero_grad(self, set_to_none: bool = True):
        pass

    def gather_state(self):
        if self.pre_state_dict is not None:
            self.pre_state_dict()
        self._gathered_at = int(self.step_dev.item())

    def state_dict(self):
        if self.pre_state_dict is not None and self._gathered_at != int(self.step_dev.item()):
            raise RuntimeError("FusedAdam.state_dict() under a sharded exchange: call optimizer.gather_state() on EVERY rank first "
                               "(checkpoint.save_training_state does), then state_dict() on the rank(s) that write")
        sd = super().state_dict()
        ps = self.model._ps
        sd["vct_fused_adam"] = {"exp_avg": self.exp_avg.detach().clone(), "exp_avg_sq": self.exp_avg_sq.detach().clone(),
                                "step": int(self.step_dev.item()), "numel": ps.flat.numel(),
                                "layout": [(k, int(ps.offsets[k])) for k in ps.params]}
        return sd

    def load_state_dict(self, state_dict):
        sd = dict(state_dict)
        fused = sd.pop("vct_fused_adam", None)
        if fused is None:
            raise ValueError("not a FusedAdam state (no 'vct_fused_adam' entry)")
        ps = self.model._ps
        if fused["numel"] != ps.flat.numel() or [tuple(x) for x in fused["layout"]] != [(k, int(ps.offsets[k])) for k in ps.params]:
            raise ValueError("optimizer state was saved for a different parameter layout")
        super().load_state_dict(sd)
        self.exp_avg.copy_(fused["exp_avg"])
        self.exp_avg_sq.copy_(fused["exp_avg_sq"])
        self.step_dev.fill_(fused["step"])
        self._gathered_at = None
        self.sync_hyper()


def build_optimizer(train_cfg: dict, model):
    oc = train_cfg["optimizer"]

    def flat():
        p = torch.nn.Parameter(model.flat_params, requires_grad=True)
        p.grad = model.flat_grads
        return [p]
    if oc["name"] == "adam":
        if model.flat_params.is_cuda:
            opt = FusedAdam(model, lr=oc["learning_rate"], betas=tuple(oc["beta"]), weight_decay=oc.get("weight_decay", 0) or 0.0)
        elif oc.get("weight_decay", 0) == 0:
            opt = torch.optim.Adam(flat(), lr=oc["learning_rate"], betas=tuple(oc["beta"]))
        else:
            opt = torch.optim.AdamW(flat(), lr=oc["learning_rate"], betas=tuple(oc["beta"]), weight_decay=oc["weight_decay"])
    elif oc["name"] == "sgd":
        opt = torch.optim.SGD(flat(), lr=oc["learning_rate"], momentum=oc["momentum"])
    else:
        raise ValueError("Do not support optimizer: {}".format(oc["name"]))
    sched = None
    sc = oc.get("lr_scheduler")
    if sc:
        if sc["name"] == "CosineAnnealingLR":
            sched = torch.optim.lr_scheduler.CosineAnnealingLR(opt, T_max=sc["T_max"], eta_min=sc["eta_min"])
        elif sc["name"] == "ReduceLROnPlateau":
            sched = torch.optim.lr_scheduler.ReduceLROnPlateau(opt, patience=sc["patience"])
        else:
            raise ValueError("Do not support lr_scheduler: {}".format(sc["name"]))
    return opt, sched
```

### video-captioning-transformer_amd/trainer/step.py

```python
from typing import Optional
import os

import torch
import torch.distributed as dist

from .. import ops
from ..engine import first_input, stage_inputs, static_inputs
from ..utils import capture_graph
from .exchange import GradExchange, ShardedExchange
from .optim import FusedAdam


class CaptionTrainer:

    def __init__(self, model, optimizer, exchange: Optional[GradExchange] = None, use_graph: bool = False,
                 launch_list: Optional[bool] = None, keep_weight_grads: Optional[bool] = None):
        self.model, self.opt, self.ex = model, optimizer, exchange
        fused = self._fused = isinstance(optimizer, FusedAdam)
        self.task = (optimizer.task if fused else model.f_type) or "caption"
        self._asked = (bool(use_graph), bool(launch_list))
        self._check_task(self.task)
        if keep_weight_grads is not None and fused:
            optimizer.set_keep_grads(bool(keep_weight_grads))
        model._unit_loss_grad = True
        single = (exchange is None or not exchange.active) and fused
        listable = single or (isinstance(exchange, ShardedExchange) and getattr(exchange.coll, "recordable", False))
        self.use_graph = bool(use_graph) and single
        self.use_list = (bool(launch_list) if launch_list is not None else False) and listable and not self.use_graph
        self._lists = {}
        self._graphs = {}
        self._static = {}
        self._attn = {}
        self._gen = None
        if single and model.flat_grads.is_cuda:
            model.cap_decoder._engine().exclusive_grads = True
        self.overlap_adam = False
        self.fuse_adam = bool(single and optimizer.fuse_dw_default and self.task == "caption"
                              and model._ps.compute_dtype == torch.bfloat16 and model.flat_grads.is_cuda)

    def _check_task(self, task):
        if task not in ("match", "cross"):
            return
        self.model.check_task(task)
        if self._asked[0] or self._asked[1]:
            raise NotImplementedError(f"task {task!r} runs on the eager executor only: use_graph / launch_list recordings of it are not built")
        if self.ex is not None and self.ex.active:
            raise NotImplementedError(f"task {task!r} is single-process only: the gradient exchange of it is not built")

    def _step_task(self, feats, mask, ids, text_feats):
        m = self.model
        if text_feats is None:
            raise ValueError(f"task {self.task!r}: pass text_feats (fp32 [B, {m.text_encoder.dim}] on the model's device)")
        ops.tap("step", 0)
        if not self._fused:
            m._ps.masters_written()
        else:
            m._ps.refresh_shadow()
        if self.task == "match":
            out = m.train_step_kernels_match(feats, mask, text_feats)
        else:
            out = m.train_step_kernels_cross(feats, mask, ids, text_feats)
        self.opt.step()
        if m.training and m.video_encoder.cfg["dropout"] > 0:
            ops.advance_seed(m._seed)
        ops.tap("step", 1)
        return out

    def _check_scst(self, num_samples, baseline):
        if self._asked[0] or self._asked[1]:
            raise NotImplementedError("scst_step runs on the eager executor only: build the trainer without use_graph / launch_list")
        if self.ex is not None and self.ex.active:
            raise NotImplementedError("scst_step is single-process only: the gradient exchange of it is not built")
        if (self.model.f_type or "caption") != "caption" or self.task != "caption":
            raise ValueError(f"scst_step trains the caption task: model.mode({self.model.f_type!r}), optimizer built for {self.task!r}")
        if int(num_samples) < 1:
            raise ValueError(f"num_samples must be >= 1, got {num_samples}")
        if baseline not in ("mean_others", "greedy"):
            raise ValueError(f"baseline must be 'mean_others' or 'greedy', got {baseline!r}")
        if baseline == "mean_others" and int(num_samples) < 2:
            raise ValueError("baseline 'mean_others' is the leave-one-out mean of the other samples: it needs num_samples >= 2")

    def scst_step(self, feats, mask, reward_fn, vids=None, *, num_samples: int = 5, baseline: str = "mean_others", max_len: int = 30,
                  temperature: float = 1.0, top_k: int = 0, top_p: float = 1.0, seed=None):
        self._check_scst(num_samples, baseline)
        if getattr(reward_fn, "on_device", False):
            return self._scst_step_device(feats, mask, reward_fn, vids, int(num_samples), baseline, max_len, temperature, top_k, top_p,
                                          seed)
        from ..rewards import advantages
        import numpy as np
        m, N = self.model, int(num_samples)
        if self._fused:
            self.opt.sync_hyper()
            m._ps.refresh_shadow()
        else:
            m._ps.masters_written()
        B = first_input(feats).shape[0]
        vids = list(range(B)) if vids is None else list(vids)
        ids = m.sample_decode_ids(feats, mask, num_samples=N, max_len=max_len, temperature=temperature, top_k=top_k, top_p=top_p,
                                  seed=seed)
        greedy = m.greedy_decode_ids(feats, mask, max_len=max_len) if baseline == "greedy" else None
        r = np.asarray(reward_fn(ids.cpu(), vids), np.float32)
        if r.shape != (B, N):
            raise ValueError(f"reward_fn must return [B = {B}, N = {N}] rewards, got {r.shape}")
        if greedy is not None:
            base = np.asarray(reward_fn(greedy.cpu().view(B, 1, -1), vids), np.float32).reshape(B)
            adv = advantages(r, base)
        else:
            adv = advantages(r, "mean_others")
            base = r - adv
        seq_w = torch.from_numpy(np.ascontiguousarray(adv.reshape(-1))).to(ids.device)
        loss = m.train_step_kernels_scst(feats, mask, ids.view(B * N, -1), seq_w, N)
        self.opt.step()
        if m.training and m.video_encoder.cfg["dropout"] > 0:
            ops.advance_seed(m._seed)
        return dict(loss=loss.clone(), reward_mean=float(r.mean()), baseline_mean=float(base.mean()), ids=ids)

    def _scst_step_device(self, feats, mask, reward_fn, vids, N, baseline, max_len, temperature, top_k, top_p, seed):
        from ..rewards import DEVICE_MAX_LEN
        if int(max_len) > 1 + DEVICE_MAX_LEN:
            raise ValueError(f"scst_step: a device reward scores the start column + at most {DEVICE_MAX_LEN} tokens, got max_len = {max_len}")
        m = self.model
        B = first_input(feats).shape[0]
        vids = list(range(B)) if vids is None else list(vids)
        if len(vids) != B:
            raise ValueError(f"scst_step: {B} videos and {len(vids)} video ids")
        rows = getattr(reward_fn, "video_rows", None)
        if rows is not None:
            rows(vids)
        if self._fused:
            self.opt.sync_hyper()
            m._ps.refresh_shadow()
        else:
            m._ps.masters_written()
        ids = m.sample_decode_ids(feats, mask, num_samples=N, max_len=max_len, temperature=temperature, top_k=top_k, top_p=top_p,
                                  seed=seed)
        greedy = m.greedy_decode_ids(feats, mask, max_len=max_len) if baseline == "greedy" else None
        r = reward_fn(ids, vids)
        if not torch.is_tensor(r) or tuple(r.shape) != (B, N) or r.dtype != torch.float32 or r.device != ids.device:
            raise ValueError(f"a device reward_fn must return fp32 [B = {B}, N = {N}] on {ids.device}, got {getattr(r, 'shape', type(r))}")
        base = reward_fn(greedy.view(B, 1, -1), vids).view(B) if greedy is not None else None
        seq_w, _, means = ops.scst_advantages(r.contiguous(), base)
        loss = m.train_step_kernels_scst(feats, mask, ids.view(B * N, -1), seq_w, N)
        self.opt.step()
        if m.training and m.video_encoder.cfg["dropout"] > 0:
            ops.advance_seed(m._seed)
        return dict(loss=loss.clone(), reward_mean=means[0], baseline_mean=means[1], ids=ids)

    adam_after_backward = os.environ.get("VCT_ADAM_TAIL", "0") == "1"
    warm_streams = os.environ.get("VCT_WARM_STREAMS", "1") != "0"

    def _step_kernels(self, feats, mask, ids):
        if not self.fuse_adam:
            return self._step_kernels_body(feats, mask, ids)
        self.opt.enable_dw_fusion(True)
        self.opt.begin_step()
        try:
            return self._step_kernels_body(feats, mask, ids)
        finally:
            self.opt.enable_dw_fusion(False)

    def _step_kernels_body(self, feats, mask, ids):
        m = self.model
        fused = self._fused
        ops.tap("step", 0)
        if not fused:
            m._ps.masters_written()
        else:
            m._ps.refresh_shadow()
        exchanging = self.ex is not None and self.ex.active
        if exchanging and isinstance(self.ex, ShardedExchange):
            loss = m.train_step_kernels(feats, mask, ids, bucket_ready=self.ex.bucket_ready)
            self.ex.finish()
        elif exchanging:
            loss = m.train_step_kernels(feats, mask, ids, bucket_ready=self.ex.bucket_ready)
            if fused:
                self.ex.finish(on_bucket_done=self.opt.step_range)
                self.opt.finish_ranges()
            else:
                self.ex.finish()
                self.opt.step()
        elif fused and self.overlap_adam and first_input(feats).is_cuda:
            buckets = m.grad_buckets()
            ctx = m._ps.ctx

            def hook(i):
                side = ctx.side
                if side is None:
                    self.opt.step_range(*buckets[i])
                    return
                ops.stream_wait(side, None)
                with torch.cuda.stream(side):
                    self.opt.step_range(*buckets[i])
            loss = m.train_step_kernels(feats, mask, ids, bucket_ready=hook)
            if ctx.side is not None:
                ops.stream_wait(None, ctx.side)
            self.opt.finish_ranges()
        elif fused and first_input(feats).is_cuda and m.overlap_enc_bwd and not self.adam_after_backward:
            loss = m.train_step_kernels(feats, mask, ids, defer_join=True)
            a = m.encoder_param_begin
            m.cap_decoder._engine().join_side()
            if m.encoder_backward_is_one_launch():
                m.launch_encoder_backward(main=True)
            ops.tap("adam", 0)
            self.opt.step_range(0, a)
            ops.tap("adam", 1)
            m.launch_encoder_backward()
            m.join_backward()
            self.opt.step_range(a, m._ps.total)
            self.opt.finish_ranges()
        else:
            loss = m.train_step_kernels(feats, mask, ids)
            self.opt.step()
        if self.warm_streams and first_input(feats).is_cuda:
            for stream in m._ps.packed.values():
                ops.warm(stream.t)
        if m.training and m.video_encoder.cfg["dropout"] > 0:
            ops.advance_seed(m._seed)
        ops.tap("step", 1)
        return loss

    def _fresh_shadow(self):
        self.model._ps.refresh_shadow()

    def drop_recordings(self):
        self._lists.clear()
        self._graphs.clear()
        self._attn.clear()

    def _static_inputs(self, key, feats, mask, ids):
        s = self._static.get(key)
        if s is None:
            s = self._static[key] = (static_inputs(feats), static_inputs(mask), ids.clone())
        else:
            stage_inputs(s[0], feats, non_blocking=True)
            if mask is not None:
                stage_inputs(s[1], mask, non_blocking=True)
            if s[2].data_ptr() != ids.data_ptr():
                s[2].copy_(ids, non_blocking=True)
        return s

    def _input_key(self, feats, mask, ids):
        if isinstance(feats, (list, tuple)):
            return (tuple((tuple(f.shape), f.dtype) for f in feats), None if mask is None else tuple(tuple(m.shape) for m in mask),
                    tuple(ids.shape), self.model.training)
        return (tuple(feats.shape), feats.dtype, None if mask is None else tuple(mask.shape), tuple(ids.shape), self.model.training)

    def adopt_inputs(self, feats, mask, ids: torch.Tensor):
        if not (self.use_graph or self.use_list):
            return feats, mask, ids
        return self._static_inputs(self._input_key(feats, mask, ids), feats, mask, ids)

    def _check_generation(self):
        gen = self.model._ps.ctx.generation
        if self._gen != gen:
            self.drop_recordings()
            self._gen = gen

    def _record_list(self, static):
        ll = ops.LaunchList()
        with ll.record():
            loss = self._step_kernels(*static)
        return ll, loss

    def _capture_graph(self, static):
        torch.cuda.synchronize()
        graph = torch.cuda.CUDAGraph()
        try:
            with capture_graph(graph):
                loss = self._step_kernels(*static)
        except Exception:
            self.use_graph = False
            return None
        return graph, loss

    def step(self, feats, mask, ids: torch.Tensor, text_feats: Optional[torch.Tensor] = None):
        task = self.model.f_type or "caption"
        if task != self.task:
            raise ValueError(f"model.mode({task!r}) but the optimizer was built for {self.task!r}: build the optimizer after model.mode(task)")
        if self._fused:
            self.opt.sync_hyper()
        if task != "caption":
            self._check_task(task)
            return self._step_task(feats, mask, ids, text_feats)
        if not (self.use_graph or self.use_list):
            return self._step_kernels(feats, mask, ids)
        self._check_generation()
        key = self._input_key(feats, mask, ids)
        static = self._static_inputs(key, feats, mask, ids)
        cache, record = (self._lists, self._record_list) if self.use_list else (self._graphs, self._capture_graph)
        hit = cache.get(key)
        if hit is None:
            eager_loss = self._step_kernels(*static).clone()
            self._check_generation()
            hit = record(static)
            if hit is not None:
                cache[key] = hit
                if self.model.cap_decoder.custom_decoder_type is not None:
                    self._attn[key] = self.model.cap_decoder.attn_weights
            return eager_loss
        recording, loss = hit
        self._fresh_shadow()
        recording.replay()
        if key in self._attn:
            self.model.cap_decoder.attn_weights = self._attn[key]
        self.model._ps.shadow_replayed()
        return loss


def _to_device(model, v_feats, v_masks):
    dev = model.flat_params.device
    if model.video_encoder.num_modal > 1:
        feats = [f.to(dev, non_blocking=True) for f in v_feats]
        mask = [m.to(dev, non_blocking=True) for m in v_masks] if v_masks is not None else None
    else:
        feats = v_feats[0].to(dev, non_blocking=True)
        mask = v_masks[0].to(dev, non_blocking=True) if v_masks is not None else None
    return feats, mask


def train_epoch(model, optimizer, dataloader, mode: str = "caption", exchange: Optional[GradExchange] = None,
                log_every: int = 0, text_feats_fn=None):
    if mode not in ("caption", "match", "cross"):
        raise ValueError(f"unknown task {mode!r}")
    model.train()
    model.mode(mode)
    trainer = CaptionTrainer(model, optimizer, exchange)
    dev = model.flat_params.device
    total = torch.zeros(3 if mode == "cross" else 1, device=dev)
    n = 0
    for v_feats, v_masks, captions, vids in dataloader:
        feats, mask = _to_device(model, v_feats, v_masks)
        if mode == "caption":
            ids, _ = model.cap_preprocessor(captions)
            total += trainer.step(feats, mask, ids)
        else:
            text = text_feats_fn(captions, vids) if text_feats_fn is not None else model.text_encoder(captions)
            text = text.to(dev, non_blocking=True) if torch.is_tensor(text) else text
            ids = model.cap_preprocessor(captions)[0] if mode == "cross" else None
            out = trainer.step(feats, mask, ids, text)
            total += torch.cat(out) if mode == "cross" else out
        n += 1
    if exchange is not None and exchange.world > 1:
        dist.all_reduce(total, op=dist.ReduceOp.SUM, group=exchange.group)
        total /= exchange.world
    if mode == "cross":
        return tuple(v / max(n, 1) for v in total.tolist())
    return float(total) / max(n, 1)


def scst_epoch(model, optimizer, dataloader, reward_fn, **kw):
    model.train()
    model.mode("caption")
    trainer = CaptionTrainer(model, optimizer)
    total = torch.zeros(1, device=model.flat_params.device)
    on_device = bool(getattr(reward_fn, "on_device", False))
    reward, n = (torch.zeros((), dtype=torch.float64, device=model.flat_params.device) if on_device else 0.0), 0
    for v_feats, v_masks, _captions, vids in dataloader:
        feats, mask = _to_device(model, v_feats, v_masks)
        out = trainer.scst_step(feats, mask, reward_fn, vids, **kw)
        total += out["loss"]
        reward += out["reward_mean"]
        n += 1
    return float(total) / max(n, 1), float(reward) / max(n, 1)
```

Before: 116,700 samples/s.

## Skip Adam updates for embedding rows with zero grad and zero moments

```diff
diff --git a/include/vct_hip.h b/include/vct_hip.h
--- a/include/vct_hip.h
+++ b/include/vct_hip.h
@@ -220,6 +220,11 @@
 int vct_embed_bwd(int dtype, int B, int S, int d, int V, const int64_t* ids, int64_t id_batch_stride,
                   int64_t pad_id, const void* dx, float* dtable, int32_t* id_ws, int64_t id_ws_ints, int incremental,
                   const uint32_t* seed, uint32_t site, float p_drop, void* stream);
+int vct_embed_bwd_live(int dtype, int B, int S, int d, int V, const int64_t* ids, int64_t id_batch_stride,
+                       int64_t pad_id, const void* dx, float* dtable, int32_t* id_ws, int64_t id_ws_ints, int incremental,
+                       const uint32_t* seed, uint32_t site, float p_drop, uint8_t* live, void* stream);
+int vct_embed_live_rebuild(int32_t V, int32_t d, const float* grad_rows, const float* exp_avg_rows, const float* exp_avg_sq_rows,
+                           uint8_t* live, void* stream);
 
 int vct_sce_loss(int dtype, int N, int S, int V, const void* logits, int64_t ldl, const int64_t* labels,
                  int64_t label_batch_stride, int64_t pad_id, float alpha, float* loss_out, void* dlogits,
@@ -300,6 +305,11 @@
                          const vct_adam_range* ranges_dev, int32_t nranges, int32_t total_blocks, float lr, float beta1, float beta2,
                          float eps, float weight_decay, int32_t* step_dev, const float* hyper_dev,
                          const vct_adam_pack_seg* segs_dev, int32_t nseg, void* stream);
+typedef struct vct_adam_rows { int64_t origin; int32_t row_len, nrows; const uint8_t* live; } vct_adam_rows;
+int vct_adam_step_ranges_rows(float* param, const float* grad, float* exp_avg, float* exp_avg_sq, void* shadow_bf16,
+                              const vct_adam_range* ranges_dev, int32_t nranges, int32_t total_blocks, float lr, float beta1, float beta2,
+                              float eps, float weight_decay, int32_t* step_dev, const float* hyper_dev,
+                              const vct_adam_pack_seg* segs_dev, int32_t nseg, const vct_adam_rows* rows_dev, void* stream);
 int vct_adam_step_2d(float* param, const float* grad, float* exp_avg, float* exp_avg_sq, void* shadow_bf16,
                      void* shadow_t_bf16, int32_t rows, int32_t cols, int64_t ld_t, float lr, float beta1, float beta2,
                      float eps, float weight_decay, int32_t* step_dev, const float* hyper_dev, void* stream);
diff --git a/video-captioning-transformer_amd/_lib.py b/video-captioning-transformer_amd/_lib.py
--- a/video-captioning-transformer_amd/_lib.py
+++ b/video-captioning-transformer_amd/_lib.py
@@ -25,6 +25,10 @@
 
 class AdamRange(C.Structure):
     _fields_ = [("begin", i64), ("end", i64), ("blk0", i32), ("shadow", i32)]
+
+
+class AdamRows(C.Structure):
+    _fields_ = [("origin", i64), ("row_len", i32), ("nrows", i32), ("live", vp)]
 
 
 class GemmDesc(C.Structure):
@@ -216,6 +220,8 @@
     "vct_axpby": (C.c_int, [vp, vp, f32, vp, f32, i64, vp]),
     "vct_embed_fwd": (C.c_int, [C.c_int, C.c_int, C.c_int, C.c_int, vp, i64, vp, vp, vp, vp, u32, f32, vp]),
     "vct_embed_bwd": (C.c_int, [C.c_int, C.c_int, C.c_int, C.c_int, C.c_int, vp, i64, i64, vp, vp, vp, i64, C.c_int, vp, u32, f32, vp]),
+    "vct_embed_bwd_live": (C.c_int, [C.c_int, C.c_int, C.c_int, C.c_int, C.c_int, vp, i64, i64, vp, vp, vp, i64, C.c_int, vp, u32, f32, vp, vp]),
+    "vct_embed_live_rebuild": (C.c_int, [i32, i32, vp, vp, vp, vp, vp]),
     "vct_sce_loss": (C.c_int, [C.c_int, C.c_int, C.c_int, C.c_int, vp, i64, vp, i64, i64, f32, vp, vp, i64, vp, vp]),
     "vct_wce_loss": (C.c_int, [C.c_int, C.c_int, C.c_int, C.c_int, vp, i64, vp, i64, i64, vp, vp, vp, vp, i64, vp, vp]),
     "vct_group_sum": (C.c_int, [C.c_int, C.c_int, C.c_int, C.c_int, C.c_int, vp, vp, vp]),
@@ -240,6 +246,7 @@
     "vct_adam_step": (C.c_int, [vp, vp, vp, vp, vp, i64, f32, f32, f32, f32, f32, vp, i64, i64, i32, vp, vp]),
     "vct_adam_step_pk": (C.c_int, [vp, vp, vp, vp, vp, i64, f32, f32, f32, f32, f32, vp, i64, i64, i32, vp, vp, C.c_int, i64, vp]),
     "vct_adam_step_ranges": (C.c_int, [vp, vp, vp, vp, vp, vp, i32, i32, f32, f32, f32, f32, f32, vp, vp, vp, i32, vp]),
+    "vct_adam_step_ranges_rows": (C.c_int, [vp, vp, vp, vp, vp, vp, i32, i32, f32, f32, f32, f32, f32, vp, vp, vp, i32, vp, vp]),
     "vct_adam_step_2d": (C.c_int, [vp, vp, vp, vp, vp, vp, i32, i32, i64, f32, f32, f32, f32, f32, vp, vp, vp]),
     "vct_cmdlist_create": (C.c_int, [C.POINTER(vp)]),
     "vct_cmdlist_destroy": (C.c_int, [vp]),
diff --git a/video-captioning-transformer_amd/csrc/vct_elem.hip b/video-captioning-transformer_amd/csrc/vct_elem.hip
--- a/video-captioning-transformer_amd/csrc/vct_elem.hip
+++ b/video-captioning-transformer_amd/csrc/vct_elem.hip
@@ -78,17 +78,19 @@
   }
 }
 
-__global__ void embed_index_kernel(int N, int S, const int64_t* __restrict__ ids, int64_t id_bstride, int64_t pad_id,
+__global__ void embed_index_kernel(int N, int S, int V, const int64_t* __restrict__ ids, int64_t id_bstride, int64_t pad_id,
                                    int32_t* __restrict__ first_pos, int32_t* __restrict__ cnt, int32_t* __restrict__ hdr,
-                                   int32_t* __restrict__ flat_cur) {
+                                   int32_t* __restrict__ flat_cur, uint8_t* __restrict__ live) {
   const int n = blockIdx.x * blockDim.x + threadIdx.x;
   if (n == 0) hdr[1] = N;
   if (n >= N) return;
   const int64_t id = ids[(size_t)(n / S) * id_bstride + (n % S)];
-  flat_cur[n] = (int32_t)id;
-  if (id == pad_id) return;
+  const bool in_table = id >= 0 && id < V;
+  flat_cur[n] = in_table ? (int32_t)id : -1;
+  if (id == pad_id || !in_table) return;
   atomicMin(&first_pos[id], n);
   atomicAdd(&cnt[id], 1);
+  if (live != nullptr) live[id] = 1;
 }
 
 constexpr int EMB_LIGHT_MAX = 8;
@@ -103,7 +105,7 @@
   const int lane = threadIdx.x & 63;
   if (n >= N) return;
   const int32_t id = flat[n];
-  if (id == pad_id || first_pos[id] != n) return;
+  if (id < 0 || id == pad_id || first_pos[id] != n) return;
   const int occurrences = cnt[id];
   if (occurrences > EMB_LIGHT_MAX) return;
   const Dropout dr = make_dropout(seed, site, p_drop);
@@ -584,6 +586,13 @@
 extern "C" int vct_embed_bwd(int dtype, int B, int S, int d, int V, const int64_t* ids, int64_t id_batch_stride,
                              int64_t pad_id, const void* dx, float* dtable, int32_t* id_ws, int64_t id_ws_ints, int incremental,
                              const uint32_t* seed, uint32_t site, float p_drop, void* stream) {
+  return vct_embed_bwd_live(dtype, B, S, d, V, ids, id_batch_stride, pad_id, dx, dtable, id_ws, id_ws_ints, incremental, seed, site, p_drop,
+                            nullptr, stream);
+}
+
+extern "C" int vct_embed_bwd_live(int dtype, int B, int S, int d, int V, const int64_t* ids, int64_t id_batch_stride,
+                                  int64_t pad_id, const void* dx, float* dtable, int32_t* id_ws, int64_t id_ws_ints, int incremental,
+                                  const uint32_t* seed, uint32_t site, float p_drop, uint8_t* live, void* stream) {
   if (!dt_ok(dtype) || !ids || !dx || !dtable || !id_ws) return VCT_E_ARG;
   if (B <= 0 || S <= 0 || d <= 0 || V <= 0) return VCT_E_SHAPE;
   if (d % vec_of(dtype) || d / vec_of(dtype) > 256 || (d % 4) || d > 1024) return VCT_E_SHAPE;
@@ -598,7 +607,8 @@
   vct::launch(embed_prep_kernel, dim3(incremental ? 512 : 2048), dim3(256), 0, st, V, d, dtable, first_pos, cnt, flat, hdr,
               incremental ? 1 : 0);
   VCT_CHECK_LAUNCH();
-  vct::launch(embed_index_kernel, dim3((N + 255) / 256), dim3(256), 0, st, N, S, ids, id_batch_stride, pad_id, first_pos, cnt, hdr, flat);
+  vct::launch(embed_index_kernel, dim3((N + 255) / 256), dim3(256), 0, st, N, S, V, ids, id_batch_stride, pad_id, first_pos, cnt,
+              hdr, flat, live);
   VCT_CHECK_LAUNCH();
   const int vecb = vec_of(dtype);
   const int slots = 1024 / (d / vecb);
diff --git a/video-captioning-transformer_amd/csrc/vct_optim.hip b/video-captioning-transformer_amd/csrc/vct_optim.hip
--- a/video-captioning-transformer_amd/csrc/vct_optim.hip
+++ b/video-captioning-transformer_amd/csrc/vct_optim.hip
@@ -93,7 +93,49 @@
 }
 
 struct AdamRange { int64_t begin, end; int32_t blk0, shadow; };
+struct AdamRows { int64_t origin; int32_t row_len, nrows; const uint8_t* live; };
 constexpr int ADAM_RANGE_EPB = 4096;
+
+__device__ __forceinline__ bool adam_zero_row_is_noop(float lr, float b1, float b2, float eps, float wd, const float* hyper,
+                                                      const int32_t* step) {
+  if (hyper != nullptr) { lr = hyper[0]; b1 = hyper[1]; b2 = hyper[2]; eps = hyper[3]; wd = hyper[4]; }
+  const bool decay_is_one = __fmaf_rn(-lr, wd, 1.0f) == 1.0f && __fsub_rn(1.0f, __fmul_rn(lr, wd)) == 1.0f;
+  return decay_is_one && eps > 0.0f && eps <= 3.402823466e+38f && lr >= 0.0f && lr <= 1e30f && b1 >= 0.0f && b1 <= 0.9999f &&
+         b2 >= 0.0f && b2 <= 0.99999f && step[0] >= 0;
+}
+
+__device__ __forceinline__ void adam_range_step4(const int64_t e, float* __restrict__ p, const float* __restrict__ g,
+                                                 float* __restrict__ m, float* __restrict__ v, bf16_t* __restrict__ shadow,
+                                                 const bool with_shadow, const AdamConsts& hc, const AdamPackSeg* __restrict__ segs,
+                                                 const int nseg) {
+  float4 pv = *reinterpret_cast<float4*>(p + e);
+  const float4 gv = *reinterpret_cast<const float4*>(g + e);
+  float4 mv = *reinterpret_cast<float4*>(m + e);
+  float4 vv = *reinterpret_cast<float4*>(v + e);
+  float* pp = &pv.x; const float* gp = &gv.x; float* mp = &mv.x; float* vp = &vv.x;
+#pragma unroll
+  for (int j = 0; j < 4; j++) adam_update(pp[j], gp[j], mp[j], vp[j], hc);
+  *reinterpret_cast<float4*>(p + e) = pv;
+  *reinterpret_cast<float4*>(m + e) = mv;
+  *reinterpret_cast<float4*>(v + e) = vv;
+  if (with_shadow) {
+    ushort4 o;
+    o.x = f2bf(pv.x); o.y = f2bf(pv.y); o.z = f2bf(pv.z); o.w = f2bf(pv.w);
+    *reinterpret_cast<ushort4*>(shadow + e) = o;
+    if (nseg > 0) {
+      int slo = 0, shi = nseg;
+      while (shi - slo > 1) { const int mid = (slo + shi) >> 1; if (segs[mid].begin <= e) slo = mid; else shi = mid; }
+      const AdamPackSeg sg = segs[slo];
+      if (e >= sg.begin && e < sg.end) {
+        const int64_t rel = e - sg.begin;
+        const int r = (int)(rel / sg.K), c = (int)(rel - (int64_t)r * sg.K);
+        const int64_t at = adam_pack_index(r, c, sg.mode, adam_pack_chunks(sg.chunk0[0], sg.chunk0[1], sg.chunk0[2], sg.chunk0[3]));
+        if (at >= 0) *reinterpret_cast<ushort4*>(sg.stream + at) = o;
+      }
+    }
+  }
+}
+
 __global__ __launch_bounds__(256) void adam_ranges_kernel(float* __restrict__ p, const float* __restrict__ g, float* __restrict__ m,
                                                           float* __restrict__ v, bf16_t* __restrict__ shadow,
                                                           const AdamRange* __restrict__ ranges, int nranges, float lr, float b1, float b2,
@@ -105,33 +147,91 @@
   const AdamRange rg = ranges[lo];
   const int64_t e0 = rg.begin + (int64_t)((int)blockIdx.x - rg.blk0) * ADAM_RANGE_EPB;
   const int64_t e1 = e0 + ADAM_RANGE_EPB < rg.end ? e0 + ADAM_RANGE_EPB : rg.end;
+  for (int64_t e = e0 + (int64_t)threadIdx.x * 4; e < e1; e += 256 * 4)
+    adam_range_step4(e, p, g, m, v, shadow, shadow != nullptr && rg.shadow, hc, segs, nseg);
+}
+
+__global__ __launch_bounds__(256) void adam_ranges_kernel_rows(float* __restrict__ p, const float* __restrict__ g, float* __restrict__ m,
+                                                               float* __restrict__ v, bf16_t* __restrict__ shadow,
+                                                               const AdamRange* __restrict__ ranges, int nranges, float lr, float b1,
+                                                               float b2, float eps, float wd, const int32_t* __restrict__ step,
+                                                               const float* __restrict__ hyper, const AdamPackSeg* __restrict__ segs,
+                                                               int nseg, const AdamRows* __restrict__ rows) {
+  int lo = 0, hi = nranges;
+  while (hi - lo > 1) { const int mid = (lo + hi) >> 1; if (ranges[mid].blk0 <= (int)blockIdx.x) lo = mid; else hi = mid; }
+  const AdamRange rg = ranges[lo];
+  const AdamRows rw = rows[lo];
+  const int64_t e0 = rg.begin + (int64_t)((int)blockIdx.x - rg.blk0) * ADAM_RANGE_EPB;
+  const int64_t e1 = e0 + ADAM_RANGE_EPB < rg.end ? e0 + ADAM_RANGE_EPB : rg.end;
+  const int lane = threadIdx.x & 63, wave = threadIdx.x >> 6;
+  const bool table = rw.live != nullptr && rw.row_len >= 4 && (rw.row_len & 3) == 0 && rw.nrows > 0 && !rg.shadow &&
+                     e0 >= rw.origin && ((e0 - rw.origin) & 3) == 0;
+  const int64_t rel0 = e0 - rw.origin;
+  const bool whole = table && (rw.row_len & 255) == 0 && ADAM_RANGE_EPB % rw.row_len == 0 && rel0 % rw.row_len == 0;
+  unsigned long long mask = 0ull;
+  int nrw = 0;
+  if (whole) {
+    nrw = (int)((e1 - e0 + rw.row_len - 1) / rw.row_len);
+    const int64_t row = rel0 / rw.row_len + lane;
+    const int on = lane < nrw ? (row < rw.nrows ? (int)rw.live[row] : 1) : 0;
+    mask = __ballot(on != 0);
+  }
+  const bool skip = table && adam_zero_row_is_noop(lr, b1, b2, eps, wd, hyper, step);
+  if (skip && whole && (mask & (0x1111111111111111ull << wave)) == 0ull) return;
+  const AdamConsts hc = adam_consts(lr, b1, b2, eps, wd, hyper, step);
+  if (!skip) {
+    for (int64_t e = e0 + (int64_t)threadIdx.x * 4; e < e1; e += 256 * 4)
+      adam_range_step4(e, p, g, m, v, shadow, shadow != nullptr && rg.shadow, hc, segs, nseg);
+    return;
+  }
+  if (whole) {
+    for (int rl = wave; rl < nrw; rl += 4) {
+      if (((mask >> rl) & 1ull) == 0ull) continue;
+      const int64_t eb = e0 + (int64_t)rl * rw.row_len;
+      for (int c = lane * 4; c < rw.row_len; c += 512) {
+        const int64_t ea[2] = {eb + c, eb + c + 256};
+        const bool has[2] = {ea[0] < e1, c + 256 < rw.row_len && ea[1] < e1};
+        float4 pv[2], gv[2], mv[2], vv[2];
+#pragma unroll
+        for (int u = 0; u < 2; u++)
+          if (has[u]) {
+            pv[u] = *reinterpret_cast<float4*>(p + ea[u]); gv[u] = *reinterpret_cast<const float4*>(g + ea[u]);
+            mv[u] = *reinterpret_cast<float4*>(m + ea[u]); vv[u] = *reinterpret_cast<float4*>(v + ea[u]);
+          }
+#pragma unroll
+        for (int u = 0; u < 2; u++)
+          if (has[u]) {
+            float* pp = &pv[u].x; const float* gp = &gv[u].x; float* mp = &mv[u].x; float* vp = &vv[u].x;
+#pragma unroll
+            for (int j = 0; j < 4; j++) adam_update(pp[j], gp[j], mp[j], vp[j], hc);
+            *reinterpret_cast<float4*>(p + ea[u]) = pv[u];
+            *reinterpret_cast<float4*>(m + ea[u]) = mv[u];
+            *reinterpret_cast<float4*>(v + ea[u]) = vv[u];
+          }
+      }
+    }
+    return;
+  }
   for (int64_t e = e0 + (int64_t)threadIdx.x * 4; e < e1; e += 256 * 4) {
-    float4 pv = *reinterpret_cast<float4*>(p + e);
-    const float4 gv = *reinterpret_cast<const float4*>(g + e);
-    float4 mv = *reinterpret_cast<float4*>(m + e);
-    float4 vv = *reinterpret_cast<float4*>(v + e);
-    float* pp = &pv.x; const float* gp = &gv.x; float* mp = &mv.x; float* vp = &vv.x;
-#pragma unroll
-    for (int j = 0; j < 4; j++) adam_update(pp[j], gp[j], mp[j], vp[j], hc);
-    *reinterpret_cast<float4*>(p + e) = pv;
-    *reinterpret_cast<float4*>(m + e) = mv;
-    *reinterpret_cast<float4*>(v + e) = vv;
-    if (shadow != nullptr && rg.shadow) {
-      ushort4 o;
-      o.x = f2bf(pv.x); o.y = f2bf(pv.y); o.z = f2bf(pv.z); o.w = f2bf(pv.w);
-      *reinterpret_cast<ushort4*>(shadow + e) = o;
-      if (nseg > 0) {
-        int slo = 0, shi = nseg;
-        while (shi - slo > 1) { const int mid = (slo + shi) >> 1; if (segs[mid].begin <= e) slo = mid; else shi = mid; }
-        const AdamPackSeg sg = segs[slo];
-        if (e >= sg.begin && e < sg.end) {
-          const int64_t rel = e - sg.begin;
-          const int r = (int)(rel / sg.K), c = (int)(rel - (int64_t)r * sg.K);
-          const int64_t at = adam_pack_index(r, c, sg.mode, adam_pack_chunks(sg.chunk0[0], sg.chunk0[1], sg.chunk0[2], sg.chunk0[3]));
-          if (at >= 0) *reinterpret_cast<ushort4*>(sg.stream + at) = o;
-        }
-      }
-    }
+    const int64_t row = (e - rw.origin) / rw.row_len;
+    if (row < rw.nrows && rw.live[row] == 0) continue;
+    adam_range_step4(e, p, g, m, v, shadow, false, hc, segs, nseg);
+  }
+}
+
+__global__ __launch_bounds__(256) void embed_live_rebuild_kernel(int V, int d, const float* __restrict__ g, const float* __restrict__ m,
+                                                                 const float* __restrict__ v, uint8_t* __restrict__ live) {
+  const int lane = threadIdx.x & 63;
+  const int nw = gridDim.x * 4;
+  for (int r = blockIdx.x * 4 + (threadIdx.x >> 6); r < V; r += nw) {
+    uint32_t any = 0;
+    const size_t base = (size_t)r * d;
+    for (int c = lane; c < d; c += 64) {
+      any |= __float_as_uint(m[base + c]) | __float_as_uint(v[base + c]);
+      if (g != nullptr) any |= __float_as_uint(g[base + c]);
+    }
+    const unsigned long long b = __ballot(any != 0);
+    if (lane == 0) live[r] = b != 0ull ? 1 : 0;
   }
 }
 
@@ -179,13 +279,40 @@
                                     const vct_adam_range* ranges_dev, int32_t nranges, int32_t total_blocks, float lr, float beta1,
                                     float beta2, float eps, float weight_decay, int32_t* step_dev, const float* hyper_dev,
                                     const vct_adam_pack_seg* segs_dev, int32_t nseg, void* stream) {
+  return vct_adam_step_ranges_rows(param, grad, exp_avg, exp_avg_sq, shadow_bf16, ranges_dev, nranges, total_blocks, lr, beta1, beta2, eps,
+                                   weight_decay, step_dev, hyper_dev, segs_dev, nseg, nullptr, stream);
+}
+
+extern "C" int vct_adam_step_ranges_rows(float* param, const float* grad, float* exp_avg, float* exp_avg_sq, void* shadow_bf16,
+                                         const vct_adam_range* ranges_dev, int32_t nranges, int32_t total_blocks, float lr, float beta1,
+                                         float beta2, float eps, float weight_decay, int32_t* step_dev, const float* hyper_dev,
+                                         const vct_adam_pack_seg* segs_dev, int32_t nseg, const vct_adam_rows* rows_dev, void* stream) {
   static_assert(sizeof(vct_adam_range) == sizeof(AdamRange), "descriptor layout");
+  static_assert(sizeof(vct_adam_rows) == sizeof(AdamRows), "descriptor layout");
   if (!param || !grad || !exp_avg || !exp_avg_sq || !step_dev || !ranges_dev || nranges < 1 || total_blocks < 1) return VCT_E_ARG;
   if (nseg < 0 || (nseg > 0 && (segs_dev == nullptr || shadow_bf16 == nullptr))) return VCT_E_ARG;
   if (((uintptr_t)param | (uintptr_t)grad | (uintptr_t)exp_avg | (uintptr_t)exp_avg_sq) & 15) return VCT_E_ALIGN;
-  vct::launch(adam_ranges_kernel, dim3(total_blocks), dim3(256), 0, (hipStream_t)stream, param, grad, exp_avg, exp_avg_sq,
-              (bf16_t*)shadow_bf16, reinterpret_cast<const AdamRange*>(ranges_dev), (int)nranges, lr, beta1, beta2, eps, weight_decay,
-              step_dev, hyper_dev, reinterpret_cast<const AdamPackSeg*>(segs_dev), (int)nseg);
+  if ((uintptr_t)rows_dev & 7) return VCT_E_ALIGN;
+  if (rows_dev == nullptr)
+    vct::launch(adam_ranges_kernel, dim3(total_blocks), dim3(256), 0, (hipStream_t)stream, param, grad, exp_avg, exp_avg_sq,
+                (bf16_t*)shadow_bf16, reinterpret_cast<const AdamRange*>(ranges_dev), (int)nranges, lr, beta1, beta2, eps, weight_decay,
+                step_dev, hyper_dev, reinterpret_cast<const AdamPackSeg*>(segs_dev), (int)nseg);
+  else
+    vct::launch(adam_ranges_kernel_rows, dim3(total_blocks), dim3(256), 0, (hipStream_t)stream, param, grad, exp_avg, exp_avg_sq,
+                (bf16_t*)shadow_bf16, reinterpret_cast<const AdamRange*>(ranges_dev), (int)nranges, lr, beta1, beta2, eps, weight_decay,
+                step_dev, hyper_dev, reinterpret_cast<const AdamPackSeg*>(segs_dev), (int)nseg,
+                reinterpret_cast<const AdamRows*>(rows_dev));
+  VCT_CHECK_LAUNCH();
+  return VCT_OK;
+}
+
+extern "C" int vct_embed_live_rebuild(int32_t V, int32_t d, const float* grad_rows, const float* exp_avg_rows, const float* exp_avg_sq_rows,
+                                      uint8_t* live, void* stream) {
+  if (!exp_avg_rows || !exp_avg_sq_rows || !live) return VCT_E_ARG;
+  if (V < 1 || d < 1) return VCT_E_SHAPE;
+  const int blocks = (V + 3) / 4 < 2048 ? (V + 3) / 4 : 2048;
+  vct::launch(embed_live_rebuild_kernel, dim3(blocks), dim3(256), 0, (hipStream_t)stream, (int)V, (int)d, grad_rows, exp_avg_rows,
+              exp_avg_sq_rows, live);
   VCT_CHECK_LAUNCH();
   return VCT_OK;
 }
diff --git a/video-captioning-transformer_amd/ops.py b/video-captioning-transformer_amd/ops.py
--- a/video-captioning-transformer_amd/ops.py
+++ b/video-captioning-transformer_amd/ops.py
@@ -472,13 +472,35 @@
 
 _embed_ws = {}
 _embed_ws_retired = []
-
-
-def embed_bwd(ids, S, pad_id, dx, dtable, dropout: Drop = None, id_ws=None, exclusive: bool = False, on_grow=None):
+_embed_live = {}
+
+
+def embed_live_table(dtable, create: bool = False):
+    key = (dtable.shape[0], dtable.device, dtable.data_ptr())
+    live = _embed_live.get(key)
+    if live is None and create:
+        live = _embed_live[key] = torch.zeros(dtable.shape[0], dtype=torch.uint8, device=dtable.device)
+    return live
+
+
+def embed_live_rebuild(live, exp_avg_rows, exp_avg_sq_rows, grad_rows=None):
+    V, d = exp_avg_rows.shape
+    assert live.numel() >= V and live.dtype == torch.uint8
+    for t in (exp_avg_rows, exp_avg_sq_rows, grad_rows):
+        assert t is None or (t.dtype == torch.float32 and t.is_contiguous() and tuple(t.shape) == (V, d))
+    L.check(L.load().vct_embed_live_rebuild(V, d, L.ptr(grad_rows), exp_avg_rows.data_ptr(), exp_avg_sq_rows.data_ptr(), live.data_ptr(),
+                                            L.stream_ptr()), "vct_embed_live_rebuild")
+
+
+def embed_bwd(ids, S, pad_id, dx, dtable, dropout: Drop = None, id_ws=None, exclusive: bool = False, on_grow=None, live=None):
     B = ids.shape[0]
     s, site, p = _drop(dropout)
     V = dtable.shape[0]
     incremental = False
+    if live is None:
+        live = embed_live_table(dtable)
+    else:
+        assert live.dtype == torch.uint8 and live.numel() >= V
     if id_ws is None:
         key = (V, dx.device, dtable.data_ptr())
         ent = _embed_ws.get(key)
@@ -494,9 +516,9 @@
         ent[1] = dtable.data_ptr() if exclusive else None
     else:
         assert id_ws.numel() >= 2 * V + 4 + B * S
-    L.check(L.load().vct_embed_bwd(L.dtype_code(dx.dtype), B, S, dx.shape[1], V, ids.data_ptr(),
-                                   ids.stride(0), int(pad_id), dx.data_ptr(), dtable.data_ptr(), id_ws.data_ptr(), id_ws.numel(), int(incremental),
-                                   s, site, p, L.stream_ptr()), "vct_embed_bwd")
+    L.check(L.load().vct_embed_bwd_live(L.dtype_code(dx.dtype), B, S, dx.shape[1], V, ids.data_ptr(),
+                                        ids.stride(0), int(pad_id), dx.data_ptr(), dtable.data_ptr(), id_ws.data_ptr(), id_ws.numel(),
+                                        int(incremental), s, site, p, L.ptr(live), L.stream_ptr()), "vct_embed_bwd_live")
 
 
 def sce_loss(logits, V, labels, S, pad_id, alpha, loss_out, dlogits, row_ws):
@@ -701,7 +723,7 @@
             "vct_adam_step")
 
 
-def adam_ranges_table(ranges, device):
+def adam_ranges_table(ranges, device, rows=None):
     EPB = 4096
     arr = (L.AdamRange * len(ranges))()
     blk = 0
@@ -710,12 +732,26 @@
         arr[i].begin, arr[i].end, arr[i].blk0, arr[i].shadow = int(a), int(b), blk, int(bool(sh))
         blk += (b - a + EPB - 1) // EPB
     table = torch.frombuffer(bytearray(bytes(arr)), dtype=torch.uint8).to(device)
-    return table, len(ranges), blk
+    if not rows:
+        return table, len(ranges), blk
+    rarr = (L.AdamRows * len(ranges))()
+    for i, (origin, row_len, nrows, live) in rows.items():
+        assert 0 <= i < len(ranges) and not ranges[i][2], "a range with a bf16 shadow is stepped densely: give it no row table"
+        assert row_len > 0 and row_len % 4 == 0 and origin % 4 == 0 and live.dtype == torch.uint8 and live.numel() >= nrows
+        rarr[i].origin, rarr[i].row_len, rarr[i].nrows, rarr[i].live = int(origin), int(row_len), int(nrows), live.data_ptr()
+    rtable = torch.frombuffer(bytearray(bytes(rarr)), dtype=torch.uint8).to(device)
+    return table, len(ranges), blk, rtable, [r[3] for r in rows.values()]
 
 
 def adam_step_ranges(param, grad, exp_avg, exp_avg_sq, shadow, table, lr, beta1, beta2, eps, weight_decay, step_dev, hyper=None, pack=None):
-    tab, n, blocks = table
+    tab, n, blocks = table[:3]
     pk, nseg = (pack[0].data_ptr(), int(pack[1])) if pack is not None and pack[1] else (0, 0)
+    if len(table) > 3:
+        L.check(L.load().vct_adam_step_ranges_rows(param.data_ptr(), grad.data_ptr(), exp_avg.data_ptr(), exp_avg_sq.data_ptr(),
+                                                   L.ptr(shadow), tab.data_ptr(), int(n), int(blocks), float(lr), float(beta1),
+                                                   float(beta2), float(eps), float(weight_decay), step_dev.data_ptr(), L.ptr(hyper), pk,
+                                                   nseg, table[3].data_ptr(), L.stream_ptr()), "vct_adam_step_ranges_rows")
+        return
     L.check(L.load().vct_adam_step_ranges(param.data_ptr(), grad.data_ptr(), exp_avg.data_ptr(), exp_avg_sq.data_ptr(), L.ptr(shadow),
                                           tab.data_ptr(), int(n), int(blocks), float(lr), float(beta1), float(beta2), float(eps),
                                           float(weight_decay), step_dev.data_ptr(), L.ptr(hyper), pk, nseg, L.stream_ptr()),
diff --git a/video-captioning-transformer_amd/trainer/optim.py b/video-captioning-transformer_amd/trainer/optim.py
--- a/video-captioning-transformer_amd/trainer/optim.py
+++ b/video-captioning-transformer_amd/trainer/optim.py
@@ -41,6 +41,11 @@
         self.range_elems = {}
         self._dw_desc = {}
         self._range_tables = {}
+        self._emb = emb
+        self._live = None
+        self._live_stale = True
+        if self.live_rows and ps.flat.is_cuda and ps.g[emb].dim() == 2:
+            self._live = ops.embed_live_table(ps.g[emb], create=True)
 
     def _hyper_now(self):
         g = self.param_groups[0]
@@ -67,6 +72,31 @@
         if bool(on) != bool(self.keep_grads):
             self.keep_grads = bool(on)
             self._dw_desc.clear()
+
+    live_rows = os.environ.get("VCT_ADAM_LIVE", "1") != "0"
+
+    def live_refresh(self):
+        if not self.live_rows or self.keep_grads:
+            return
+        ps = self.model._ps
+        g = ps.g[self._emb]
+        if g.dim() != 2 or not ps.flat.is_cuda:
+            return
+        if self._live is None:
+            self._live = ops.embed_live_table(g, create=True)
+            self._live_stale = True
+        if self._live_stale:
+            a, (V, d) = self.skip[0], g.shape
+            ops.embed_live_rebuild(self._live, self.exp_avg[a:a + V * d].view(V, d), self.exp_avg_sq[a:a + V * d].view(V, d), g)
+            self._live_stale = False
+
+    def _live_rows_for(self, left):
+        if not self.live_rows or self.keep_grads or self._live is None or self._live_stale:
+            return None
+        s0, s1 = self.skip
+        V, d = self.model._ps.g[self._emb].shape
+        rows = {i: (s0, d, V, self._live) for i, (lo, hi, sh) in enumerate(left) if not sh and lo >= s0 and hi <= s1}
+        return rows or None
 
     def begin_step(self):
         self._dw_ranges = []
@@ -141,14 +171,19 @@
             self.range_elems[(a, b)] = sum(r[1] - r[0] for r in left)
             table, nseg, pk_parts = ps.adam_pack_table(a, b) if (self.pack_in_adam and ps.packed) else (None, 0, [])
             if left:
-                key = (tuple(left), )
+                rows = self._live_rows_for(left)
+                if rows is None and any(lo < self.skip[1] and hi > self.skip[0] for lo, hi, _sh in left):
+                    self._live_stale = True
+                key = (tuple(left), rows is not None)
                 tab = self._range_tables.get(key)
                 if tab is None:
-                    tab = self._range_tables[key] = ops.adam_ranges_table(left, ps.flat.device)
+                    tab = self._range_tables[key] = ops.adam_ranges_table(left, ps.flat.device, rows)
                 ops.adam_step_ranges(ps.flat, ps.gflat, self.exp_avg, self.exp_avg_sq, ps.cflat, tab, lr, b1, b2, eps, wd, self.step_dev,
                                      hyper=self.hyper, pack=(table, nseg) if nseg else None)
             ps.refresh_transposed(a, b, packed_done=pk_parts)
             return
+        if a < self.skip[1] and b > self.skip[0]:
+            self._live_stale = True
         fused = []
         if bf and self.adam_2d:
             fused = sorted((x, y, name, t) for name, t, x, y in ps.eager_transposed_in(a, b)
@@ -212,6 +247,7 @@
         self.exp_avg.copy_(fused["exp_avg"])
         self.exp_avg_sq.copy_(fused["exp_avg_sq"])
         self.step_dev.fill_(fused["step"])
+        self._live_stale = True
         self._gathered_at = None
         self.sync_hyper()
 
diff --git a/video-captioning-transformer_amd/trainer/step.py b/video-captioning-transformer_amd/trainer/step.py
--- a/video-captioning-transformer_amd/trainer/step.py
+++ b/video-captioning-transformer_amd/trainer/step.py
@@ -279,6 +279,8 @@
             raise ValueError(f"model.mode({task!r}) but the optimizer was built for {self.task!r}: build the optimizer after model.mode(task)")
         if self._fused:
             self.opt.sync_hyper()
+        if self.fuse_adam:
+            self.opt.live_refresh()
         if task != "caption":
             self._check_task(task)
             return self._step_task(feats, mask, ids, text_feats)
```

After: 120,100 samples/s (median of 6 runs). +2.9%, better.
